# TheoCoombes/ClipCap

Measured on AMD Instinct MI355X. Metric: train samples/sec (512-d prefix, 40-tok caption), higher is better.
Workload: dtype bf16; 1 GPU; BASELINE configs[1]: TransformerMapper(8L,P=L=10,H=8)+frozen GPT-2-small; per_gpu_batch=256, global_batch=256, encoder_dim=512, train_language_model=False, parallelism=dp1

## Files before the change

### clipcap_amd/csrc/api.hip

```cpp
#include "../../include/clipcap_hip.h"
#include "gemm_api.h"
#include "kernels.h"
#include "shared.h"
#include "layout.h"
#include <vector>

using namespace CC_NS;

namespace {

#define CC_TIMED(site, st, expr)                 \
    do {                                         \
        cc_shared::ProfScope _ps(site, st);      \
        int _e = (expr);                         \
        if (_e != CC_OK) return _e;              \
    } while (0)

struct TileScope {
    int old;
    bool on;
    explicit TileScope(int mode) : old(cc_shared::g_gemm_tile_mode), on(mode != -2) { if (on) cc_shared::g_gemm_tile_mode = mode; }
    ~TileScope() { if (on) cc_shared::g_gemm_tile_mode = old; }
};
inline int env_tile(const char* name) {
// ... 70 lines not shown
        w.wg_scratch = cv.take<float>(WGRAD_SCRATCH_BYTES / sizeof(float));
        w.red = cv.take<float>(RED_SCRATCH_FLOATS);
        w.adelta = cv.take<float>((size_t)B * c->H * S);
        w.gimg = kX3 ? reinterpret_cast<uint16_t*>(cv.take<char>(x3_img(M, std::max<size_t>(3 * (size_t)D, c->Hm)))) : nullptr;
    } else {
        w.dx32 = nullptr; w.dx16 = w.dx16b = w.dh16 = w.dxn16 = w.datt16 = w.dqkv16 = w.dlin16 = nullptr; w.wg_scratch = nullptr; w.adelta = nullptr;
        w.red = nullptr;
        w.gimg = nullptr;
        for (int l = 0; l < c->N; l++) w.gdx[l] = w.gdxb[l] = w.gdh[l] = w.gdqkv[l] = nullptr;
        w.own_grads = false;
    }
    w.x3 = nullptr; w.x3_bytes = 0;
    if (kX3) {
        const size_t Hm = c->Hm, Mb = (size_t)B * c->W, PD = (size_t)c->P * D;
        size_t need = std::max(x3_img(Mb, c->E), x3_img(M, std::max(D, Hm)));
        if (save) {
            need = std::max(need, x3_img(M, 3 * D));
            need = std::max(need, std::max(x3_img(M, D) + x3_img(M, Hm), x3_img(M, 3 * D) + x3_img(M, D)));
            need = std::max(need, x3_img(Mb, PD) + x3_img(Mb, c->E));
        }
        w.x3_bytes = need;
        w.x3 = cv.take<char>(need);
    }
    w.bytes = cv.bytes();
}

struct MapperPass {
    hipStream_t st;
    MapperOff o;
    MapperWS w;
    Call cx;
    int D, PP, S, M, H, hd, Hm, PD;
    MapperPass(const cc_mapper_cfg* c, int B, int save, void* ws, void* stream)
        : st(S_(stream)), o(c), D(c->D), PP(c->W * c->P), S(PP + c->L), M(B * S), H(c->H), hd(c->D / c->H), Hm(c->Hm), PD(c->P * c->D) {
        mapper_carve(c, B, save, ws, w);
        cx = call_of(st, w);
    }
};

static bool x3_img_on() {
    static const bool on = []() { const char* e = cc_lab_env("CC_X3_IMG"); return !e || atoi(e) != 0; }();
    return on;
}
static bool lm_exp_form(const cc_gpt2_shape* s) {
    static const bool env = []() { const char* e = cc_lab_env("CC_LM_EXPFORM"); return !e || atoi(e) != 0; }();
    if (CC_OP == 0) return env;
    if (CC_OP == 2) return env && x3_img_on() && s->mode == 1;
    return false;
}
static Act lm_logits(const cc_gpt2_cfg* c, const cc_gpt2_shape* s, act_t* logits16) { return Act(logits16, (kX3 && lm_exp_form(s)) ? c->Vp : 0); }

struct Gpt2WS {
    float* x[MAX_LAYERS + 1];
    float* x1[MAX_LAYERS];
    act_t *qkv[MAX_LAYERS], *u[MAX_LAYERS];
    Act xn1[MAX_LAYERS], xn2[MAX_LAYERS], att[MAX_LAYERS], hact[MAX_LAYERS];
    float *lse[MAX_LAYERS], *mean1[MAX_LAYERS], *rstd1[MAX_LAYERS], *mean2[MAX_LAYERS], *rstd2[MAX_LAYERS];
    act_t* hf16;
    float *meanf, *rstdf;
    int *target, *row_map;
    int* keep;
    act_t* logits16;
    float *pmax, *psum, *tgt_logit, *lse_row, *row_loss;
    float *cref, *lmfac;
    act_t* hfs16;
    float* dx32;
    Act dx16, dx16b, du16, dqkv16;
    act_t *dhf16, *dxn16, *datt16;
    float* wg_scratch;
    float* red;
    void* scat;
    float* adelta;
    char* x3;
    size_t x3_bytes;
    size_t bytes;
};

void gpt2_carve(const cc_gpt2_cfg* c, const cc_gpt2_shape* s, int cap, void* ws, Gpt2WS& w) {
    Carver cv(ws);
    const int B = s->B, T = s->T, hd = c->D / c->H;
    const size_t M = (size_t)B * T, D = c->D, Mc = (size_t)B * cap;
    const bool keep = s->mode >= 1, full = s->mode >= 2;
    const auto take_img = [&](size_t n) { return cv.take<act_t>(n * ((kX3 && !full) ? 3 : 2) / 2); };
    const bool img = kX3 && !full && x3_img_on();
    const bool bimg = img && keep && s->p_resid == 0.f && s->p_attn == 0.f && s->p_embd == 0.f;
    const int xw = img ? (int)D : 0, attw = (img && attn_fwd_can_image(T, hd)) ? (int)D : 0, hw = img ? 4 * (int)D : 0;
    const int dxw = bimg ? (int)D : 0, dqw = (bimg && attn_bwd_can_image(T, hd)) ? 3 * (int)D : 0;
    const int nx = keep ? c->NL + 1 : 2;
    float* xb[MAX_LAYERS + 1];
    for (int i = 0; i < nx; i++) xb[i] = cv.take<float>(M * D);
    for (int l = 0; l <= c->NL; l++) w.x[l] = keep ? xb[l] : xb[l & 1];
    for (int l = 0; l < c->NL; l++) {
        const bool k0 = keep || l == 0, f0 = full || l == 0;
        w.x1[l] = k0 ? cv.take<float>(M * D) : w.x1[0];
        w.qkv[l] = k0 ? cv.take<act_t>(M * 3 * D) : w.qkv[0];
        w.u[l] = k0 ? cv.take<act_t>(M * 4 * D) : w.u[0];
        w.lse[l] = k0 ? cv.take<float>((size_t)B * c->H * T) : w.lse[0];
        w.mean1[l] = k0 ? cv.take<float>(M) : w.mean1[0];
        w.rstd1[l] = k0 ? cv.take<float>(M) : w.rstd1[0];
        w.mean2[l] = k0 ? cv.take<float>(M) : w.mean2[0];
        w.rstd2[l] = k0 ? cv.take<float>(M) : w.rstd2[0];
        w.xn1[l] = f0 ? Act(take_img(M * D), xw) : w.xn1[0];
        w.xn2[l] = f0 ? Act(take_img(M * D), xw) : w.xn2[0];
        w.att[l] = k0 ? Act(take_img(M * D), attw) : w.att[0];
        w.hact[l] = f0 ? Act(take_img(M * 4 * D), hw) : w.hact[0];
    }
    const size_t Mh = std::max(M, Mc);
    w.hf16 = cv.take<act_t>(Mh * D);
    w.meanf = cv.take<float>(Mh);
    w.rstdf = cv.take<float>(Mh);
    w.target = cv.take<int>(Mh);
    w.row_map = cv.take<int>(Mh);
    w.keep = nullptr;
    if (keep) {
        const int npart = c->Vp / 64;
        w.logits16 = take_img(Mc * c->Vp);
        w.pmax = cv.take<float>(Mc * npart);
        w.psum = cv.take<float>(Mc * npart);
        w.tgt_logit = cv.take<float>(Mc);
        w.lse_row = cv.take<float>(Mc);
        w.row_loss = cv.take<float>(Mc);
        w.cref = cv.take<float>(Mc);
        w.lmfac = cv.take<float>(2 * Mc);
        w.hfs16 = full ? cv.take<act_t>(Mc * D) : nullptr;
        w.dx32 = cv.take<float>(M * D);
        w.dx16 = Act(take_img(M * D), dxw);
        w.dx16b = full ? Act(cv.take<act_t>(M * D)) : w.dx16;
        w.dhf16 = cv.take<act_t>(Mc * D);
        w.du16 = Act(take_img(M * 4 * D), hw);
        w.dxn16 = cv.take<act_t>(M * D);
        w.datt16 = cv.take<act_t>(M * D);
        w.dqkv16 = Act(take_img(M * 3 * D), dqw);
        w.wg_scratch = full ? cv.take<float>(WGRAD_SCRATCH_BYTES / sizeof(float)) : nullptr;
        w.red = full ? cv.take<float>(RED_SCRATCH_FLOATS) : nullptr;
        w.scat = full ? cv.take<char>(scatter_ws_bytes((int)Mc, (int)D)) : nullptr;
        w.adelta = cv.take<float>((size_t)B * c->H * T);
    } else {
        w.wg_scratch = nullptr; w.adelta = nullptr; w.red = nullptr; w.scat = nullptr;
        w.logits16 = nullptr; w.pmax = w.psum = w.tgt_logit = w.lse_row = w.row_loss = nullptr;
        w.cref = w.lmfac = nullptr; w.hfs16 = nullptr;
        w.dx32 = nullptr; w.dx16 = w.dx16b = w.du16 = w.dqkv16 = Act(); w.dhf16 = w.dxn16 = w.datt16 = nullptr;
        if (Mc > 0) {
            const int npart = c->Vp / 64;
            w.pmax = cv.take<float>(Mc * npart);
            w.psum = cv.take<float>(Mc * npart);
            w.tgt_logit = cv.take<float>(Mc);
            w.lse_row = cv.take<float>(Mc);
            w.keep = cv.take<int>(Mc);
        }
    }
    w.x3 = nullptr; w.x3_bytes = 0;
    if (kX3) {
        size_t need = x3_img(Mh, 4 * D);
        if (keep) need = std::max(need, x3_img(Mc, c->Vp));
        if (full) need = std::max(need, std::max(x3_img(M, D) + x3_img(M, 4 * D), x3_img(Mc, c->Vp) + x3_img(Mc, D)));
        w.x3_bytes = need;
        w.x3 = cv.take<char>(need);
    }
    w.bytes = cv.bytes();
}

struct Gpt2Pass {
    hipStream_t st;
    Gpt2Off o;
    Gpt2WS w;
    Call cx;
    int D, M, H, hd;
    Gpt2Pass(const cc_gpt2_cfg* c, const cc_gpt2_shape* s, int cap, void* ws, void* stream)
        : st(S_(stream)), o(c), D(c->D), M(s->B * s->T), H(c->H), hd(c->D / c->H) {
        gpt2_carve(c, s, cap, ws, w);
        cx = call_of(st, w);
    }
};

}

extern "C" {

int CC_API(cc_mapper_bwd_range)(const cc_mapper_cfg* c, int32_t B, const float* w32, const uint16_t* w16, void* ws, const float* dout, float* g32,
                        int32_t l_hi, int32_t l_lo, void* stream);
int CC_API(cc_gpt2_bwd_range)(const cc_gpt2_cfg* c, const cc_gpt2_shape* s, const float* w32, const uint16_t* w16, void* ws, const int64_t* tokens,
                      float* dprefix, float* g32, int32_t l_hi, int32_t l_lo, void* stream);

int64_t CC_API(cc_mapper_param_count)(const cc_mapper_cfg* cfg) {
    if (!mapper_cfg_ok(cfg)) return CC_ERR_SHAPE;
    return MapperOff(cfg).total;
}

int CC_API(cc_mapper_param_offsets)(const cc_mapper_cfg* cfg, int64_t* offs) {
    if (!mapper_cfg_ok(cfg) || !offs) return CC_ERR_SHAPE;
    const MapperOff o(cfg);
    *offs++ = o.lin_w; *offs++ = o.lin_b; *offs++ = o.prefix; *offs++ = o.pos;
    for (int l = 0; l < cfg->N; l++) offs = put_layer(offs, o.layer(l));
    return CC_OK;
}

int64_t CC_API(cc_mapper_ws_bytes)(const cc_mapper_cfg* cfg, int32_t B, int32_t save) {
    if (!mapper_cfg_ok(cfg) || B <= 0) return CC_ERR_SHAPE;
    MapperWS w;
    mapper_carve(cfg, B, save, nullptr, w);
    return (int64_t)w.bytes;
}

#if CC_OP == 2
static int mapper_sync_x3(const cc_mapper_cfg* c, const float* w32, uint16_t* w16, hipStream_t st) {
    const MapperOff o(c);
    const int D = c->D, Hm = c->Hm;
    X3SplitBatch sb;
    sb.add(w32 + o.lin_w, W16(w16, o.lin_w), c->P * D, c->E, 0, 1);
    for (int l = 0; l < c->N; l++) {
        const auto y = o.layer(l);
        const int64_t off[4] = {y.wq, y.wp, y.w1, y.w2};
        const int R[4] = {3 * D, D, Hm, D}, C[4] = {D, D, D, Hm};
        for (int i = 0; i < 4; i++) {
            if (sb.n + 2 > 32) { CC_TRY(x3_split_multi(sb, st)); sb.n = 0; }
            sb.add(w32 + off[i], W16(w16, off[i]), R[i], C[i], 0, 1);
            sb.add(w32 + off[i], W16(w16, o.total + off[i]), R[i], C[i], 1, 1);
        }
    }
    return x3_split_multi(sb, st);
}
#endif

static int mapper_transposes(const cc_mapper_cfg* c, uint16_t* w16, hipStream_t st) {
    if (kX3) return CC_ERR_ARG;
    const MapperOff o(c);
    op16_t* t = w16 + o.total;
    const int D = c->D, Hm = c->Hm;
    TransposeBatch tb;
    for (int l = 0; l < c->N; l++) {
        const auto y = o.layer(l);
        tb.add(w16 + y.wq, t + y.wq, 3 * D, D);
        tb.add(w16 + y.wp, t + y.wp, D, D);
        tb.add(w16 + y.w1, t + y.w1, Hm, D);
        tb.add(w16 + y.w2, t + y.w2, D, Hm);
        if (tb.n == 32) { CC_TRY(transpose_bf16_multi(tb, st)); tb.n = 0; }
    }
    CC_TRY(transpose_bf16_multi(tb, st));
    return CC_OK;
}

int CC_API(cc_mapper_sync_weights)(const cc_mapper_cfg* c, const float* w32, uint16_t* w16, void* stream) {
    if (!mapper_cfg_ok(c) || !w32 || !w16) return CC_ERR_ARG;
    hipStream_t st = S_(stream);
#if CC_OP == 2
    return mapper_sync_x3(c, w32, w16, st);
#else
    CC_TRY(f32_to_bf16(w32, w16, (size_t)MapperOff(c).total, st));
    return mapper_transposes(c, w16, st);
#endif
}

int CC_API(cc_mapper_transpose_weights)(const cc_mapper_cfg* c, uint16_t* w16, void* stream) {
    if (!mapper_cfg_ok(c) || !w16) return CC_ERR_ARG;
    return mapper_transposes(c, w16, S_(stream));
}

int CC_API(cc_mapper_fwd)(const cc_mapper_cfg* c, int32_t B, const float* w32, const uint16_t* w16, const float* emb, void* ws, float* out,
                  int32_t save, void* stream) {
    if (!mapper_cfg_ok(c) || B <= 0 || !w32 || !w16 || !emb || !ws || !out) return CC_ERR_ARG;
    MapperPass ps(c, B, save, ws, stream);
    auto& [st, o, w, cx, D, PP, S, M, H, hd, Hm, PD] = ps;
    CC_TRY(f32_to_act(emb, w.emb16, (size_t)B * c->W * c->E, st));
    if (c->W == 1) {
        CC_TRY(gemm_f32out(0, 0, w.emb16, c->E, W16(w16, o.lin_w), c->E, B, PD, c->E, w.x[0], S * D, w32 + o.lin_b, 0, 1.0f, 1, cx));
    } else {
        CC_TRY(gemm_f32out(0, 0, w.emb16, c->E, W16(w16, o.lin_w), c->E, B * c->W, PD, c->E, w.lin_tmp, PD, w32 + o.lin_b, 0, 1.0f, 1, cx));
        CC_TRY(copy_rows(w.lin_tmp, (size_t)PP * D, w.x[0], (size_t)S * D, PP * D, B, st));
        if (o.pos >= 0) CC_TRY(add_rows(w.x[0], (size_t)S * D, w32 + o.pos, PP * D, B, st));
    }
    CC_TRY(broadcast_rows(w.x[0] + (size_t)PP * D, (size_t)S * D, w32 + o.prefix, c->L * D, B, st));
    for (int l = 0; l < c->N; l++) {
        const auto y = o.layer(l);
        CC_TRY(ln_fwd(w.x[l], D, nullptr, w32 + y.n1w, w32 + y.n1b, w.xn1[l], nullptr, w.mean1[l], w.rstd1[l], M, D, st));
        CC_TIMED(CC_SITE_MAPPER_QKV_FWD, st, gemm_bf16out(0, 0, w.xn1[l], D, W16(w16, y.wq), D, M, 3 * D, D, w.qkv[l], 3 * D, nullptr, 0, nullptr, cx));
        CC_TRY(attn_fwd(w.qkv[l], B, S, H, hd, false, w.att[l], w.lse[l], st));
        CC_TRY(gemm_resid(0, 0, w.att[l], D, W16(w16, y.wp), D, M, D, D, w.x1[l], w.x[l], D, w32 + y.bp, cx));
        CC_TRY(ln_fwd(w.x1[l], D, nullptr, w32 + y.n2w, w32 + y.n2b, w.xn2[l], nullptr, w.mean2[l], w.rstd2[l], M, D, st));
        CC_TIMED(CC_SITE_MAPPER_FC1_FWD, st, gemm_bf16out(0, 0, w.xn2[l], D, W16(w16, y.w1), D, M, Hm, D, w.h[l], Hm, w32 + y.b1, 1, nullptr, cx));
        CC_TRY(gemm_resid(0, 0, w.h[l], Hm, W16(w16, y.w2), Hm, M, D, Hm, w.x[l + 1], w.x1[l], D, w32 + y.b2, cx));
    }
    CC_TRY(copy_rows(w.x[c->N] + (size_t)PP * D, (size_t)S * D, out, (size_t)c->L * D, c->L * D, B, st));
    return CC_OK;
}

int CC_API(cc_mapper_attention_probs)(const cc_mapper_cfg* c, int32_t B, void* ws, int32_t layer, float* out, void* stream) {
    if (!mapper_cfg_ok(c) || B <= 0 || !ws || !out || layer < 0 || layer >= c->N) return CC_ERR_ARG;
    MapperPass ps(c, B, 1, ws, stream);
    return attn_probs(ps.w.qkv[layer], B, ps.S, ps.H, ps.hd, out, ps.st);
}

int CC_API(cc_mapper_bwd)(const cc_mapper_cfg* c, int32_t B, const float* w32, const uint16_t* w16, void* ws, const float* dout, float* g32,
                  void* stream) {
    if (!mapper_cfg_ok(c)) return CC_ERR_ARG;
    return CC_API(cc_mapper_bwd_range)(c, B, w32, w16, ws, dout, g32, c->N, 0, stream);
}

int CC_API(cc_mapper_bwd_range)(const cc_mapper_cfg* c, int32_t B, const float* w32, const uint16_t* w16, void* ws, const float* dout, float* g32,
                        int32_t l_hi, int32_t l_lo, void* stream) {
    if (!mapper_cfg_ok(c) || B <= 0 || !w32 || !w16 || !ws || !dout || !g32 || l_lo < 0 || l_hi > c->N || l_lo > l_hi) return CC_ERR_ARG;
    MapperPass ps(c, B, 1, ws, stream);
    auto& [st, o, w, cx, D, PP, S, M, H, hd, Hm, PD] = ps;
    const uint16_t* w16t = W16(w16, o.total);
    if (l_hi == c->N) {
        if (hipMemsetAsync(w.dx32, 0, (size_t)M * D * sizeof(float), st) != hipSuccess) return CC_ERR_LAUNCH;
        CC_TRY(copy_rows(dout, (size_t)c->L * D, w.dx32 + (size_t)PP * D, (size_t)S * D, c->L * D, B, st));
        if (c->N > 0) CC_TRY(f32_to_act(w.dx32, w.gdx[c->N - 1], (size_t)M * D, st));
    }
    WgradBatch wb;
    wb.defer = true;
    constexpr bool kDeferAll = !kX3;
    static const bool defer_all_on = []() { const char* e = cc_lab_env("CC_MAPPER_WGRAD_DEFER"); return !e || atoi(e) != 0; }();
    static const int defer_rows = []() { const char* e = cc_lab_env("CC_MAPPER_DEFER_ROWS"); return e ? std::min(atoi(e), kDeferRows) : kDeferRows; }();
    const bool defer_all = kDeferAll && defer_all_on && w.own_grads && 4 * (l_hi - l_lo) <= 32 && M <= defer_rows;
    if (defer_all) { wb.direct = true; wb.cap = 4 * (l_hi - l_lo); }
    ColsumBatch cs;
#if CC_OP == 2
    static const bool share = []() { const char* e = cc_lab_env("CC_X3_SHARE"); return !e || atoi(e) != 0; }();
    int g2rc = CC_OK;
    auto G2 = [&](const act_t* t, int width) -> ActIn {
        if (!share) return t;
        auto& [st, o, w, cx, D, PP, S, M, H, hd, Hm, PD] = ps;
        g2rc = x3_split_rows(t, (size_t)width, w.gimg, M, width, 0, st);
        return ActIn(reinterpret_cast<const act_t*>(w.gimg), width);
    };
#else
    auto G2 = [&](const act_t* t, int) -> ActIn { return t; };
    const int g2rc = CC_OK;
#endif
    for (int l = l_hi - 1; l >= l_lo; l--) {
        const auto y = o.layer(l);
        act_t* dx16 = w.gdx[l];
        act_t* dx16b = w.gdxb[l];
        act_t* dh16 = w.gdh[l];
        act_t* dqkv16 = w.gdqkv[l];
        act_t* dx16_below = l > 0 ? w.gdx[l - 1] : w.datt16;
        const ActIn gx = G2(dx16, D);
        CC_TRY(g2rc);
        CC_TIMED(CC_SITE_MAPPER_WGRAD_FC2, st, gemm_wgrad(gx, D, w.h[l], Hm, D, Hm, M, g32 + y.w2, Hm, w.wg_scratch, cx, &wb));
        if (l == c->N - 1) CC_TRY(colsum_bf16(dx16, D, M, D, g32 + y.b2, cx));
        CC_TRY(gemm_dact(0, 0, gx, D, W16(w16t, y.w2), D, M, Hm, D, dh16, Hm, w.h[l], 1, cx));
        const ActIn gh = G2(dh16, Hm);
        CC_TRY(g2rc);
        CC_TRY(gemm_wgrad(gh, Hm, w.xn2[l], D, Hm, D, M, g32 + y.w1, D, w.wg_scratch, cx, &wb));
        if (defer_all) cs.add(dh16, g32 + y.b1);
        else CC_TRY(colsum_bf16(dh16, Hm, M, Hm, g32 + y.b1, cx));
        CC_TRY(gemm_bf16out(0, 0, gh, Hm, W16(w16t, y.w1), Hm, M, D, Hm, w.dxn16, D, nullptr, 0, nullptr, cx));
        CC_TRY(ln_bwd(w.dxn16, w.x1[l], D, nullptr, w.mean2[l], w.rstd2[l], w32 + y.n2w, w.dx32, w.dx32, dx16b, g32 + y.n2w,
                      g32 + y.n2b, M, D, cx, g32 + y.bp));
        const ActIn gb = G2(dx16b, D);
        CC_TRY(g2rc);
        CC_TRY(gemm_wgrad(gb, D, w.att[l], D, D, D, M, g32 + y.wp, D, w.wg_scratch, cx, &wb));
        CC_TRY(gemm_bf16out(0, 0, gb, D, W16(w16t, y.wp), D, M, D, D, w.datt16, D, nullptr, 0, nullptr, cx));
        CC_TRY(attn_bwd(w.qkv[l], w.datt16, w.att[l], w.lse[l], w.adelta, B, S, H, hd, false, dqkv16, st));
        const ActIn gq = G2(dqkv16, 3 * D);
        CC_TRY(g2rc);
        CC_TRY(gemm_wgrad(gq, 3 * D, w.xn1[l], D, 3 * D, D, M, g32 + y.wq, D, w.wg_scratch, cx, &wb));
        CC_TRY(gemm_bf16out(0, 0, gq, 3 * D, W16(w16t, y.wq), 3 * D, M, D, 3 * D, w.dxn16, D, nullptr, 0, nullptr, cx));
        if (!defer_all) CC_TRY(wgrad_flush(wb, st));
        CC_TRY(ln_bwd(w.dxn16, w.x[l], D, nullptr, w.mean1[l], w.rstd1[l], w32 + y.n1w, w.dx32, w.dx32, dx16_below, g32 + y.n1w,
                      g32 + y.n1b, M, D, cx, l > 0 ? g32 + o.layer(l - 1).b2 : nullptr));
    }
    CC_TRY(wgrad_flush(wb, st));
    CC_TRY(colsum_bf16_multi(cs, Hm, M, Hm, cx));
    if (l_lo > 0) return CC_OK;
    CC_TRY(batch_sum(w.dx32 + (size_t)PP * D, (size_t)S * D, g32 + o.prefix, c->L * D, B, cx));
    if (o.pos >= 0) CC_TRY(batch_sum(w.dx32, (size_t)S * D, g32 + o.pos, PP * D, B, cx));
    CC_TRY(slice_f32_to_bf16(w.dx32, (size_t)S * D, w.dlin16, (size_t)PP * D, PP * D, B, st));
    CC_TRY(gemm_wgrad(w.dlin16, PD, w.emb16, c->E, PD, c->E, B * c->W, g32 + o.lin_w, c->E, w.wg_scratch, cx));
    CC_TRY(colsum_bf16(w.dlin16, PD, B * c->W, PD, g32 + o.lin_b, cx));
    return CC_OK;
}

namespace {
static bool gelu_grad_fwd() {
    static const bool on = []() { const char* e = cc_lab_env("CC_GELU_GRAD_FWD"); return !e || atoi(e) != 0; }();
    return on;
}
static bool shape_ok(const cc_gpt2_cfg* c, const cc_gpt2_shape* s) {
    return s && s->B > 0 && s->T > 0 && s->L >= 0 && s->L <= s->T && s->cap >= s->T - s->L && s->mode >= 0 && s->mode <= 2 && s->T <= c->NPOS &&
           s->p_embd >= 0.f && s->p_embd < 1.f && s->p_attn >= 0.f && s->p_attn < 1.f && s->p_resid >= 0.f && s->p_resid < 1.f;
}
}

int64_t CC_API(cc_gpt2_param_count)(const cc_gpt2_cfg* cfg) {
    if (!gpt2_cfg_ok(cfg)) return CC_ERR_SHAPE;
    return Gpt2Off(cfg).total;
}

int CC_API(cc_gpt2_param_offsets)(const cc_gpt2_cfg* cfg, int64_t* offs) {
    if (!gpt2_cfg_ok(cfg) || !offs) return CC_ERR_SHAPE;
    const Gpt2Off o(cfg);
    *offs++ = o.wte; *offs++ = o.wpe;
    for (int l = 0; l < cfg->NL; l++) offs = put_layer(offs, o.layer(l));
    *offs++ = o.lnf_w; *offs++ = o.lnf_b;
    return CC_OK;
}

int64_t CC_API(cc_gpt2_ws_bytes)(const cc_gpt2_cfg* cfg, const cc_gpt2_shape* s) {
    if (!gpt2_cfg_ok(cfg) || !shape_ok(cfg, s)) return CC_ERR_SHAPE;
    Gpt2WS w;
    gpt2_carve(cfg, s, s->T - s->L, nullptr, w);
    return (int64_t)w.bytes;
}

#if CC_OP == 2
static int gpt2_sync_x3(const cc_gpt2_cfg* c, const float* w32, uint16_t* w16, hipStream_t st) {
    const Gpt2Off o(c);
    const int D = c->D;
    X3SplitBatch sb;
    sb.add(w32 + o.wte, W16(w16, o.wte), c->Vp, D, 0, 1);
    sb.add(w32 + o.wte, W16(w16, o.total + o.wte), c->Vp, D, 1, 1);
    CC_TRY(x3_split_multi(sb, st));
    sb.n = 0;
    for (int l = 0; l < c->NL; l++) {
        const auto y = o.layer(l);
        const int64_t off[4] = {y.aw, y.pw, y.fw, y.p2w};
        const int R[4] = {D, D, D, 4 * D}, C[4] = {3 * D, D, 4 * D, D};
        for (int i = 0; i < 4; i++) {
            if (sb.n + 2 > 32) { CC_TRY(x3_split_multi(sb, st)); sb.n = 0; }
            sb.add(w32 + off[i], W16(w16, off[i]), R[i], C[i], 0, 1);
            sb.add(w32 + off[i], W16(w16, o.total + off[i]), R[i], C[i], 1, 1);
        }
    }
    return x3_split_multi(sb, st);
}
#endif

static int gpt2_transposes(const cc_gpt2_cfg* c, uint16_t* w16, hipStream_t st) {
    if (kX3) return CC_ERR_ARG;
    const Gpt2Off o(c);
    op16_t* t = w16 + o.total;
    const int D = c->D;
    CC_TRY(transpose_bf16(w16 + o.wte, t + o.wte, c->Vp, D, st));
    TransposeBatch tb;
    for (int l = 0; l < c->NL; l++) {
        const auto y = o.layer(l);
        tb.add(w16 + y.aw, t + y.aw, D, 3 * D);
        tb.add(w16 + y.pw, t + y.pw, D, D);
        tb.add(w16 + y.fw, t + y.fw, D, 4 * D);
        tb.add(w16 + y.p2w, t + y.p2w, 4 * D, D);
        if (tb.n == 32) { CC_TRY(transpose_bf16_multi(tb, st)); tb.n = 0; }
    }
    CC_TRY(transpose_bf16_multi(tb, st));
    return CC_OK;
}

int CC_API(cc_gpt2_sync_weights)(const cc_gpt2_cfg* c, const float* w32, uint16_t* w16, void* stream) {
    if (!gpt2_cfg_ok(c) || !w32 || !w16) return CC_ERR_ARG;
    hipStream_t st = S_(stream);
#if CC_OP == 2
    return gpt2_sync_x3(c, w32, w16, st);
#else
    CC_TRY(f32_to_bf16(w32, w16, (size_t)Gpt2Off(c).total, st));
    return gpt2_transposes(c, w16, st);
#endif
}

int CC_API(cc_gpt2_transpose_weights)(const cc_gpt2_cfg* c, uint16_t* w16, void* stream) {
    if (!gpt2_cfg_ok(c) || !w16) return CC_ERR_ARG;
    return gpt2_transposes(c, w16, S_(stream));
}

int CC_API(cc_dropout_mask)(uint64_t seed, int32_t site, int32_t layer, float p, int64_t n, uint8_t* out, void* stream) {
    if (!out || n < 0 || site < 0 || site > 3 || layer < 0 || layer > 255 || p < 0.f || p >= 1.f) return CC_ERR_ARG;
    return dropout_mask_u8(out, (size_t)n, make_drop(p, seed, (unsigned)site, (unsigned)layer), S_(stream));
}

int CC_API(cc_gpt2_embed)(const cc_gpt2_cfg* c, const cc_gpt2_shape* s, const float* w32, const float* prefix, const int64_t* tokens, void* ws,
                  void* stream) {
    if (!gpt2_cfg_ok(c) || !shape_ok(c, s) || !w32 || !ws || (s->L > 0 && !prefix) || (s->T > s->L && !tokens)) return CC_ERR_ARG;
    Gpt2Pass ps(c, s, s->T - s->L, ws, stream);
    auto& [st, o, w, cx, D, M, H, hd] = ps;
    CC_TRY(embed_concat(prefix, reinterpret_cast<const long long*>(tokens), s->cap, w32 + o.wte, w32 + o.wpe, w.x[0], s->B, s->L, s->T, D, 0, st));
    return dropout_f32(w.x[0], (size_t)s->B * s->T * D, make_drop(s->p_embd, s->drop_seed, DROP_EMBD, 0), st);
}

int CC_API(cc_gpt2_embed_from)(const cc_gpt2_cfg* c, const cc_gpt2_shape* s, const float* w32, const float* inputs_embeds, void* ws,
                       void* stream) {
    if (!gpt2_cfg_ok(c) || !shape_ok(c, s) || !w32 || !ws || !inputs_embeds) return CC_ERR_ARG;
    Gpt2Pass ps(c, s, s->T - s->L, ws, stream);
    return embed_concat(inputs_embeds, nullptr, 0, w32 + ps.o.wte, w32 + ps.o.wpe, ps.w.x[0], s->B, s->T, s->T, ps.D, 0, ps.st);
}

int CC_API(cc_gpt2_fwd)(const cc_gpt2_cfg* c, const cc_gpt2_shape* s, const float* w32, const uint16_t* w16, void* ws, void* stream) {
    if (!gpt2_cfg_ok(c) || !shape_ok(c, s) || !w32 || !w16 || !ws) return CC_ERR_ARG;
    Gpt2Pass ps(c, s, s->T - s->L, ws, stream);
    auto& [st, o, w, cx, D, M, H, hd] = ps;
    const uint16_t* w16t = W16(w16, o.total);
    for (int l = 0; l < c->NL; l++) {
        const auto y = o.layer(l);
        CC_TRY(ln_fwd(w.x[l], D, nullptr, w32 + y.l1w, w32 + y.l1b, w.xn1[l], nullptr, w.mean1[l], w.rstd1[l], M, D, st));
        CC_TRY(gemm_bf16out(0, 0, w.xn1[l], D, W16(w16t, y.aw), D, M, 3 * D, D, w.qkv[l], 3 * D, w32 + y.ab, 0, nullptr, cx));
        CC_TRY(attn_fwd(w.qkv[l], s->B, s->T, H, hd, true, w.att[l], w.lse[l], st, make_drop(s->p_attn, s->drop_seed, DROP_ATTN, l)));
        {
            static const int tile_proj = env_tile("CC_TILE_PROJ");
            TileScope ts(tile_proj);
            CC_TRY(gemm_resid(0, 0, w.att[l], D, W16(w16t, y.pw), D, M, D, D, w.x1[l], w.x[l], D, w32 + y.pb, cx,
                              make_drop(s->p_resid, s->drop_seed, DROP_RESID_ATTN, l)));
        }
        CC_TRY(ln_fwd(w.x1[l], D, nullptr, w32 + y.l2w, w32 + y.l2b, w.xn2[l], nullptr, w.mean2[l], w.rstd2[l], M, D, st));
        {
            static const int tile_fc = env_tile("CC_TILE_FC");
            TileScope ts(tile_fc);
            CC_TIMED(CC_SITE_GPT2_FC_FWD, st, gemm_bf16out(0, 0, w.xn2[l], D, W16(w16t, y.fw), D, M, 4 * D, D, w.hact[l], 4 * D, w32 + y.fb, (s->mode >= 1 && gelu_grad_fwd()) ? 3 : 2,
                                                            s->mode >= 1 ? w.u[l] : nullptr, cx));
        }
        {
            static const int tile_proj2 = env_tile("CC_TILE_PROJ2");
            TileScope ts(tile_proj2);
            CC_TIMED(CC_SITE_GPT2_PROJ2_FWD, st, gemm_resid(0, 0, w.hact[l], 4 * D, W16(w16t, y.p2w), 4 * D, M, D, 4 * D, w.x[l + 1], w.x1[l], D, w32 + y.p2b, cx,
                                                           make_drop(s->p_resid, s->drop_seed, DROP_RESID_MLP, l)));
        }
    }
    return CC_OK;
}

int CC_API(cc_gpt2_logits)(const cc_gpt2_cfg* c, const cc_gpt2_shape* s, const float* w32, const uint16_t* w16, void* ws, float* logits,
                   int64_t ldl, void* stream) {
    if (!gpt2_cfg_ok(c) || !shape_ok(c, s) || !w32 || !w16 || !ws || !logits) return CC_ERR_ARG;
    const int Ns = std::min(c->Vp, rup(c->V, 8));
    if (ldl < Ns || (ldl & 3) || ldl > 0x7fffffff) return CC_ERR_SHAPE;
    Gpt2Pass ps(c, s, s->T - s->L, ws, stream);
    auto& [st, o, w, cx, D, M, H, hd] = ps;
    CC_TRY(ln_fwd(w.x[c->NL], D, nullptr, w32 + o.lnf_w, w32 + o.lnf_b, w.hf16, nullptr, w.meanf, w.rstdf, M, D, st));
    return gemm_f32out(0, 0, w.hf16, D, W16(w16, o.wte), D, M, Ns, D, logits, (int)ldl, nullptr, 0, 1.0f, 1, cx);
}

int CC_API(cc_lmhead_ce_fwd)(const cc_gpt2_cfg* c, const cc_gpt2_shape* s, const float* w32, const uint16_t* w16, void* ws, const int64_t* tokens,
                     float* stats, void* stream) {
    if (!gpt2_cfg_ok(c) || !shape_ok(c, s) || s->mode < 1 || s->L < 1 || !w32 || !w16 || !ws || !tokens || !stats) return CC_ERR_ARG;
    const int cap = s->T - s->L;
    if (cap != s->cap) return CC_ERR_SHAPE;
    Gpt2Pass ps(c, s, cap, ws, stream);
    auto& [st, o, w, cx, D, M, H, hd] = ps;
    const int Mc = s->B * cap, npart = c->Vp / 64;
    if (hipMemsetAsync(stats, 0, 2 * sizeof(float), st) != hipSuccess) return CC_ERR_LAUNCH;
    CC_TRY(ce_targets(reinterpret_cast<const long long*>(tokens), w.target, w.row_map, s->B, cap, s->L, s->T, st));
    CC_TRY(ln_fwd(w.x[c->NL], D, w.row_map, w32 + o.lnf_w, w32 + o.lnf_b, w.hf16, nullptr, w.meanf, w.rstdf, Mc, D, st));
    const bool ef = lm_exp_form(s);
    const op16_t* wte_rows = kX3 ? reinterpret_cast<const op16_t*>(w32 + o.wte) : W16(w16, o.wte);
    if (ef) CC_TRY(lm_tgt_ref(w.hf16, wte_rows, D, w.target, w.cref, Mc, st));
    CC_TIMED(CC_SITE_LMHEAD_FWD, st, gemm_lmhead(w.hf16, D, W16(w16, o.wte), D, Mc, c->Vp, c->V, D, lm_logits(c, s, w.logits16), c->Vp, w.pmax, w.psum, npart, w.target, w.tgt_logit, cx,
                                                 ef ? w.cref : nullptr));
    CC_TRY(ce_rows(w.pmax, w.psum, npart, w.target, ef ? w.cref : w.tgt_logit, w.lse_row, w.row_loss, stats, Mc, st));
    return CC_OK;
}

int CC_API(cc_lmhead_score)(const cc_gpt2_cfg* c, const cc_gpt2_shape* s, const float* w32, const uint16_t* w16, void* ws, const int64_t* tokens,
                    int32_t ignore_zero, float* token_logprob, float* sample_stats, void* stream) {
    if (!gpt2_cfg_ok(c) || !shape_ok(c, s) || s->mode != 0 || s->L < 1 || !w32 || !w16 || !ws || !tokens || !token_logprob || !sample_stats)
        return CC_ERR_ARG;
    const int cap = s->T - s->L;
    if (cap < 1 || cap != s->cap) return CC_ERR_SHAPE;
    Gpt2Pass ps(c, s, cap, ws, stream);
    auto& [st, o, w, cx, D, M, H, hd] = ps;
    const int Mc = s->B * cap, npart = c->Vp / 64;
    CC_TRY(ce_targets(reinterpret_cast<const long long*>(tokens), w.target, w.row_map, s->B, cap, s->L, s->T, st));
    CC_TRY(score_keep(reinterpret_cast<const long long*>(tokens), w.keep, Mc, ignore_zero, st));
    CC_TRY(ln_fwd(w.x[c->NL], D, w.row_map, w32 + o.lnf_w, w32 + o.lnf_b, w.hf16, nullptr, w.meanf, w.rstdf, Mc, D, st));
    CC_TIMED(CC_SITE_LMHEAD_FWD, st, gemm_lmhead_score(w.hf16, D, W16(w16, o.wte), D, Mc, c->Vp, c->V, D, w.pmax, w.psum, npart, w.target, w.tgt_logit, cx));
    return score_rows(w.pmax, w.psum, npart, w.keep, w.tgt_logit, w.lse_row, token_logprob, sample_stats, s->B, cap, st);
}

int CC_API(cc_lmhead_ce_bwd)(const cc_gpt2_cfg* c, const cc_gpt2_shape* s, const float* w32, const uint16_t* w16, void* ws, const float* denom,
                     const float* loss_scale, float* g32, void* stream) {
    if (!gpt2_cfg_ok(c) || !shape_ok(c, s) || s->mode < 1 || !w32 || !w16 || !ws || !denom || (s->mode == 2 && !g32)) return CC_ERR_ARG;
    const int cap = s->T - s->L;
    Gpt2Pass ps(c, s, cap, ws, stream);
    auto& [st, o, w, cx, D, M, H, hd] = ps;
    const int Mc = s->B * cap;
    const bool full = s->mode == 2;
    const bool ef = lm_exp_form(s);
    const LmFix fix{w.lmfac, w.target, kX3 ? reinterpret_cast<const op16_t*>(w32 + o.wte) : W16(w16, o.wte)};
    if (ef) CC_TRY(lm_rowfac(w.cref, w.lse_row, w.target, denom, loss_scale, w.lmfac, Mc, st));
    const Act lg = lm_logits(c, s, w.logits16);
    ActIn dlog = lg;
    op16_t* dimg = (kX3 && !ef && !full && x3_img_on()) ? x3_scratch_block(cx, x3_img(Mc, c->Vp)) : nullptr;
    if (dimg) dlog = ActIn(reinterpret_cast<const act_t*>(dimg), c->Vp);
    if (!ef) CC_TRY(ce_dlogits(w.logits16, c->Vp, c->V, w.target, w.lse_row, denom, loss_scale, Mc, st, dimg));
    const auto lm_dgrad = [&]() {
        auto& [st, o, w, cx, D, M, H, hd] = ps;
        const int rc = gemm_nt_deepk(dlog, c->Vp, W16(w16, o.total + o.wte), c->Vp, Mc, D, c->Vp, w.dhf16, D, reinterpret_cast<float*>(w.du16.p),
                                     (size_t)M * 4 * D * sizeof(act_t), cx, ef ? &fix : nullptr);
        if (rc != CC_ERR_SHAPE) return rc;
        const int rc2 = gemm_bf16out(0, 0, dlog, c->Vp, W16(w16, o.total + o.wte), c->Vp, Mc, D, c->Vp, w.dhf16, D, nullptr, 0, nullptr, cx);
        return (rc2 != CC_OK || !ef) ? rc2 : lm_dgrad_fix(w.dhf16, w.lmfac, w.target, fix.wte, D, Mc, st);
    };
    CC_TIMED(CC_SITE_LMHEAD_DGRAD, st, lm_dgrad());
    if (full) {
        if (ef) {
            CC_TRY(lm_scale_rows(w.hf16, w.lmfac, w.hfs16, D, Mc, st));
            CC_TRY(gemm_wgrad(lg, c->Vp, w.hfs16, D, c->Vp, D, Mc, g32 + o.wte, D, w.wg_scratch, cx));
            ScatterSrc oh;
            oh.ids32 = w.target; oh.act = w.hf16; oh.fac = w.lmfac;
            CC_TRY(scatter_rows(oh, Mc, D, c->Vp, g32 + o.wte, w.scat, st));
        } else {
            CC_TRY(gemm_wgrad(lg, c->Vp, w.hf16, D, c->Vp, D, Mc, g32 + o.wte, D, w.wg_scratch, cx));
        }
    }
    if (hipMemsetAsync(w.dx32, 0, (size_t)M * D * sizeof(float), st) != hipSuccess) return CC_ERR_LAUNCH;
    const size_t dx16_bytes = (size_t)M * D * (w.dx16.img ? 3 * sizeof(op16_t) : sizeof(act_t));
    if (hipMemsetAsync(w.dx16.p, 0, dx16_bytes, st) != hipSuccess) return CC_ERR_LAUNCH;
    CC_TRY(ln_bwd(w.dhf16, w.x[c->NL], D, w.row_map, w.meanf, w.rstdf, w32 + o.lnf_w, nullptr, w.dx32, w.dx16, full ? g32 + o.lnf_w : nullptr,
                  full ? g32 + o.lnf_b : nullptr, Mc, D, cx));
    return CC_OK;
}

int CC_API(cc_lmhead_put_x)(const cc_gpt2_cfg* c, const cc_gpt2_shape* s, void* ws, const float* x, void* stream) {
    if (!gpt2_cfg_ok(c) || !shape_ok(c, s) || !ws || !x) return CC_ERR_ARG;
    Gpt2Pass ps(c, s, s->T - s->L, ws, stream);
    const size_t bytes = (size_t)s->B * s->T * c->D * sizeof(float);
    return hipMemcpyAsync(ps.w.x[c->NL], x, bytes, hipMemcpyDeviceToDevice, ps.st) == hipSuccess ? CC_OK : CC_ERR_LAUNCH;
}

int CC_API(cc_lmhead_get)(const cc_gpt2_cfg* c, const cc_gpt2_shape* s, void* ws, int32_t field, void* dst, int64_t dst_bytes, void* stream) {
    if (!gpt2_cfg_ok(c) || !shape_ok(c, s) || !ws || !dst || field < CC_LM_LSE || field > CC_LM_DX32) return CC_ERR_ARG;
    if (s->T - s->L < 1) return CC_ERR_SHAPE;
    Gpt2Pass ps(c, s, s->T - s->L, ws, stream);
    const Gpt2WS& w = ps.w;
    const size_t Mc = (size_t)s->B * (s->T - s->L), M = (size_t)s->B * s->T, D = c->D;
    const void* src = nullptr;
    size_t bytes = 0;
    switch (field) {
        case CC_LM_LSE: src = w.lse_row; bytes = Mc * sizeof(float); break;
        case CC_LM_TGT: src = (s->mode >= 1 && lm_exp_form(s)) ? w.cref : w.tgt_logit; bytes = Mc * sizeof(float); break;
        case CC_LM_ROW_LOSS: src = w.row_loss; bytes = Mc * sizeof(float); break;
        case CC_LM_HF: src = w.hf16; bytes = Mc * D * sizeof(act_t); break;
        case CC_LM_DHF: src = w.dhf16; bytes = Mc * D * sizeof(act_t); break;
        default: src = w.dx32; bytes = M * D * sizeof(float); break;
    }
    if (!src) return CC_ERR_STATE;
    if (dst_bytes < 0 || (size_t)dst_bytes != bytes) return CC_ERR_SHAPE;
    return hipMemcpyAsync(dst, src, bytes, hipMemcpyDeviceToDevice, ps.st) == hipSuccess ? CC_OK : CC_ERR_LAUNCH;
}

int CC_API(cc_gpt2_logits_bwd)(const cc_gpt2_cfg* c, const cc_gpt2_shape* s, const float* w32, const uint16_t* w16, void* ws, const float* dlogits,
                       int64_t ldl, float* dx0, float* g32, void* stream) {
    if (!gpt2_cfg_ok(c) || !shape_ok(c, s) || s->mode < 1 || s->L != 0 || !w32 || !w16 || !ws || !dlogits || ldl < c->V || (s->mode == 2 && !g32))
        return CC_ERR_ARG;
    Gpt2Pass ps(c, s, s->T, ws, stream);
    auto& [st, o, w, cx, D, M, H, hd] = ps;
    const bool full = s->mode == 2;
    CC_TRY(f32_to_op16_pad(dlogits, ldl, c->V, w.logits16, c->Vp, M, st));
    CC_TRY(gemm_bf16out(0, 0, w.logits16, c->Vp, W16(w16, o.total + o.wte), c->Vp, M, D, c->Vp, w.dhf16, D, nullptr, 0, nullptr, cx));
    if (full) CC_TRY(gemm_wgrad(w.logits16, c->Vp, w.hf16, D, c->Vp, D, M, g32 + o.wte, D, w.wg_scratch, cx));
    if (hipMemsetAsync(w.dx32, 0, (size_t)M * D * sizeof(float), st) != hipSuccess) return CC_ERR_LAUNCH;
    CC_TRY(ln_bwd(w.dhf16, w.x[c->NL], D, nullptr, w.meanf, w.rstdf, w32 + o.lnf_w, nullptr, w.dx32, w.dx16, full ? g32 + o.lnf_w : nullptr,
                  full ? g32 + o.lnf_b : nullptr, M, D, cx));
    CC_TRY(CC_API(cc_gpt2_bwd_range)(c, s, w32, w16, ws, nullptr, nullptr, g32, c->NL, 0, stream));
    if (dx0 && hipMemcpyAsync(dx0, w.dx32, (size_t)M * D * sizeof(float), hipMemcpyDeviceToDevice, st) != hipSuccess) return CC_ERR_LAUNCH;
    return CC_OK;
}

int CC_API(cc_gpt2_bwd)(const cc_gpt2_cfg* c, const cc_gpt2_shape* s, const float* w32, const uint16_t* w16, void* ws, const int64_t* tokens,
                float* dprefix, float* g32, void* stream) {
    if (!gpt2_cfg_ok(c)) return CC_ERR_ARG;
    return CC_API(cc_gpt2_bwd_range)(c, s, w32, w16, ws, tokens, dprefix, g32, c->NL, 0, stream);
}

int CC_API(cc_gpt2_bwd_range)(const cc_gpt2_cfg* c, const cc_gpt2_shape* s, const float* w32, const uint16_t* w16, void* ws, const int64_t* tokens,
                      float* dprefix, float* g32, int32_t l_hi, int32_t l_lo, void* stream) {
    if (!gpt2_cfg_ok(c) || !shape_ok(c, s) || s->mode < 1 || !w32 || !w16 || !ws || (s->L > 0 && !dprefix) || (s->mode == 2 && !g32) ||
        l_lo < 0 || l_hi > c->NL || l_lo > l_hi)
        return CC_ERR_ARG;
    Gpt2Pass ps(c, s, s->T - s->L, ws, stream);
    auto& [st, o, w, cx, D, M, H, hd] = ps;
    const int D3 = 3 * D, D4 = 4 * D;
    const bool full = s->mode == 2;
    WgradBatch wb;
    wb.defer = full;
    WgradBatch* wbp = full ? &wb : nullptr;
    if (full && (w.dx16.img || w.dx16b.img || w.du16.img || w.dqkv16.img)) return CC_ERR_STATE;
    for (int l = l_hi - 1; l >= l_lo; l--) {
        const auto y = o.layer(l);
        const bool top = l == c->NL - 1;
        if (top) CC_TRY(dropout_bf16(w.dx16.p, (size_t)M * D, make_drop(s->p_resid, s->drop_seed, DROP_RESID_MLP, l), st));
        if (full) {
            CC_TRY(gemm_wgrad(w.hact[l], D4, w.dx16.p, D, D4, D, M, g32 + y.p2w, D, w.wg_scratch, cx, wbp));
            if (top) CC_TRY(colsum_bf16(w.dx16.p, D, M, D, g32 + y.p2b, cx));
        }
        {
            static const int tile_dact = env_tile("CC_TILE_DACT");
            TileScope ts(tile_dact);
            CC_TRY(gemm_dact(0, 0, w.dx16, D, W16(w16, y.p2w), D, M, D4, D, w.du16, D4, w.u[l], gelu_grad_fwd() ? 3 : 2, cx));
        }
        if (full) {
            CC_TRY(gemm_wgrad(w.xn2[l], D, w.du16.p, D4, D, D4, M, g32 + y.fw, D4, w.wg_scratch, cx, wbp));
            CC_TRY(colsum_bf16(w.du16.p, D4, M, D4, g32 + y.fb, cx));
        }
        CC_TIMED(CC_SITE_GPT2_FC_DGRAD, st, gemm_bf16out(0, 0, w.du16, D4, W16(w16, y.fw), D4, M, D, D4, w.dxn16, D, nullptr, 0, nullptr, cx));
        CC_TRY(ln_bwd(w.dxn16, w.x1[l], D, nullptr, w.mean2[l], w.rstd2[l], w32 + y.l2w, w.dx32, w.dx32, w.dx16b, full ? g32 + y.l2w : nullptr,
                      full ? g32 + y.l2b : nullptr, M, D, cx, full ? g32 + y.pb : nullptr,
                      make_drop(s->p_resid, s->drop_seed, DROP_RESID_ATTN, l)));
        if (full) CC_TRY(gemm_wgrad(w.att[l], D, w.dx16b.p, D, D, D, M, g32 + y.pw, D, w.wg_scratch, cx, wbp));
        CC_TRY(gemm_bf16out(0, 0, w.dx16b, D, W16(w16, y.pw), D, M, D, D, w.datt16, D, nullptr, 0, nullptr, cx));
        CC_TRY(attn_bwd(w.qkv[l], w.datt16, w.att[l].p, w.lse[l], w.adelta, s->B, s->T, H, hd, true, w.dqkv16, st,
                        make_drop(s->p_attn, s->drop_seed, DROP_ATTN, l)));
        if (full) {
            CC_TRY(gemm_wgrad(w.xn1[l], D, w.dqkv16.p, D3, D, D3, M, g32 + y.aw, D3, w.wg_scratch, cx, wbp));
            CC_TRY(colsum_bf16(w.dqkv16.p, D3, M, D3, g32 + y.ab, cx));
        }
        CC_TRY(gemm_bf16out(0, 0, w.dqkv16, D3, W16(w16, y.aw), D3, M, D, D3, w.dxn16, D, nullptr, 0, nullptr, cx));
        if (full) CC_TRY(wgrad_flush(wb, st));
        CC_TRY(ln_bwd(w.dxn16, w.x[l], D, nullptr, w.mean1[l], w.rstd1[l], w32 + y.l1w, w.dx32, w.dx32, w.dx16, full ? g32 + y.l1w : nullptr,
                      full ? g32 + y.l1b : nullptr, M, D, cx, (full && l > 0) ? g32 + o.layer(l - 1).p2b : nullptr,
                      l > 0 ? make_drop(s->p_resid, s->drop_seed, DROP_RESID_MLP, l - 1) : Drop()));
    }
    if (l_lo > 0) return CC_OK;
    CC_TRY(dropout_f32(w.dx32, (size_t)M * D, make_drop(s->p_embd, s->drop_seed, DROP_EMBD, 0), st));
    if (s->L > 0) CC_TRY(copy_rows(w.dx32, (size_t)s->T * D, dprefix, (size_t)s->L * D, s->L * D, s->B, st));
    if (full) {
        if (tokens) {
            ScatterSrc e;
            e.ids64 = reinterpret_cast<const long long*>(tokens);
            e.ids_ld = s->cap;
            e.f32 = w.dx32 + (size_t)s->L * D; e.rpb = s->T - s->L; e.bstride = (size_t)s->T * D;
            CC_TRY(scatter_rows(e, s->B * (s->T - s->L), D, c->Vp, g32 + o.wte, w.scat, st));
        }
        CC_TRY(batch_sum(w.dx32, (size_t)s->T * D, g32 + o.wpe, s->T * D, s->B, cx));
    }
    return CC_OK;
}

int CC_API(cc_adamw_step)(float* p32, const float* g32, float* m, float* v, int64_t n, float lr, float beta1, float beta2, float eps,
                  float weight_decay, int32_t step, float grad_scale, const float* loss_scale, const float* found_inf, void* stream) {
    if (!p32 || !g32 || !m || !v || n < 0 || step < 0 || (step == 0 && !loss_scale)) return CC_ERR_ARG;
    return adamw(p32, g32, m, v, (size_t)n, lr, beta1, beta2, eps, weight_decay, step, grad_scale, loss_scale, found_inf, S_(stream));
}

int CC_API(cc_adamw_step_cast)(float* p32, const float* g32, float* m, float* v, int64_t n, float lr, float beta1, float beta2, float eps,
                       float weight_decay, int32_t step, float grad_scale, const float* loss_scale, const float* found_inf, uint16_t* w16, void* stream) {
    if (!p32 || !g32 || !m || !v || !w16 || n < 0 || step < 0 || (step == 0 && !loss_scale)) return CC_ERR_ARG;
    if (kX3) return CC_ERR_ARG;
    return adamw(p32, g32, m, v, (size_t)n, lr, beta1, beta2, eps, weight_decay, step, grad_scale, loss_scale, found_inf, S_(stream), w16);
}

int CC_API(cc_adamw_step_clip)(float* p32, const float* g32, float* m, float* v, int64_t n, float lr, float beta1, float beta2, float eps,
                       float weight_decay, int32_t step, float grad_scale, const float* loss_scale, const float* found_inf, const float* clip,
                       uint16_t* w16, void* stream) {
    if (!p32 || !g32 || !m || !v || n < 0 || step < 0 || (step == 0 && !loss_scale)) return CC_ERR_ARG;
    if (w16 && kX3) return CC_ERR_ARG;
    return adamw(p32, g32, m, v, (size_t)n, lr, beta1, beta2, eps, weight_decay, step, grad_scale, loss_scale, found_inf, S_(stream), w16, clip);
}

int64_t CC_API(cc_grad_norm_scratch_floats)(void) { return (int64_t)GRAD_NORM_BLOCKS; }

int CC_API(cc_cast_op16)(const float* src, uint16_t* dst, int64_t n, void* stream) {
    if (!src || !dst || n < 0 || kX3) return CC_ERR_ARG;
    return f32_to_bf16(src, dst, (size_t)n, S_(stream));
}

int CC_API(cc_gemm_op16_f32)(int32_t al, int32_t bl, const uint16_t* A, int32_t lda, const uint16_t* B, int32_t ldb, int32_t M, int32_t N, int32_t K,
                     float* C, int32_t ldc, const float* bias, int32_t ksplit, void* stream) {
    if (!A || !B || !C || kX3) return CC_ERR_ARG;
    Call cx{S_(stream)};
    return gemm_f32out(al, bl, reinterpret_cast<const act_t*>(A), lda, B, ldb, M, N, K, C, ldc, ksplit > 1 ? nullptr : bias, ksplit > 1 ? 2 : 0, 1.0f, ksplit, cx);
}

int64_t CC_API(cc_wgrad_scratch_bytes)(void) { return (int64_t)WGRAD_SCRATCH_BYTES; }

int CC_API(cc_gemm_wgrad)(const uint16_t* X, int32_t ldx, const uint16_t* Y, int32_t ldy, int32_t Mw, int32_t Nw, int32_t K, float* dW, int32_t ldw,
                  float* scratch, void* stream) {
    if (!X || !Y || !dW || kX3) return CC_ERR_ARG;
    Call cx{S_(stream)};
    return gemm_wgrad(reinterpret_cast<const act_t*>(X), ldx, reinterpret_cast<const act_t*>(Y), ldy, Mw, Nw, K, dW, ldw, scratch, cx);
}

int CC_API(cc_layernorm_fwd)(const float* x, const float* gamma, const float* beta, uint16_t* y, float* mean, float* rstd, int32_t rows, int32_t D,
                     void* stream) {
    if (!x || !gamma || !beta || !y) return CC_ERR_ARG;
    return ln_fwd(x, D, nullptr, gamma, beta, reinterpret_cast<act_t*>(y), nullptr, mean, rstd, rows, D, S_(stream));
}

int64_t CC_API(cc_red_scratch_floats)(void) { return (int64_t)RED_SCRATCH_FLOATS; }

int CC_API(cc_layernorm_bwd)(const uint16_t* dy, const float* x, int32_t ldx, const int32_t* row_map, const float* mean, const float* rstd,
                     const float* gamma, const float* dres, float* dx32, uint16_t* dx16, float* dgamma, float* dbeta, float* dcol, int32_t rows,
                     int32_t D, float* red_ws, void* stream) {
    if (!dy || !x || !mean || !rstd || !gamma || !dx32 || !dgamma != !dbeta || kX3) return CC_ERR_ARG;
    Call cx{S_(stream), red_ws};
    return ln_bwd(reinterpret_cast<const act_t*>(dy), x, ldx, row_map, mean, rstd, gamma, dres, dx32, reinterpret_cast<act_t*>(dx16), dgamma,
                  dbeta, rows, D, cx, dcol);
}

int CC_API(cc_colsum_bf16)(const uint16_t* X, int32_t ld, int32_t M, int32_t N, float* out, float* red_ws, void* stream) {
    if (!X || !out || kX3) return CC_ERR_ARG;
    Call cx{S_(stream), red_ws};
    return colsum_bf16(reinterpret_cast<const act_t*>(X), ld, M, N, out, cx);
}

int CC_API(cc_colsum_multi)(const uint16_t* const* X_host, float* const* out_host, int32_t n, int32_t ld, int32_t M, int32_t N, float* red_ws,
                    void* stream) {
    if (!X_host || !out_host || n < 0 || n > 32 || kX3) return CC_ERR_ARG;
    ColsumBatch b;
    for (int i = 0; i < n; i++) {
        if (!X_host[i] || !out_host[i]) return CC_ERR_ARG;
        b.add(reinterpret_cast<const act_t*>(X_host[i]), out_host[i]);
    }
    Call cx{S_(stream), red_ws};
    return colsum_bf16_multi(b, ld, M, N, cx);
}

int CC_API(cc_batch_sum)(const float* src, int64_t src_stride, float* dst, int32_t len, int32_t B, float* red_ws, void* stream) {
    if (!src || !dst || len < 0 || src_stride < len) return CC_ERR_ARG;
    Call cx{S_(stream), red_ws};
    return batch_sum(src, (size_t)src_stride, dst, len, B, cx);
}

int CC_API(cc_attention_fwd)(const uint16_t* qkv, int32_t B, int32_t S, int32_t H, int32_t hd, int32_t causal, uint16_t* out, float* lse, void* stream) {
    if (!qkv || !out) return CC_ERR_ARG;
    return attn_fwd(reinterpret_cast<const act_t*>(qkv), B, S, H, hd, causal != 0, reinterpret_cast<act_t*>(out), lse, S_(stream));
}

int CC_API(cc_attention_bwd)(const uint16_t* qkv, const uint16_t* dout, const uint16_t* o, const float* lse, float* delta_ws, int32_t B, int32_t S,
                     int32_t H, int32_t hd, int32_t causal, uint16_t* dqkv, void* stream) {
    if (!qkv || !dout || !lse || !dqkv) return CC_ERR_ARG;
    return attn_bwd(reinterpret_cast<const act_t*>(qkv), reinterpret_cast<const act_t*>(dout), reinterpret_cast<const act_t*>(o), lse, delta_ws, B, S, H, hd,
                    causal != 0, reinterpret_cast<act_t*>(dqkv), S_(stream));
}

int CC_API(cc_attention_fwd_x)(const uint16_t* qkv, int32_t B, int32_t S, int32_t H, int32_t hd, int32_t causal, uint16_t* out, int32_t out_img, float* lse,
                       float p, uint64_t seed, int32_t layer, void* stream) {
    if (!qkv || !out || !(p >= 0.f && p < 1.f) || layer < 0 || layer > 255 || out_img < 0 || (!kX3 && out_img)) return CC_ERR_ARG;
    return attn_fwd(reinterpret_cast<const act_t*>(qkv), B, S, H, hd, causal != 0, Act(reinterpret_cast<act_t*>(out), out_img), lse, S_(stream),
                    make_drop(p, seed, DROP_ATTN, (unsigned)layer));
}

int CC_API(cc_attention_bwd_x)(const uint16_t* qkv, const uint16_t* dout, const uint16_t* o, const float* lse, float* delta_ws, int32_t B, int32_t S,
                       int32_t H, int32_t hd, int32_t causal, uint16_t* dqkv, int32_t dqkv_img, float p, uint64_t seed, int32_t layer, void* stream) {
    if (!qkv || !dout || !lse || !dqkv || !(p >= 0.f && p < 1.f) || layer < 0 || layer > 255 || dqkv_img < 0 || (!kX3 && dqkv_img)) return CC_ERR_ARG;
    return attn_bwd(reinterpret_cast<const act_t*>(qkv), reinterpret_cast<const act_t*>(dout), reinterpret_cast<const act_t*>(o), lse, delta_ws, B, S, H, hd,
                    causal != 0, Act(reinterpret_cast<act_t*>(dqkv), dqkv_img), S_(stream), make_drop(p, seed, DROP_ATTN, (unsigned)layer));
}

namespace {
inline bool al16(const void* p) { return ((uintptr_t)p & 15) == 0; }
inline bool hook_operands_ok(int al, int bl, const void* A, int a_img, int lda, const void* B, int ldb, int M, int N, int K) {
    if (!A || !B || !al16(A) || !al16(B) || M <= 0 || N <= 0 || K <= 0 || a_img < 0) return false;
    if (!kX3 && a_img) return false;
    return lda >= (a_img ? 0 : (al ? M : K)) && ldb >= (bl ? N : K);
}
inline void hook_scratch(Call& cx, void* x3, int64_t x3_bytes) {
    if (kX3 && x3 && x3_bytes > 0 && al16(x3)) { cx.x3 = static_cast<char*>(x3); cx.x3_bytes = (size_t)x3_bytes; }
}
inline bool hook_c_img_ok(int c_img, int N) { return c_img == 0 || (kX3 && c_img == N); }
}

int64_t CC_API(cc_x3_image_bytes)(int64_t rows, int64_t depth) {
    if (rows < 0 || depth < 0) return CC_ERR_ARG;
    return (int64_t)x3_img((size_t)rows, (size_t)depth);
}

int CC_API(cc_x3_split_rows)(const float* src, int64_t ld, int32_t rows, int32_t width, int32_t form, uint16_t* dst, void* stream) {
#if CC_OP == 2
    if (!src || !dst || rows < 0 || width < 0 || ld < width || (form != 0 && form != 1)) return CC_ERR_ARG;
    return x3_split_rows(src, (size_t)ld, dst, rows, width, form, S_(stream));
#else
    (void)src; (void)ld; (void)rows; (void)width; (void)form; (void)dst; (void)stream;
    return CC_ERR_ARG;
#endif
}

int CC_API(cc_gemm_act)(int32_t al, int32_t bl, const void* A, int32_t a_img, int32_t lda, const uint16_t* B, int32_t ldb, int32_t M, int32_t N, int32_t K,
                void* C, int32_t c_img, int32_t ldc, const float* bias, int32_t act, void* pre, void* x3, int64_t x3_bytes, void* stream) {
    if (!hook_operands_ok(al, bl, A, a_img, lda, B, ldb, M, N, K) || !C || !al16(C) || !al16(pre) || !al16(bias) || ldc < N || act < 0 || act > 3 ||
        !hook_c_img_ok(c_img, N))
        return CC_ERR_ARG;
    Call cx{S_(stream)};
    hook_scratch(cx, x3, x3_bytes);
    return gemm_bf16out(al, bl, ActIn(static_cast<const act_t*>(A), a_img), lda, B, ldb, M, N, K, Act(static_cast<act_t*>(C), c_img), ldc, bias, act,
                        static_cast<act_t*>(pre), cx);
}

int CC_API(cc_gemm_resid)(int32_t al, int32_t bl, const void* A, int32_t a_img, int32_t lda, const uint16_t* B, int32_t ldb, int32_t M, int32_t N, int32_t K,
                  float* out, const float* res, int32_t ld, const float* bias, float p, uint64_t seed, int32_t site, int32_t layer, void* x3,
                  int64_t x3_bytes, void* stream) {
    if (!hook_operands_ok(al, bl, A, a_img, lda, B, ldb, M, N, K) || !out || !res || !al16(out) || !al16(res) || !al16(bias) || ld < N || site < 0 ||
        site > 3 || layer < 0 || layer > 255 || p < 0.f || p >= 1.f)
        return CC_ERR_ARG;
    Call cx{S_(stream)};
    hook_scratch(cx, x3, x3_bytes);
    return gemm_resid(al, bl, ActIn(static_cast<const act_t*>(A), a_img), lda, B, ldb, M, N, K, out, res, ld, bias, cx,
                      make_drop(p, seed, (unsigned)site, (unsigned)layer));
}

int CC_API(cc_gemm_dact)(int32_t al, int32_t bl, const void* A, int32_t a_img, int32_t lda, const uint16_t* B, int32_t ldb, int32_t M, int32_t N, int32_t K,
                 void* C, int32_t c_img, int32_t ldc, const void* aux, int32_t act, void* x3, int64_t x3_bytes, void* stream) {
    if (!hook_operands_ok(al, bl, A, a_img, lda, B, ldb, M, N, K) || !C || !aux || !al16(C) || !al16(aux) || ldc < N || act < 1 || act > 3 ||
        !hook_c_img_ok(c_img, N))
        return CC_ERR_ARG;
    Call cx{S_(stream)};
    hook_scratch(cx, x3, x3_bytes);
    return gemm_dact(al, bl, ActIn(static_cast<const act_t*>(A), a_img), lda, B, ldb, M, N, K, Act(static_cast<act_t*>(C), c_img), ldc,
                     static_cast<const act_t*>(aux), act, cx);
}

int CC_API(cc_gemm_f32)(int32_t al, int32_t bl, const void* A, int32_t a_img, int32_t lda, const uint16_t* B, int32_t ldb, int32_t M, int32_t N, int32_t K,
                float* C, int32_t ldc, const float* bias, int32_t mode, float alpha, int32_t ksplit, void* x3, int64_t x3_bytes, void* stream) {
    if (!hook_operands_ok(al, bl, A, a_img, lda, B, ldb, M, N, K) || !C || !al16(C) || !al16(bias) || ldc < N || mode < 0 || mode > 2 || ksplit < 1 ||
        (bias && mode != 0))
        return CC_ERR_ARG;
    Call cx{S_(stream)};
    hook_scratch(cx, x3, x3_bytes);
    return gemm_f32out(al, bl, ActIn(static_cast<const act_t*>(A), a_img), lda, B, ldb, M, N, K, C, ldc, bias, mode, alpha, ksplit, cx);
}

int CC_API(cc_gemm_wgrad_split)(const void* X, int32_t x_img, int32_t ldx, const float* Y, int32_t ldy, int32_t Mw, int32_t Nw, int32_t K, float* dW,
                     int32_t ldw, float* scratch, void* x3, int64_t x3_bytes, void* stream) {
#if CC_OP == 2
    if (!X || !Y || !dW || !al16(X) || !al16(Y) || !al16(dW) || Mw <= 0 || Nw <= 0 || K <= 0 || x_img < 0 || (!x_img && ldx < Mw) || ldy < Nw || ldw < Nw)
        return CC_ERR_ARG;
    Call cx{S_(stream)};
    hook_scratch(cx, x3, x3_bytes);
    return gemm_wgrad(ActIn(static_cast<const act_t*>(X), x_img), ldx, Y, ldy, Mw, Nw, K, dW, ldw, scratch, cx);
#else
    (void)X; (void)x_img; (void)ldx; (void)Y; (void)ldy; (void)Mw; (void)Nw; (void)K; (void)dW; (void)ldw; (void)scratch; (void)x3; (void)x3_bytes; (void)stream;
    return CC_ERR_ARG;
#endif
}

}
```

### clipcap_amd/csrc/attention.hip

```cpp
#include "kernels.h"

namespace CC_NS {

__device__ __forceinline__ void load_head_rows(float* dst, int hdp, const act_t* src, size_t ld, int S, int hd) {
    const int c8n = hd >> 3;
    for (int idx = threadIdx.x; idx < S * c8n; idx += blockDim.x) {
        const int r = idx / c8n, c = idx % c8n;
        float f[8];
        act_ld8(src + (size_t)r * ld + c * 8, f);
        float* d = dst + r * hdp + c * 8;
        *reinterpret_cast<float4*>(d) = make_float4(f[0], f[1], f[2], f[3]);
        *reinterpret_cast<float4*>(d + 4) = make_float4(f[4], f[5], f[6], f[7]);
    }
}

template <auto Kernel, class... Args>
static void attn_launch(dim3 grid, dim3 block, size_t sh, hipStream_t st, const Args&... args) {
    if (sh > 64 * 1024) (void)hipFuncSetAttribute((const void*)Kernel, hipFuncAttributeMaxDynamicSharedMemorySize, (int)sh);
    hipLaunchKernelGGL(Kernel, grid, block, sh, st, args...);
}
#define ATTN_LADDER(LAUNCH) { if (drop.thresh) { LAUNCH(true, true); } else if (causal) { LAUNCH(true, false); } else { LAUNCH(false, false); } }

__device__ __forceinline__ unsigned attn_drop_idx(int b, int H, int h, int S, int q, int k) { return ((unsigned)(b * H + h) * S + q) * S + k; }
template <bool CAUSAL>
// ... 223 lines not shown
            ps += p[r];
        }
        ps += __shfl_xor(ps, 32, 64);
        l = l * alpha + ps;
        m = m_new;
#pragma unroll
        for (int nb = 0; nb < NB; nb++)
#pragma unroll
            for (int r = 0; r < 16; r++) o[nb][r] *= alpha;
        if (DROP) {
            const unsigned rowbase = attn_drop_idx(b, H, h, S, min(q, S - 1), 0);
#pragma unroll
            for (int r = 0; r < 16; r++) p[r] *= drop_mul(drop, rowbase + min(kb * 32 + c_row(r, half), S - 1));
        }
        op16x8 ph[2], pl[2];
#pragma unroll
        for (int t = 0; t < 2; t++) {
            const float f[8] = {p[t * 8 + 0], p[t * 8 + 1], p[t * 8 + 2], p[t * 8 + 3], p[t * 8 + 4], p[t * 8 + 5], p[t * 8 + 6], p[t * 8 + 7]};
            x3_split8(f, ph[t], pl[t]);
        }
#pragma unroll
        for (int t = 0; t < 2; t++)
#pragma unroll
            for (int nb = 0; nb < NB; nb++) {
                const op16x8 fh = frag_tr<HD>(vh, nb, t, lane), fl = frag_tr<HD>(vl, nb, t, lane);
                o[nb] = CC_MFMA_32x32x16(fl, ph[t], o[nb]);
                o[nb] = CC_MFMA_32x32x16(fh, pl[t], o[nb]);
                o[nb] = CC_MFMA_32x32x16(fh, ph[t], o[nb]);
            }
    }
    if (q < S) {
        const float inv = l > 0.f ? 1.f / l : 0.f;
#pragma unroll
        for (int nb = 0; nb < NB; nb++)
#pragma unroll
            for (int g = 0; g < 4; g++) {
                const int d0 = nb * 32 + 8 * g + 4 * half;
                const float o0 = o[nb][g * 4 + 0] * inv, o1 = o[nb][g * 4 + 1] * inv, o2 = o[nb][g * 4 + 2] * inv, o3 = o[nb][g * 4 + 3] * inv;
                if (img) {
                    const unsigned h01 = pack2op(o0, o1), h23 = pack2op(o2, o3);
                    float a0, a1, a2, a3;
                    unpack2(h01, a0, a1);
                    unpack2(h23, a2, a3);
                    const uint2 hi = make_uint2(h01, h23), lo = make_uint2(pack2op(o0 - a0, o1 - a1), pack2op(o2 - a2, o3 - a3));
                    op16_t* r3 = reinterpret_cast<op16_t*>(out) + ((size_t)b * S + q) * 3 * D + h * HD + d0;
                    *reinterpret_cast<uint2*>(r3) = hi;
                    *reinterpret_cast<uint2*>(r3 + D) = hi;
                    *reinterpret_cast<uint2*>(r3 + 2 * D) = lo;
                } else {
                    *reinterpret_cast<float4*>(out + ((size_t)b * S + q) * D + h * HD + d0) = make_float4(o0, o1, o2, o3);
                }
            }
        if (half == 0 && lse_out) lse_out[((size_t)b * H + h) * S + q] = m + __logf(l);
    }
}
template <int HD>
static int attn_fwd_mfma3_launch(const float* qkv, int B, int S, int H, bool causal, float* out, float* lse, hipStream_t st, Drop drop, int img) {
    const int items = B * H * ((S + 31) / 32);
    const float scale = 1.0f / sqrtf((float)HD);
    if (drop.thresh && !causal) return CC_ERR_SHAPE;
#define CC_L(C, DR) attn_launch<k_attn_fwd_mfma3<HD, C, DR>>(dim3((items + 3) / 4), dim3(256), 0, st, qkv, B, S, H, scale, out, lse, drop, img)
    ATTN_LADDER(CC_L)
#undef CC_L
    return hipGetLastError() == hipSuccess ? CC_OK : CC_ERR_LAUNCH;
}
template <int LD>
__device__ __forceinline__ op16x8 frag_tr_p(const op16_t* blk, int nb, int t, int lane) {
    typedef __attribute__((ext_vector_type(4))) short s16x4_t;
    typedef __attribute__((address_space(3))) s16x4_t* lp_t;
    const int half = lane >> 5, j = lane & 15, dsub = (lane >> 4) & 1;
    const op16_t* p = blk + (16 * t + 4 * half + (j >> 2)) * LD + nb * 32 + 16 * dsub + 4 * (j & 3);
    const s16x4_t lo = __builtin_amdgcn_ds_read_tr16_b64_v4i16((lp_t)p);
    const s16x4_t hi = __builtin_amdgcn_ds_read_tr16_b64_v4i16((lp_t)(p + 8 * LD));
    typedef __attribute__((ext_vector_type(8))) short s16x8_t;
    const s16x8_t v = {lo[0], lo[1], lo[2], lo[3], hi[0], hi[1], hi[2], hi[3]};
    return __builtin_bit_cast(op16x8, v);
}
__device__ __forceinline__ op16x8 frag_row_p(const op16_t* row, int t, int half) {
    const uint2 a = *reinterpret_cast<const uint2*>(row + 16 * t + 4 * half), c = *reinterpret_cast<const uint2*>(row + 16 * t + 8 + 4 * half);
    return __builtin_bit_cast(op16x8, make_uint4(a.x, a.y, c.x, c.y));
}
#define CC_MFMA3(AH, AL, BH, BL, ACC) { ACC = CC_MFMA_32x32x16(AL, BH, ACC); ACC = CC_MFMA_32x32x16(AH, BL, ACC); ACC = CC_MFMA_32x32x16(AH, BH, ACC); }
template <int HD, int NBLK> struct AttM3 {
    static constexpr int R = 32 * NBLK, LD = AttLd<HD>::v, LDP = NBLK == 2 ? 96 : 32, SP = NBLK == 2 ? 68 : 32, NW = NBLK == 2 ? 8 : 4;
    static constexpr int PLANE = R * LD, PPLANE = R * LDP;
    static constexpr size_t lds = (size_t)8 * PLANE * 2 + (size_t)4 * PPLANE * 2 + R * 4;
};
template <int HD, int NBLK, bool CAUSAL, bool DROP>
__global__ __launch_bounds__(NBLK == 2 ? 512 : 256, 1) void k_attn_bwd_m3(const float* __restrict__ qkv, const float* __restrict__ dout,
                                                                              const float* __restrict__ lse, int B, int S, int H, float scale,
                                                                              float* __restrict__ dqkv, Drop drop, int img) {
    typedef AttM3<HD, NBLK> G;
    constexpr int R = G::R, LD = G::LD, LDP = G::LDP, SP = G::SP, NW = G::NW, NB = HD / 32, KK = HD / 16, C8 = HD / 8, NT = 64 * NW;
    static_assert((size_t)2 * R * SP * 4 <= (size_t)4 * G::PPLANE * 2, "the fp32 scratch lives in the P / dS plane area");
    extern __shared__ __attribute__((aligned(16))) unsigned char m3raw[];
    op16_t* pl = reinterpret_cast<op16_t*>(m3raw);
    op16_t* Qh = pl, *Ql = pl + G::PLANE, *Kh = pl + 2 * G::PLANE, *Kl = pl + 3 * G::PLANE, *Vh = pl + 4 * G::PLANE, *Vl = pl + 5 * G::PLANE;
    op16_t* Oh = pl + 6 * G::PLANE, *Ol = pl + 7 * G::PLANE;
    op16_t* pp = pl + 8 * G::PLANE;
    op16_t* Ph = pp, *Pl = pp + G::PPLANE, *Dh = pp + 2 * G::PPLANE, *Dl = pp + 3 * G::PPLANE;
    float* scrS = reinterpret_cast<float*>(pp);
    float* scrD = scrS + R * SP;
    float* lse_s = reinterpret_cast<float*>(pp + 4 * G::PPLANE);
    const int tid = threadIdx.x, lane = tid & 63, wave = tid >> 6, half = lane >> 5, l31 = lane & 31;
    const int D = H * HD, nitems = B * H;
    const size_t rs = (size_t)3 * D;
    constexpr int PER = 4 * R * C8 / NT;
    static_assert(PER * NT == 4 * R * C8, "staging items tile the threads");
    float4 x[PER], y[PER];
    float lse_r = 0.f;
    auto request = [&](int item) {
        const int b_ = item / H, h_ = item - b_ * H;
        const float* base = qkv + (size_t)b_ * S * rs + h_ * HD;
        const float* dbase = dout + (size_t)b_ * S * D + h_ * HD;
#pragma unroll
        for (int it = 0; it < PER; it++) {
            const int idx = tid + it * NT;
            const int which = idx / (R * C8), rem = idx - which * (R * C8), row = rem / C8, c = rem - row * C8;
            const float* src = which == 3 ? dbase + (size_t)min(row, S - 1) * D + c * 8 : base + which * D + (size_t)min(row, S - 1) * rs + c * 8;
            x[it] = *reinterpret_cast<const float4*>(src);
            y[it] = *reinterpret_cast<const float4*>(src + 4);
        }
        if (tid < R) lse_r = lse[((size_t)b_ * H + h_) * S + min(tid, S - 1)];
    };
    if ((int)blockIdx.x < nitems) request(blockIdx.x);
    for (int item = blockIdx.x; item < nitems; item += gridDim.x) {
    const int b = item / H, h = item - b * H;
    {
#pragma unroll
        for (int it = 0; it < PER; it++) {
            const int idx = tid + it * NT;
            const int which = idx / (R * C8), rem = idx - which * (R * C8), row = rem / C8, c = rem - row * C8;
            const bool ok = row < S;
            const float f[8] = {ok ? x[it].x : 0.f, ok ? x[it].y : 0.f, ok ? x[it].z : 0.f, ok ? x[it].w : 0.f,
                                ok ? y[it].x : 0.f, ok ? y[it].y : 0.f, ok ? y[it].z : 0.f, ok ? y[it].w : 0.f};
            op16x8 hi, lo;
            x3_split8(f, hi, lo);
            *reinterpret_cast<op16x8*>(pl + (2 * which) * G::PLANE + row * LD + c * 8) = hi;
            *reinterpret_cast<op16x8*>(pl + (2 * which + 1) * G::PLANE + row * LD + c * 8) = lo;
        }
        if (tid < R) lse_s[tid] = tid < S ? lse_r : 0.f;
    }
    if (item + (int)gridDim.x < nitems) request(item + gridDim.x);
    __syncthreads();
    {
        constexpr int NTILE = CAUSAL ? NBLK * (NBLK + 1) / 2 : NBLK * NBLK;
        for (int job = wave; job < 2 * NTILE; job += NW) {
            const int prod = job & 1, tl = job >> 1;
            int i, j;
            if (CAUSAL) { i = tl == 0 ? 0 : 1; j = tl == 2 ? 1 : 0; if (NBLK == 1) { i = 0; j = 0; } }
            else { i = tl / NBLK; j = tl % NBLK; }
            const op16_t* ah = (prod ? Oh : Qh) + (i * 32 + l31) * LD + 8 * half;
            const op16_t* al = (prod ? Ol : Ql) + (i * 32 + l31) * LD + 8 * half;
            const op16_t* bh = (prod ? Vh : Kh) + (j * 32 + l31) * LD + 8 * half;
            const op16_t* bl = (prod ? Vl : Kl) + (j * 32 + l31) * LD + 8 * half;
            f32x16 acc;
#pragma unroll
            for (int r = 0; r < 16; r++) acc[r] = 0.f;
#pragma unroll
            for (int kk = 0; kk < KK; kk++) {
                const op16x8 a_h = *reinterpret_cast<const op16x8*>(ah + kk * 16), a_l = *reinterpret_cast<const op16x8*>(al + kk * 16);
                const op16x8 b_h = *reinterpret_cast<const op16x8*>(bh + kk * 16), b_l = *reinterpret_cast<const op16x8*>(bl + kk * 16);
                CC_MFMA3(a_h, a_l, b_h, b_l, acc)
            }
            float* dst = (prod ? scrD : scrS) + j * 32 + l31;
#pragma unroll
            for (int r = 0; r < 16; r++) dst[(i * 32 + (r & 3) + 8 * (r >> 2) + 4 * half) * SP] = acc[r];
        }
    }
    __syncthreads();
    {
        constexpr int CPR = R / 8;
        const int q = tid / CPR, c = tid - q * CPR;
        const bool act = q < R;
        float pm[8], ds[8];
        {
            float sv[8], dv[8];
            const float* ps = scrS + (act ? q : 0) * SP + c * 8;
            const float* pd = scrD + (act ? q : 0) * SP + c * 8;
            const float4 s0 = *reinterpret_cast<const float4*>(ps), s1 = *reinterpret_cast<const float4*>(ps + 4);
            const float4 d0 = *reinterpret_cast<const float4*>(pd), d1 = *reinterpret_cast<const float4*>(pd + 4);
            sv[0] = s0.x; sv[1] = s0.y; sv[2] = s0.z; sv[3] = s0.w; sv[4] = s1.x; sv[5] = s1.y; sv[6] = s1.z; sv[7] = s1.w;
            dv[0] = d0.x; dv[1] = d0.y; dv[2] = d0.z; dv[3] = d0.w; dv[4] = d1.x; dv[5] = d1.y; dv[6] = d1.z; dv[7] = d1.w;
            const float lq = lse_s[act ? q : 0];
            float dpm[8], dl = 0.f;
#pragma unroll
            for (int e = 0; e < 8; e++) {
                const int key = c * 8 + e;
                const bool ok = act && attn_live<CAUSAL>(q, key, S);
                const float pe = ok ? __expf(sv[e] * scale - lq) : 0.f;
                const float mk = DROP ? drop_mul(drop, attn_drop_idx(b, H, h, S, min(q, S - 1), min(key, S - 1))) : 1.f;
                dpm[e] = ok ? dv[e] * mk : 0.f;
                dl += pe * dpm[e];
                pm[e] = pe;
                ds[e] = mk;
            }
#pragma unroll
            for (int o = CPR / 2; o > 0; o >>= 1) dl += __shfl_xor(dl, o, 64);
#pragma unroll
            for (int e = 0; e < 8; e++) {
                const float mk = ds[e];
                ds[e] = pm[e] * (dpm[e] - dl) * scale;
                pm[e] *= mk;
            }
        }
        __syncthreads();
        if (act) {
            op16x8 ph, plo, dh, dlo;
            x3_split8(pm, ph, plo);
            x3_split8(ds, dh, dlo);
            *reinterpret_cast<op16x8*>(Ph + q * LDP + c * 8) = ph;
            *reinterpret_cast<op16x8*>(Pl + q * LDP + c * 8) = plo;
            *reinterpret_cast<op16x8*>(Dh + q * LDP + c * 8) = dh;
            *reinterpret_cast<op16x8*>(Dl + q * LDP + c * 8) = dlo;
        }
    }
    __syncthreads();
    for (int job = wave; job < 3 * NBLK * NB; job += NW) {
        const int kind = job / (NBLK * NB), rem = job - kind * (NBLK * NB), blk = rem / NB, nb = rem - blk * NB;
        f32x16 acc;
#pragma unroll
        for (int r = 0; r < 16; r++) acc[r] = 0.f;
        if (kind == 0) {
            const int jn = CAUSAL ? blk + 1 : NBLK;
            for (int j = 0; j < jn; j++)
#pragma unroll
                for (int t = 0; t < 2; t++) {
                    const op16x8 a_h = frag_row_p(Dh + (blk * 32 + l31) * LDP + j * 32, t, half), a_l = frag_row_p(Dl + (blk * 32 + l31) * LDP + j * 32, t, half);
                    const op16x8 b_h = frag_tr_p<LD>(Kh + j * 32 * LD, nb, t, lane), b_l = frag_tr_p<LD>(Kl + j * 32 * LD, nb, t, lane);
                    CC_MFMA3(a_h, a_l, b_h, b_l, acc)
                }
        } else {
            const op16_t* Ah = kind == 1 ? Dh : Ph, *Al = kind == 1 ? Dl : Pl, *Bh = kind == 1 ? Qh : Oh, *Bl = kind == 1 ? Ql : Ol;
            for (int i = CAUSAL ? blk : 0; i < NBLK; i++)
#pragma unroll
                for (int t = 0; t < 2; t++) {
                    const op16x8 a_h = frag_tr_p<LDP>(Ah + i * 32 * LDP, blk, t, lane), a_l = frag_tr_p<LDP>(Al + i * 32 * LDP, blk, t, lane);
                    const op16x8 b_h = frag_tr_p<LD>(Bh + i * 32 * LD, nb, t, lane), b_l = frag_tr_p<LD>(Bl + i * 32 * LD, nb, t, lane);
                    CC_MFMA3(a_h, a_l, b_h, b_l, acc)
                }
        }
        const int d = nb * 32 + l31;
        if (img) {
            const int odd = lane & 1;
            op16_t* r3 = reinterpret_cast<op16_t*>(dqkv) + (size_t)b * S * 9 * D + kind * D + h * HD + (d & ~1);
#pragma unroll
            for (int rp = 0; rp < 8; rp++) {
                const float v0 = acc[2 * rp], v1 = acc[2 * rp + 1];
                const float got = __shfl_xor(odd ? v0 : v1, 1, 64);
                const float a0 = odd ? got : v0, a1 = odd ? v1 : got;
                const int row = blk * 32 + ((2 * rp) & 3) + 8 * ((2 * rp) >> 2) + 4 * half + odd;
                const unsigned hi = pack2op(a0, a1);
                float h0, h1;
                unpack2(hi, h0, h1);
                const unsigned lo = pack2op(a0 - h0, a1 - h1);
                if (row < S) {
                    op16_t* o3 = r3 + (size_t)row * 9 * D;
                    *reinterpret_cast<unsigned*>(o3) = hi;
                    *reinterpret_cast<unsigned*>(o3 + 3 * D) = hi;
                    *reinterpret_cast<unsigned*>(o3 + 6 * D) = lo;
                }
            }
        } else {
            float* o1 = dqkv + (size_t)b * S * rs + kind * D + h * HD + d;
#pragma unroll
            for (int r = 0; r < 16; r++) {
                const int row = blk * 32 + (r & 3) + 8 * (r >> 2) + 4 * half;
                if (row < S) o1[(size_t)row * rs] = acc[r];
            }
        }
    }
    __syncthreads();
    }
}
template <int HD, int NBLK>
static int attn_bwd_m3_launch(const float* qkv, const float* dout, const float* lse, int B, int S, int H, bool causal, float* dqkv, hipStream_t st,
                              Drop drop, int img) {
    typedef AttM3<HD, NBLK> G;
    const float scale = 1.0f / sqrtf((float)HD);
    static int ncu = 0;
    if (!ncu) {
        int dev = 0;
        hipDeviceProp_t pr;
        if (hipGetDevice(&dev) != hipSuccess || hipGetDeviceProperties(&pr, dev) != hipSuccess) return CC_ERR_STATE;
        ncu = pr.multiProcessorCount;
    }
    const int per_cu = (int)((size_t)160 * 1024 / G::lds);
    const dim3 grid(min(B * H, ncu * max(1, per_cu))), blk(64 * G::NW);
    if (drop.thresh && !causal) return CC_ERR_SHAPE;
#define CC_L(C, DR) attn_launch<k_attn_bwd_m3<HD, NBLK, C, DR>>(grid, blk, G::lds, st, qkv, dout, lse, B, S, H, scale, dqkv, drop, img)
    ATTN_LADDER(CC_L)
#undef CC_L
    return hipGetLastError() == hipSuccess ? CC_OK : CC_ERR_LAUNCH;
}
static bool attn_x3mfma_on();
static bool attn_bwd_m3_ok(int S, int hd) { return attn_x3mfma_on() && (hd == 64 || hd == 96) && S > 0 && S <= 64; }
static bool attn_x3mfma_on() {
    static const bool on = !(cc_lab_env("CC_ATTN_X3MFMA") && atoi(cc_lab_env("CC_ATTN_X3MFMA")) == 0) && !cc_lab_env("CC_ATTN_F32MFMA");
    return on;
}
#endif

#if CC_OP != 2
template <int HD, bool CAUSAL, bool DROP = false>
__global__ __launch_bounds__(256, HD == 64 ? 3 : 2) void k_attn_fwd_mfma(const op16_t* __restrict__ qkv, int B, int S, int H, float scale,
                                                       op16_t* __restrict__ out, float* __restrict__ lse_out, Drop drop = Drop()) {
    constexpr int KK = HD / 16, NB = HD / 32, C8 = HD / 8;
    __shared__ __attribute__((aligned(16))) op16_t vsm[4][32 * AttLd<HD>::v];
    const int lane = threadIdx.x & 63, wave = threadIdx.x >> 6;
    const int nqb = (S + 31) >> 5;
    const int item = blockIdx.x * 4 + wave;
    if (item >= B * H * nqb) return;
    const int qb = item % nqb, h = (item / nqb) % H, b = item / (nqb * H);
    const int D = H * HD;
    const size_t rs = (size_t)3 * D;
    const op16_t* base = qkv + (size_t)b * S * rs + h * HD;
    const int half = lane >> 5, q = qb * 32 + (lane & 31);
    op16_t* vs = vsm[wave];

    op16x8 qf[KK];
#pragma unroll
    for (int kk = 0; kk < KK; kk++) {
        qf[kk] = load_frag(base + (size_t)min(q, S - 1) * rs + kk * 16 + half * 8, q < S);
    }
    f32x16 o[NB];
    acc_zero(o);
    float m = -INFINITY, l = 0.f;
    const int nkb = CAUSAL ? qb + 1 : nqb;
    uint4 kq[KK], vq[HD / 16];
    auto fetch = [&](int kb, uint4 (&kd)[KK], uint4 (&vd)[HD / 16]) {
        const int key = kb * 32 + (lane & 31);
#pragma unroll
        for (int kk = 0; kk < KK; kk++) {
            kd[kk] = *reinterpret_cast<const uint4*>(base + D + (size_t)min(key, S - 1) * rs + kk * 16 + half * 8);
            if (key >= S) kd[kk] = make_uint4(0, 0, 0, 0);
        }
#pragma unroll
        for (int c = 0; c < HD / 16; c++) {
            const int idx = lane + 64 * c;
            const int vk = idx / C8, vc = idx % C8;
            vd[c] = *reinterpret_cast<const uint4*>(base + 2 * D + (size_t)min(kb * 32 + vk, S - 1) * rs + vc * 8);
            if (kb * 32 + vk >= S) vd[c] = make_uint4(0, 0, 0, 0);
        }
    };
    fetch(0, kq, vq);
    for (int kb = 0; kb < nkb; kb++) {
        uint4 kn[KK], vn[HD / 16];
        fetch(kb + 1, kn, vn);
        f32x16 s;
        acc_zero(s);
#pragma unroll
        for (int kk = 0; kk < KK; kk++) s = CC_MFMA_32x32x16(__builtin_bit_cast(op16x8, kq[kk]), qf[kk], s);
#pragma unroll
        for (int c = 0; c < HD / 16; c++) {
            const int idx = lane + 64 * c;
            *reinterpret_cast<uint4*>(vs + (idx / C8) * AttLd<HD>::v + (idx % C8) * 8) = vq[c];
        }
        float mx = -INFINITY;
#pragma unroll
        for (int r = 0; r < 16; r++) {
            const int kr = kb * 32 + c_row(r, half);
            const bool ok = kr < S && (!CAUSAL || kr <= q);
            s[r] = ok ? s[r] * scale : -INFINITY;
            mx = fmaxf(mx, s[r]);
        }
        mx = fmaxf(mx, __shfl_xor(mx, 32, 64));
        const float m_new = fmaxf(m, mx);
        const float alpha = (m == -INFINITY) ? 0.f : __expf(m - m_new);
        float p[16], ps = 0.f;
#pragma unroll
        for (int r = 0; r < 16; r++) {
            p[r] = (m_new == -INFINITY) ? 0.f : __expf(s[r] - m_new);
            ps += p[r];
        }
        ps += __shfl_xor(ps, 32, 64);
        l = l * alpha + ps;
        m = m_new;
#pragma unroll
        for (int nb = 0; nb < NB; nb++)
#pragma unroll
            for (int r = 0; r < 16; r++) o[nb][r] *= alpha;
        if (DROP) {
            const unsigned rowbase = attn_drop_idx(b, H, h, S, min(q, S - 1), 0);
#pragma unroll
            for (int r = 0; r < 16; r++) p[r] *= drop_mul(drop, rowbase + min(kb * 32 + c_row(r, half), S - 1));
        }
        op16x8 pf[2];
#pragma unroll
        for (int t = 0; t < 2; t++) pf[t] = pack_frag(p + t * 8);
#pragma unroll
        for (int t = 0; t < 2; t++)
#pragma unroll
            for (int nb = 0; nb < NB; nb++) o[nb] = CC_MFMA_32x32x16(frag_tr<HD>(vs, nb, t, lane), pf[t], o[nb]);
#pragma unroll
        for (int kk = 0; kk < KK; kk++) kq[kk] = kn[kk];
#pragma unroll
        for (int c = 0; c < HD / 16; c++) vq[c] = vn[c];
    }
    if (q < S) {
        const float inv = l > 0.f ? 1.f / l : 0.f;
        op16_t* orow = out + ((size_t)b * S + q) * D + h * HD;
        store_acc_row<NB, true>(orow, o, half, inv);
        if (half == 0 && lse_out) lse_out[((size_t)b * H + h) * S + q] = m + __logf(l);
    }
}

template <int HD>
static int attn_fwd_mfma_launch(const op16_t* qkv, int B, int S, int H, bool causal, op16_t* out, float* lse, hipStream_t st, Drop drop) {
    const int items = B * H * ((S + 31) / 32);
    const float scale = 1.0f / sqrtf((float)HD);
    if (drop.thresh && !causal) return CC_ERR_SHAPE;
#define CC_L(C, DR) attn_launch<k_attn_fwd_mfma<HD, C, DR>>(dim3((items + 3) / 4), dim3(256), 0, st, qkv, B, S, H, scale, out, lse, drop)
    ATTN_LADDER(CC_L)
#undef CC_L
    return hipGetLastError() == hipSuccess ? CC_OK : CC_ERR_LAUNCH;
}


template <int HD, bool CAUSAL, bool DROP = false>
__global__ __launch_bounds__(256, HD == 64 ? 2 : 1) void k_attn_bwd_dkv(const op16_t* __restrict__ qkv, const op16_t* __restrict__ dout,
                                                      const float* __restrict__ lse, const float* __restrict__ delta, int B, int S, int H,
                                                      float scale, op16_t* __restrict__ dqkv, Drop drop = Drop()) {
    constexpr int KK = HD / 16, NB = HD / 32;
    __shared__ __attribute__((aligned(16))) op16_t qsm[4][32 * AttLd<HD>::v];
    __shared__ __attribute__((aligned(16))) op16_t dsm[4][32 * AttLd<HD>::v];
    __shared__ __attribute__((aligned(16))) float ldsm[4][64];
    const int lane = threadIdx.x & 63, wave = threadIdx.x >> 6;
    const int nblk = (S + 31) >> 5;
    const int item = blockIdx.x * 4 + wave;
    if (item >= B * H * nblk) return;
    const int j = item % nblk, h = (item / nblk) % H, b = item / (nblk * H);
    const int D = H * HD;
    const size_t rs = (size_t)3 * D;
    const op16_t* base = qkv + (size_t)b * S * rs + h * HD;
    const op16_t* dbase = dout + (size_t)b * S * D + h * HD;
    const float* lrow = lse + ((size_t)b * H + h) * S;
    const float* drow = delta + ((size_t)b * H + h) * S;
    const int half = lane >> 5, key = j * 32 + (lane & 31);
    op16x8 kf[KK], vf[KK];
#pragma unroll
    for (int kk = 0; kk < KK; kk++) {
        kf[kk] = load_frag(base + D + (size_t)min(key, S - 1) * rs + kk * 16 + half * 8, key < S);
        vf[kk] = load_frag(base + 2 * D + (size_t)min(key, S - 1) * rs + kk * 16 + half * 8, key < S);
    }
    f32x16 dk[NB], dv[NB];
#pragma unroll
    for (int nb = 0; nb < NB; nb++)
#pragma unroll
        for (int r = 0; r < 16; r++) { dk[nb][r] = 0.f; dv[nb][r] = 0.f; }
    const int i0 = CAUSAL ? j : 0;
    op16x8 qf[KK], df[KK];
    {
        const int qa = i0 * 32 + (lane & 31);
#pragma unroll
        for (int kk = 0; kk < KK; kk++) {
            qf[kk] = load_frag(base + (size_t)min(qa, S - 1) * rs + kk * 16 + half * 8, qa < S);
            df[kk] = load_frag(dbase + (size_t)min(qa, S - 1) * D + kk * 16 + half * 8, qa < S);
        }
    }
    for (int i = i0; i < nblk; i++) {
        op16x8 qn[KK], dn[KK];
        {
            const int qa = (i + 1) * 32 + (lane & 31);
#pragma unroll
            for (int kk = 0; kk < KK; kk++) {
                qn[kk] = load_frag(base + (size_t)min(qa, S - 1) * rs + kk * 16 + half * 8, qa < S);
                dn[kk] = load_frag(dbase + (size_t)min(qa, S - 1) * D + kk * 16 + half * 8, qa < S);
            }
        }
        f32x16 s, dp;
#pragma unroll
        for (int r = 0; r < 16; r++) { s[r] = 0.f; dp[r] = 0.f; }
#pragma unroll
        for (int kk = 0; kk < KK; kk++) {
            s = CC_MFMA_32x32x16(qf[kk], kf[kk], s);
            dp = CC_MFMA_32x32x16(df[kk], vf[kk], dp);
            *reinterpret_cast<op16x8*>(qsm[wave] + (lane & 31) * AttLd<HD>::v + kk * 16 + half * 8) = qf[kk];
            *reinterpret_cast<op16x8*>(dsm[wave] + (lane & 31) * AttLd<HD>::v + kk * 16 + half * 8) = df[kk];
        }
        {
            const int qq = min(i * 32 + (lane & 31), S - 1);
            ldsm[wave][lane] = half ? drow[qq] : lrow[qq];
        }
        float lq[16], dq_[16];
#pragma unroll
        for (int g4 = 0; g4 < 4; g4++) {
            const float4 a = *reinterpret_cast<const float4*>(&ldsm[wave][4 * half + 8 * g4]);
            const float4 b = *reinterpret_cast<const float4*>(&ldsm[wave][32 + 4 * half + 8 * g4]);
            lq[g4 * 4 + 0] = a.x; lq[g4 * 4 + 1] = a.y; lq[g4 * 4 + 2] = a.z; lq[g4 * 4 + 3] = a.w;
            dq_[g4 * 4 + 0] = b.x; dq_[g4 * 4 + 1] = b.y; dq_[g4 * 4 + 2] = b.z; dq_[g4 * 4 + 3] = b.w;
        }
        float p[16], ds[16];
#pragma unroll
        for (int r = 0; r < 16; r++) {
            const int qr = i * 32 + c_row(r, half);
            const bool ok = attn_live<CAUSAL>(qr, key, S);
            p[r] = ok ? __expf(s[r] * scale - lq[r]) : 0.f;
            if (DROP) {
                const float mk = drop_mul(drop, attn_drop_idx(b, H, h, S, min(qr, S - 1), min(key, S - 1)));
                ds[r] = p[r] * (mk * dp[r] - dq_[r]) * scale;
                p[r] *= mk;
            } else {
                ds[r] = p[r] * (dp[r] - dq_[r]) * scale;
            }
        }
        const op16x8 pf[2] = {pack_frag(p), pack_frag(p + 8)};
        const op16x8 dsf[2] = {pack_frag(ds), pack_frag(ds + 8)};
#pragma unroll
        for (int t = 0; t < 2; t++)
#pragma unroll
            for (int nb = 0; nb < NB; nb++) {
                dv[nb] = CC_MFMA_32x32x16(frag_tr<HD>(dsm[wave], nb, t, lane), pf[t], dv[nb]);
                dk[nb] = CC_MFMA_32x32x16(frag_tr<HD>(qsm[wave], nb, t, lane), dsf[t], dk[nb]);
            }
#pragma unroll
        for (int kk = 0; kk < KK; kk++) { qf[kk] = qn[kk]; df[kk] = dn[kk]; }
    }
    if (key < S) {
        op16_t* orow = dqkv + ((size_t)b * S + key) * rs + h * HD;
#pragma unroll
        for (int nb = 0; nb < NB; nb++)
#pragma unroll
            for (int g = 0; g < 4; g++) {
                const int d0 = nb * 32 + 8 * g + 4 * half;
                *reinterpret_cast<uint2*>(orow + D + d0) =
                    make_uint2(pack2op(dk[nb][g * 4 + 0], dk[nb][g * 4 + 1]), pack2op(dk[nb][g * 4 + 2], dk[nb][g * 4 + 3]));
                *reinterpret_cast<uint2*>(orow + 2 * D + d0) =
                    make_uint2(pack2op(dv[nb][g * 4 + 0], dv[nb][g * 4 + 1]), pack2op(dv[nb][g * 4 + 2], dv[nb][g * 4 + 3]));
            }
    }
}

template <int HD, bool CAUSAL, bool DROP = false>
__global__ __launch_bounds__(256, HD == 64 ? 3 : (HD == 96 ? 2 : 1)) void k_attn_bwd_dq(const op16_t* __restrict__ qkv, const op16_t* __restrict__ dout, const op16_t* __restrict__ o,
                                                     const float* __restrict__ lse, float* __restrict__ delta, int B, int S, int H,
                                                     float scale, op16_t* __restrict__ dqkv, Drop drop = Drop()) {
    constexpr int KK = HD / 16, NB = HD / 32;
    __shared__ __attribute__((aligned(16))) op16_t ksm[4][32 * AttLd<HD>::v];
    const int lane = threadIdx.x & 63, wave = threadIdx.x >> 6;
    const int nblk = (S + 31) >> 5;
    const int item = blockIdx.x * 4 + wave;
    if (item >= B * H * nblk) return;
    const int i = item % nblk, h = (item / nblk) % H, b = item / (nblk * H);
    const int D = H * HD;
    const size_t rs = (size_t)3 * D;
    const op16_t* base = qkv + (size_t)b * S * rs + h * HD;
    const op16_t* dbase = dout + (size_t)b * S * D + h * HD;
    const int half = lane >> 5, q = i * 32 + (lane & 31);
    const float my_lse = q < S ? lse[((size_t)b * H + h) * S + q] : 0.f;
    op16x8 qf[KK], dof[KK];
    float my_delta = 0.f;
#pragma unroll
    for (int kk = 0; kk < KK; kk++) {
        qf[kk] = load_frag(base + (size_t)min(q, S - 1) * rs + kk * 16 + half * 8, q < S);
        dof[kk] = load_frag(dbase + (size_t)min(q, S - 1) * D + kk * 16 + half * 8, q < S);
        const op16x8 of = load_frag(o + ((size_t)b * S + min(q, S - 1)) * D + h * HD + kk * 16 + half * 8, q < S);
        float x[8], y[8];
        unpack8(__builtin_bit_cast(uint4, dof[kk]), x);
        unpack8(__builtin_bit_cast(uint4, of), y);
#pragma unroll
        for (int e = 0; e < 8; e++) my_delta += x[e] * y[e];
    }
    my_delta += __shfl_xor(my_delta, 32, 64);
    if (half == 0 && q < S) delta[((size_t)b * H + h) * S + q] = my_delta;
    f32x16 dq[NB];
#pragma unroll
    for (int nb = 0; nb < NB; nb++)
#pragma unroll
        for (int r = 0; r < 16; r++) dq[nb][r] = 0.f;
    const int jend = CAUSAL ? i + 1 : nblk;
    op16x8 kf[KK], vf[KK];
    {
        const int key = lane & 31;
#pragma unroll
        for (int kk = 0; kk < KK; kk++) {
            kf[kk] = load_frag(base + D + (size_t)min(key, S - 1) * rs + kk * 16 + half * 8, key < S);
            vf[kk] = load_frag(base + 2 * D + (size_t)min(key, S - 1) * rs + kk * 16 + half * 8, key < S);
        }
    }
    for (int j = 0; j < jend; j++) {
        op16x8 kn[KK], vn[KK];
        {
            const int key = (j + 1) * 32 + (lane & 31);
#pragma unroll
            for (int kk = 0; kk < KK; kk++) {
                kn[kk] = load_frag(base + D + (size_t)min(key, S - 1) * rs + kk * 16 + half * 8, key < S);
                vn[kk] = load_frag(base + 2 * D + (size_t)min(key, S - 1) * rs + kk * 16 + half * 8, key < S);
            }
        }
        f32x16 st, dpt;
#pragma unroll
        for (int r = 0; r < 16; r++) { st[r] = 0.f; dpt[r] = 0.f; }
#pragma unroll
        for (int kk = 0; kk < KK; kk++) {
            st = CC_MFMA_32x32x16(kf[kk], qf[kk], st);
            dpt = CC_MFMA_32x32x16(vf[kk], dof[kk], dpt);
            *reinterpret_cast<op16x8*>(ksm[wave] + (lane & 31) * AttLd<HD>::v + kk * 16 + half * 8) = kf[kk];
        }
        float ds[16];
#pragma unroll
        for (int r = 0; r < 16; r++) {
            const int kr = j * 32 + c_row(r, half);
            const bool ok = kr < S && q < S && (!CAUSAL || kr <= q);
            const float p = ok ? __expf(st[r] * scale - my_lse) : 0.f;
            const float mk = DROP ? drop_mul(drop, attn_drop_idx(b, H, h, S, min(q, S - 1), min(kr, S - 1))) : 1.0f;
            ds[r] = p * (mk * dpt[r] - my_delta) * scale;
        }
        const op16x8 dsf[2] = {pack_frag(ds), pack_frag(ds + 8)};
#pragma unroll
        for (int t = 0; t < 2; t++)
#pragma unroll
            for (int nb = 0; nb < NB; nb++)
                dq[nb] = CC_MFMA_32x32x16(frag_tr<HD>(ksm[wave], nb, t, lane), dsf[t], dq[nb]);
#pragma unroll
        for (int kk = 0; kk < KK; kk++) { kf[kk] = kn[kk]; vf[kk] = vn[kk]; }
    }
    if (q < S) {
        op16_t* orow = dqkv + ((size_t)b * S + q) * rs + h * HD;
        store_acc_row<NB>(orow, dq, half);
    }
}

#ifndef CC_ATTN_FUSED_OCC
#define CC_ATTN_FUSED_OCC 2
#endif
template <int LD, int ROWS = 32>
__device__ __forceinline__ op16x8 frag_tr_ld(const op16_t* blk, int nb, int t, int lane) {
    typedef __attribute__((ext_vector_type(4))) short s16x4_t;
    typedef __attribute__((address_space(3))) s16x4_t* lp_t;
    const int half = lane >> 5, j = lane & 15, dsub = (lane >> 4) & 1;
    const int r0 = 16 * t + 4 * half + (j >> 2);
    const op16_t* col = blk + nb * 32 + 16 * dsub + 4 * (j & 3);
    const op16_t* p = col + (ROWS < 32 ? min(r0, ROWS - 1) : r0) * LD;
    const op16_t* ph = col + (ROWS < 32 ? min(r0 + 8, ROWS - 1) : r0 + 8) * LD;
    const s16x4_t lo = __builtin_amdgcn_ds_read_tr16_b64_v4i16((lp_t)p);
    const s16x4_t hi = __builtin_amdgcn_ds_read_tr16_b64_v4i16((lp_t)ph);
    typedef __attribute__((ext_vector_type(8))) short s16x8_t;
    const s16x8_t v = {lo[0], lo[1], lo[2], lo[3], hi[0], hi[1], hi[2], hi[3]};
    return __builtin_bit_cast(op16x8, v);
}

template <int HD>
__device__ __forceinline__ void attn_store_tile(op16_t* T, const f32x16 (&acc)[HD / 32], op16_t* gblock, size_t gstride, int rows_left, int lane) {
    constexpr int LD = AttLd<HD>::v, C8 = HD / 8;
    const int half = lane >> 5, l31 = lane & 31;
#pragma unroll
    for (int nb = 0; nb < HD / 32; nb++)
#pragma unroll
        for (int g = 0; g < 4; g++)
            *reinterpret_cast<uint2*>(T + l31 * LD + nb * 32 + 8 * g + 4 * half) =
                make_uint2(pack2op(acc[nb][g * 4 + 0], acc[nb][g * 4 + 1]), pack2op(acc[nb][g * 4 + 2], acc[nb][g * 4 + 3]));
#pragma unroll
    for (int it = 0; it < C8 / 2; it++) {
        const int idx = lane + 64 * it, row = idx / C8, chunk = idx % C8;
        const uint4 v = *reinterpret_cast<const uint4*>(T + row * LD + chunk * 8);
        if (row < rows_left) *reinterpret_cast<uint4*>(gblock + (size_t)row * gstride + chunk * 8) = v;
    }
}

template <int HD, bool CAUSAL, bool DROP, int NBLK, int OCC, int DR = 32>
__global__ __launch_bounds__(256, OCC) void k_attn_bwd_fused(const op16_t* __restrict__ qkv, const op16_t* __restrict__ dout, const op16_t* __restrict__ o,
                                                             const float* __restrict__ lse, int B, int S, int H, float scale,
                                                             op16_t* __restrict__ dqkv, Drop drop = Drop()) {
    constexpr int KK = HD / 16, NB = HD / 32, LD = AttLd<HD>::v;
    constexpr bool SPARE = LD >= HD + 32;
    constexpr int LT = SPARE ? LD : 32;
    __shared__ __attribute__((aligned(16))) op16_t ksm[4][32 * LD];
    __shared__ __attribute__((aligned(16))) op16_t qsm[4][32 * LD];
    __shared__ __attribute__((aligned(16))) op16_t dsm[4][32 * LD];
    static_assert(DR == 32 || (!SPARE && NBLK == 1), "the short dS^T tile is for the single-block form with its own tile");
    __shared__ __attribute__((aligned(16))) op16_t dtx[SPARE ? 1 : 4][SPARE ? 8 : DR * 32];
    __shared__ __attribute__((aligned(16))) float ldsm[4][NBLK][64];
    const int lane = threadIdx.x & 63, wave = threadIdx.x >> 6;
    const int item = blockIdx.x * 4 + wave;
    if (item >= B * H) return;
    const int h = item % H, b = item / H;
    const int D = H * HD;
    const size_t rs = (size_t)3 * D;
    const op16_t* base = qkv + (size_t)b * S * rs + h * HD;
    const op16_t* dbase = dout + (size_t)b * S * D + h * HD;
    const op16_t* obase = o + (size_t)b * S * D + h * HD;
    const float* lrow = lse + ((size_t)b * H + h) * S;
    const int half = lane >> 5, l31 = lane & 31;
    const int coff = half * 8;
    op16_t* dtm = SPARE ? ksm[wave] + HD : dtx[SPARE ? 0 : wave];

    op16x8 qf[KK], dof[KK], kf[KK], vf[KK];
    auto load_q = [&](int i) {
        const int q = i * 32 + l31, qc = min(q, S - 1);
#pragma unroll
        for (int kk = 0; kk < KK; kk++) {
            qf[kk] = load_frag(base + (size_t)qc * rs + kk * 16 + coff, q < S);
            dof[kk] = load_frag(dbase + (size_t)qc * D + kk * 16 + coff, q < S);
        }
    };
    auto load_k = [&](int j) {
        const int key = j * 32 + l31, kc = min(key, S - 1);
#pragma unroll
        for (int kk = 0; kk < KK; kk++) {
            kf[kk] = load_frag(base + D + (size_t)kc * rs + kk * 16 + coff, key < S);
            vf[kk] = load_frag(base + 2 * D + (size_t)kc * rs + kk * 16 + coff, key < S);
        }
    };
    load_k(0);
    load_q(0);
#pragma unroll
    for (int i = 0; i < NBLK; i++) {
        const int q = i * 32 + l31, qc = min(q, S - 1);
        float acc = 0.f;
#pragma unroll
        for (int kk = 0; kk < KK; kk++) {
            const op16x8 df = load_frag(dbase + (size_t)qc * D + kk * 16 + coff, q < S);
            const op16x8 of = load_frag(obase + (size_t)qc * D + kk * 16 + coff, q < S);
            float x[8], y[8];
// ... 918 lines not shown
```

### clipcap_amd/csrc/gemm.hip.h

```cpp
#pragma once
#include <cstdlib>
#include <type_traits>
#include "common.hip.h"
#include "gemm_api.h"
#include "gemm_plan.h"

namespace CC_NS {

using cc_plan::G_BM; using cc_plan::G_BN; using cc_plan::G_BK; using cc_plan::G_THREADS; using cc_plan::G_TILE_BYTES;
using cc_plan::H_BM; using cc_plan::H_BN; using cc_plan::H_BK; using cc_plan::H_NS; using cc_plan::H_STAGE;
constexpr int G_EPI_LD = 68;

struct GemmShape {
    int M, N, K;
    int lda, ldb;
    int k_chunk;
    int group_m;
    int stagger;
    int flags = 0;
};

__device__ __forceinline__ int g_lds_off(int row, int chunk) {
    return row * 128 + (((chunk ^ (row >> 1) ^ ((row >> 4) & 3)) & 7) << 4);
}

struct StageRegs {
    uint4 v[4];
};

__device__ __forceinline__ void g_load_kc(StageRegs& s, const op16_t* __restrict__ base, int ld, int rows, int r0,
                                          int k0, int kend, int tid) {
    const int c = tid & 7, rr = tid >> 3;
    const int k = k0 + c * 8;
#pragma unroll
    for (int i = 0; i < 4; i++) {
        const int r = r0 + rr + 32 * i;
        if (r < rows && k < kend)
            s.v[i] = *reinterpret_cast<const uint4*>(base + (size_t)r * ld + k);
        else
            s.v[i] = make_uint4(0, 0, 0, 0);
    }
}
__device__ __forceinline__ void l_store_kc(const StageRegs& s, char* lds, int tid) {
    const int c = tid & 7, rr = tid >> 3;
#pragma unroll
    for (int i = 0; i < 4; i++) *reinterpret_cast<uint4*>(lds + g_lds_off(rr + 32 * i, c)) = s.v[i];
}

__device__ __forceinline__ void g_load_ks(StageRegs& s, const op16_t* __restrict__ base, int ld, int rows, int r0,
                                          int k0, int kend, int tid) {
    const int ng = (tid & 7) | (((tid >> 4) & 1) << 3);
    const int kg = ((tid >> 3) & 1) | ((tid >> 5) << 1);
    const int r = r0 + ng * 8;
#pragma unroll
    for (int j = 0; j < 4; j++) {
        const int k = k0 + kg * 4 + j;
        if (k < kend && r < rows)
            s.v[j] = *reinterpret_cast<const uint4*>(base + (size_t)k * ld + r);
        else
            s.v[j] = make_uint4(0, 0, 0, 0);
    }
}
__device__ __forceinline__ void l_store_ks(const StageRegs& s, char* lds, int tid) {
    const int ng = (tid & 7) | (((tid >> 4) & 1) << 3);
    const int kg = ((tid >> 3) & 1) | ((tid >> 5) << 1);
    const int kc = kg >> 1, half = (kg & 1) * 8;
    const unsigned in[4][4] = {{s.v[0].x, s.v[0].y, s.v[0].z, s.v[0].w},
                               {s.v[1].x, s.v[1].y, s.v[1].z, s.v[1].w},
                               {s.v[2].x, s.v[2].y, s.v[2].z, s.v[2].w},
                               {s.v[3].x, s.v[3].y, s.v[3].z, s.v[3].w}};
#pragma unroll
    for (int c = 0; c < 4; c++) {
        uint2 ev, od;
        ev.x = __builtin_amdgcn_perm(in[1][c], in[0][c], 0x05040100u);
        ev.y = __builtin_amdgcn_perm(in[3][c], in[2][c], 0x05040100u);
        od.x = __builtin_amdgcn_perm(in[1][c], in[0][c], 0x07060302u);
        od.y = __builtin_amdgcn_perm(in[3][c], in[2][c], 0x07060302u);
        const int n = ng * 8 + 2 * c;
        *reinterpret_cast<uint2*>(lds + g_lds_off(n, kc) + half) = ev;
        *reinterpret_cast<uint2*>(lds + g_lds_off(n + 1, kc) + half) = od;
    }
}

template <int L>
__device__ __forceinline__ void g_load(StageRegs& s, const op16_t* base, int ld, int rows, int r0, int k0, int kend,
                                       int tid) {
    if constexpr (L == 0)
        g_load_kc(s, base, ld, rows, r0, k0, kend, tid);
    else
        g_load_ks(s, base, ld, rows, r0, k0, kend, tid);
}
template <int L>
__device__ __forceinline__ void l_store(const StageRegs& s, char* lds, int tid) {
    if constexpr (L == 0)
        l_store_kc(s, lds, tid);
    else
        l_store_ks(s, lds, tid);
}


template <class E> struct epi_row_strip { static constexpr bool value = false; };
template <class E, class = void> struct epi_acc_init { static constexpr bool value = false; };
template <class E> struct epi_acc_init<E, decltype((void)&E::init4)> { static constexpr bool value = true; };
template <class E, class = void> struct epi_strip_aux { static constexpr bool value = false; typedef char type; };
template <class E> struct epi_strip_aux<E, decltype((void)sizeof(typename E::StripAux))> { static constexpr bool value = true; typedef typename E::StripAux type; };

template <class Epi, int I0 = 0, int I1 = 4>
__device__ __forceinline__ void gemm_epilogue(f32x4 (&acc)[4][4], char* smem, int wave, int lane, int row0, int col0, const Epi& epi) {
    float* strip = reinterpret_cast<float*>(smem) + wave * (16 * G_EPI_LD);
    const int er = (lane >> 4) * 4, ec = lane & 15;
    constexpr bool kAux = epi_strip_aux<Epi>::value;
    typename epi_strip_aux<Epi>::type aux[4][2];
    (void)aux;
    if constexpr (kAux) {
#pragma unroll
        for (int i = I0; i < I1; i++)
#pragma unroll
            for (int s = 0; s < 2; s++) {
                const int q = lane + 64 * s;
                aux[i][s] = epi.load_aux(row0 + i * 16 + (q >> 3), col0 + (q & 7) * 8);
            }
        __builtin_amdgcn_sched_barrier(0);
    }
#pragma unroll
    for (int i = I0; i < I1; i++) {
#pragma unroll
        for (int j = 0; j < 4; j++)
#pragma unroll
            for (int r = 0; r < 4; r++) strip[(er + r) * G_EPI_LD + j * 16 + ec] = acc[i][j][r];
#pragma unroll
        for (int s = 0; s < 2; s++) {
            const int q = lane + 64 * s;
            const int lr = q >> 3, c8 = q & 7;
            float v[8];
            const float4 a = *reinterpret_cast<const float4*>(strip + lr * G_EPI_LD + c8 * 8);
            const float4 b = *reinterpret_cast<const float4*>(strip + lr * G_EPI_LD + c8 * 8 + 4);
            v[0] = a.x; v[1] = a.y; v[2] = a.z; v[3] = a.w; v[4] = b.x; v[5] = b.y; v[6] = b.z; v[7] = b.w;
            if constexpr (kAux) epi(row0 + i * 16 + lr, col0 + c8 * 8, v, aux[i][s]);
            else epi(row0 + i * 16 + lr, col0 + c8 * 8, v);
        }
    }
}

template <class Epi, int NI, int NJ>
__device__ __forceinline__ void gemm_epilogue_regs(f32x4 (&acc)[NI][NJ], int lane, int row0, int col0, const Epi& epi) {
    static_assert(NI % 2 == 0 || NJ % 2 == 0, "leftover column tiles pair along i");
    const int q = lane >> 4, rl = lane & 15;
#define G_PAIR(X, Y, V)                                                                                                  \
    _Pragma("unroll") for (int r_ = 0; r_ < 4; r_++) {                                                                   \
        const auto s_ = __builtin_amdgcn_permlane16_swap(__float_as_uint((X)[r_]), __float_as_uint((Y)[r_]), false, false); \
        (V)[r_] = __uint_as_float(s_[0]);                                                                                \
        (V)[4 + r_] = __uint_as_float(s_[1]);                                                                            \
    }
    if constexpr (epi_row_strip<Epi>::value) {
        static_assert(!epi_row_strip<Epi>::value || NJ == 4, "row-strip epilogues need a 64-column wave strip");
        typename Epi::RowAux tg[NI];
#pragma unroll
        for (int i = 0; i < NI; i++) tg[i] = epi.load_row(row0 + i * 16 + rl);
#pragma unroll
        for (int i = 0; i < NI; i++) {
            float va[8], vb[8];
            G_PAIR(acc[i][0], acc[i][1], va);
            G_PAIR(acc[i][NJ - 2], acc[i][NJ - 1], vb);
            const int cb = col0 + (q & 1) * 16 + (q >> 1) * 8;
            epi.strip(row0 + i * 16 + rl, cb, cb + 32, va, vb, tg[i]);
        }
    } else {
        if constexpr (Epi::kPre) {
#pragma unroll
            for (int i = 0; i < NI; i++)
#pragma unroll
                for (int j = 0; j < NJ; j++) epi.pre4(row0 + i * 16 + rl, col0 + j * 16 + q * 4, acc[i][j]);
        }
        float bias[(NJ + 1) / 2][8];
#pragma unroll
        for (int jp = 0; jp < NJ / 2; jp++) epi.bias8(col0 + (2 * jp + (q & 1)) * 16 + (q >> 1) * 8, bias[jp]);
        if constexpr (NJ & 1) epi.bias8(col0 + (NJ - 1) * 16 + (q >> 1) * 8, bias[NJ / 2]);
        __builtin_amdgcn_sched_barrier(0);
#pragma unroll
        for (int i = 0; i < NI; i++) {
#pragma unroll
            for (int jp = 0; jp < NJ / 2; jp++) {
                float v[8];
                G_PAIR(acc[i][2 * jp], acc[i][2 * jp + 1], v);
                epi.fin(row0 + i * 16 + rl, col0 + (2 * jp + (q & 1)) * 16 + (q >> 1) * 8, v, bias[jp]);
            }
            if constexpr (NJ & 1) {
                if (i & 1) {
                    float v[8];
                    G_PAIR(acc[i - 1][NJ - 1], acc[i][NJ - 1], v);
                    epi.fin(row0 + (i - 1 + (q & 1)) * 16 + rl, col0 + (NJ - 1) * 16 + (q >> 1) * 8, v, bias[NJ / 2]);
                }
            }
        }
    }
#undef G_PAIR
}

__device__ __forceinline__ void tile_coords(int tile, int tiles_m, int tiles_n, int G, int& tm, int& tn) {
    const int band = tile / (G * tiles_n);
    const int first = band * G;
    const int gm = min(G, tiles_m - first);
    const int r = tile - band * G * tiles_n;
    tm = first + r % gm;
    tn = r / gm;
}

__device__ __forceinline__ void acc_zero(f32x4 (&acc)[4][4]) {
#pragma unroll
    for (int i = 0; i < 4; i++)
#pragma unroll
        for (int j = 0; j < 4; j++) acc[i][j] = f32x4{0.f, 0.f, 0.f, 0.f};
}

template <int AL, int BL, class Epi>
__global__ __launch_bounds__(G_THREADS, 2) void gemm_bf16_kernel(const op16_t* __restrict__ A,
                                                                  const op16_t* __restrict__ B, GemmShape g, Epi epi) {
    __shared__ __attribute__((aligned(16))) char smem[4 * G_TILE_BYTES];
    const int tid = threadIdx.x, lane = tid & 63, wave = tid >> 6;
    const int wm = wave >> 1, wn = wave & 1;
    const int tiles_n = (g.N + G_BN - 1) / G_BN, tiles_m = (g.M + G_BM - 1) / G_BM;
    int tm, tn;
    tile_coords(xcd_remap(blockIdx.x, gridDim.x), tiles_m, tiles_n, g.group_m, tm, tn);
    const int m0 = tm * G_BM, n0 = tn * G_BN;
    const int kbeg = blockIdx.z * g.k_chunk;
    const int kend = min(g.K, kbeg + g.k_chunk);
    const int nk = (kend - kbeg + G_BK - 1) / G_BK;

    f32x4 acc[4][4];
    acc_zero(acc);

    StageRegs ra, rb;
    if (nk > 0) {
        g_load<AL>(ra, A, g.lda, g.M, m0, kbeg, kend, tid);
        g_load<BL>(rb, B, g.ldb, g.N, n0, kbeg, kend, tid);
        l_store<AL>(ra, smem, tid);
        l_store<BL>(rb, smem + G_TILE_BYTES, tid);
    }
    __syncthreads();

    const int frow = lane & 15, fchunk = lane >> 4;
    for (int kt = 0; kt < nk; kt++) {
        char* cur = smem + (kt & 1) * 2 * G_TILE_BYTES;
        char* nxt = smem + ((kt + 1) & 1) * 2 * G_TILE_BYTES;
        const bool more = (kt + 1 < nk);
        if (more) {
            const int k0 = kbeg + (kt + 1) * G_BK;
            g_load<AL>(ra, A, g.lda, g.M, m0, k0, kend, tid);
            g_load<BL>(rb, B, g.ldb, g.N, n0, k0, kend, tid);
        }
#pragma unroll
        for (int ks = 0; ks < 2; ks++) {
            op16x8 af[4], bfr[4];
#pragma unroll
            for (int i = 0; i < 4; i++)
                af[i] = *reinterpret_cast<const op16x8*>(cur + g_lds_off(wm * 64 + i * 16 + frow, ks * 4 + fchunk));
#pragma unroll
            for (int j = 0; j < 4; j++)
                bfr[j] = *reinterpret_cast<const op16x8*>(cur + G_TILE_BYTES +
                                                          g_lds_off(wn * 64 + j * 16 + frow, ks * 4 + fchunk));
#pragma unroll
            for (int i = 0; i < 4; i++)
#pragma unroll
                for (int j = 0; j < 4; j++)
                    acc[i][j] = CC_MFMA_16x16x32(af[i], bfr[j], acc[i][j]);
        }
        if (more) {
            l_store<AL>(ra, nxt, tid);
            l_store<BL>(rb, nxt + G_TILE_BYTES, tid);
        }
        __syncthreads();
    }

    gemm_epilogue(acc, smem, wave, lane, m0 + wm * 64, n0 + wn * 64, epi);
}

typedef const __attribute__((address_space(1))) void* gptr_t;
typedef __attribute__((address_space(3))) void* lptr_t;

__device__ __forceinline__ void glds_tile(const op16_t* __restrict__ base, int ld, int rows, int r0, int k0, char* lds, int wave, int lane) {
#pragma unroll
    for (int i = 0; i < 4; i++) {
        const int seg = wave + 4 * i;
        const int row = seg * 8 + (lane >> 3);
        const int chunk = (lane & 7) ^ ((row >> 1) & 7) ^ ((row >> 4) & 3);
        const int gr = min(r0 + row, rows - 1);
        const op16_t* src = base + (size_t)gr * ld + k0 + chunk * 8;
        __builtin_amdgcn_global_load_lds((gptr_t)src, (lptr_t)(lds + seg * 1024), 16, 0, 0);
    }
}

template <class Epi, int ABL = 0>
__global__ __launch_bounds__(G_THREADS, 2) void gemm_nt_glds_kernel(const op16_t* __restrict__ A, const op16_t* __restrict__ B,
                                                                     GemmShape g, Epi epi) {
    __shared__ __attribute__((aligned(1024))) char smem[4 * G_TILE_BYTES];
    const int tid = threadIdx.x, lane = tid & 63;
    const int wave = __builtin_amdgcn_readfirstlane(tid >> 6);
    const int wm = wave >> 1, wn = wave & 1;
    const int tiles_n = (g.N + G_BN - 1) / G_BN, tiles_m = (g.M + G_BM - 1) / G_BM;
    int tm, tn;
    tile_coords(xcd_remap(blockIdx.x, gridDim.x), tiles_m, tiles_n, g.group_m, tm, tn);
    const int m0 = tm * G_BM, n0 = tn * G_BN;
    const int kbeg = blockIdx.z * g.k_chunk;
    const int nk = (min(g.K, kbeg + g.k_chunk) - kbeg) / G_BK;

    f32x4 acc[4][4];
    acc_zero(acc);

    if (g.stagger > 0 && ((blockIdx.x >> 8) & 1)) {
        for (int s_ = g.stagger; s_ > 0; s_ -= 64) __builtin_amdgcn_s_sleep(64);
    }
    glds_tile(A, g.lda, g.M, m0, kbeg, smem, wave, lane);
    glds_tile(B, g.ldb, g.N, n0, kbeg, smem + G_TILE_BYTES, wave, lane);
    const int frow = lane & 15, fchunk = lane >> 4;
    for (int kt = 0; kt < nk; kt++) {
        char* cur = smem + (kt & 1) * 2 * G_TILE_BYTES;
        char* nxt = smem + ((kt + 1) & 1) * 2 * G_TILE_BYTES;
        asm volatile("s_waitcnt vmcnt(0)" ::: "memory");
        __syncthreads();
        if (kt + 1 < nk && !(ABL & 1)) {
            glds_tile(A, g.lda, g.M, m0, kbeg + (kt + 1) * G_BK, nxt, wave, lane);
            glds_tile(B, g.ldb, g.N, n0, kbeg + (kt + 1) * G_BK, nxt + G_TILE_BYTES, wave, lane);
        }
#pragma unroll
        for (int ks = 0; ks < 2; ks++) {
            op16x8 af[4], bfr[4];
#pragma unroll
            for (int i = 0; i < 4; i++) {
                if (!(ABL & 4) || kt == 0) af[i] = *reinterpret_cast<const op16x8*>(cur + g_lds_off(wm * 64 + i * 16 + frow, ks * 4 + fchunk));
                else asm volatile("" : "=v"(af[i]));
            }
#pragma unroll
            for (int j = 0; j < 4; j++) {
                if (!(ABL & 4) || kt == 0) bfr[j] = *reinterpret_cast<const op16x8*>(cur + G_TILE_BYTES + g_lds_off(wn * 64 + j * 16 + frow, ks * 4 + fchunk));
                else asm volatile("" : "=v"(bfr[j]));
            }
            if (ABL & 2) {
#pragma unroll
                for (int i = 0; i < 4; i++) asm volatile("" ::"v"(af[i]), "v"(bfr[i]));
            } else {
#pragma unroll
                for (int i = 0; i < 4; i++)
#pragma unroll
                    for (int j = 0; j < 4; j++)
                        acc[i][j] = CC_MFMA_16x16x32(af[i], bfr[j], acc[i][j]);
            }
        }
    }
    __syncthreads();
    gemm_epilogue(acc, smem, wave, lane, m0 + wm * 64, n0 + wn * 64, epi);
}

template <class Epi>
__global__ __launch_bounds__(G_THREADS, 2) void gemm_nt_glds_x3f_kernel(const op16_t* __restrict__ A, const op16_t* __restrict__ B,
                                                                         GemmShape g, Epi epi) {
    __shared__ __attribute__((aligned(1024))) char smem[4 * G_TILE_BYTES];
    const int tid = threadIdx.x, lane = tid & 63;
    const int wave = __builtin_amdgcn_readfirstlane(tid >> 6);
    const int wm = wave >> 1, wn = wave & 1;
    const int tiles_n = (g.N + G_BN - 1) / G_BN, tiles_m = (g.M + G_BM - 1) / G_BM;
    int tm, tn;
    tile_coords(xcd_remap(blockIdx.x, gridDim.x), tiles_m, tiles_n, g.group_m, tm, tn);
    const int m0 = tm * G_BM, n0 = tn * G_BN;
    const int Kl = g.K / 3, nc = Kl / G_BK;
    f32x4 acc[4][4];
    acc_zero(acc);
    const int frow = lane & 15, fchunk = lane >> 4;
    op16x8 ah[2][4], bh[2][4];
#define X3F_ISSUE(C, LO, BUF)                                                                                            \
    {                                                                                                                    \
        glds_tile(A, g.lda, g.M, m0, (C)*G_BK + ((LO) ? 2 * Kl : 0), (BUF), wave, lane);                                 \
        glds_tile(B, g.ldb, g.N, n0, (C)*G_BK + ((LO) ? Kl : 0), (BUF) + G_TILE_BYTES, wave, lane);                      \
    }
    char* buf0 = smem;
    char* buf1 = smem + 2 * G_TILE_BYTES;
    X3F_ISSUE(0, 0, buf0)
    for (int c = 0; c < nc; c++) {
        asm volatile("s_waitcnt vmcnt(0)" ::: "memory");
        __syncthreads();
        X3F_ISSUE(c, 1, buf1)
#pragma unroll
        for (int ks = 0; ks < 2; ks++) {
#pragma unroll
            for (int i = 0; i < 4; i++) ah[ks][i] = *reinterpret_cast<const op16x8*>(buf0 + g_lds_off(wm * 64 + i * 16 + frow, ks * 4 + fchunk));
#pragma unroll
            for (int j = 0; j < 4; j++) bh[ks][j] = *reinterpret_cast<const op16x8*>(buf0 + G_TILE_BYTES + g_lds_off(wn * 64 + j * 16 + frow, ks * 4 + fchunk));
#pragma unroll
            for (int i = 0; i < 4; i++)
#pragma unroll
                for (int j = 0; j < 4; j++) acc[i][j] = CC_MFMA_16x16x32(ah[ks][i], bh[ks][j], acc[i][j]);
        }
        asm volatile("s_waitcnt vmcnt(0)" ::: "memory");
        __syncthreads();
        if (c + 1 < nc) X3F_ISSUE(c + 1, 0, buf0)
#pragma unroll
        for (int ks = 0; ks < 2; ks++) {
            op16x8 al[4], bl[4];
#pragma unroll
            for (int i = 0; i < 4; i++) al[i] = *reinterpret_cast<const op16x8*>(buf1 + g_lds_off(wm * 64 + i * 16 + frow, ks * 4 + fchunk));
#pragma unroll
            for (int j = 0; j < 4; j++) bl[j] = *reinterpret_cast<const op16x8*>(buf1 + G_TILE_BYTES + g_lds_off(wn * 64 + j * 16 + frow, ks * 4 + fchunk));
#pragma unroll
            for (int i = 0; i < 4; i++)
#pragma unroll
                for (int j = 0; j < 4; j++) acc[i][j] = CC_MFMA_16x16x32(ah[ks][i], bl[j], acc[i][j]);
#pragma unroll
            for (int i = 0; i < 4; i++)
#pragma unroll
                for (int j = 0; j < 4; j++) acc[i][j] = CC_MFMA_16x16x32(al[i], bh[ks][j], acc[i][j]);
        }
    }
#undef X3F_ISSUE
    __syncthreads();
    gemm_epilogue(acc, smem, wave, lane, m0 + wm * 64, n0 + wn * 64, epi);
}

template <class Epi>
__global__ __launch_bounds__(G_THREADS, 1) void gemm_nt_glds4_kernel(const op16_t* __restrict__ A, const op16_t* __restrict__ B,
                                                                      GemmShape g, Epi epi) {
    extern __shared__ __attribute__((aligned(1024))) char smem4[];
    const int tid = threadIdx.x, lane = tid & 63;
    const int wave = __builtin_amdgcn_readfirstlane(tid >> 6);
    const int wm = wave >> 1, wn = wave & 1;
    const int tiles_n = (g.N + G_BN - 1) / G_BN, tiles_m = (g.M + G_BM - 1) / G_BM;
    int tm, tn;
    tile_coords(xcd_remap(blockIdx.x, gridDim.x), tiles_m, tiles_n, g.group_m, tm, tn);
    const int m0 = tm * G_BM, n0 = tn * G_BN;
    const int kbeg = blockIdx.z * g.k_chunk;
    const int nk = (min(g.K, kbeg + g.k_chunk) - kbeg) / G_BK;
    f32x4 acc[4][4];
    acc_zero(acc);
#define G4_ISSUE(T)                                                                                                      \
    {                                                                                                                    \
        char* st_ = smem4 + ((T) & 3) * 2 * G_TILE_BYTES;                                                                \
        glds_tile(A, g.lda, g.M, m0, kbeg + (T)*G_BK, st_, wave, lane);                                                  \
        glds_tile(B, g.ldb, g.N, n0, kbeg + (T)*G_BK, st_ + G_TILE_BYTES, wave, lane);                                   \
    }
    G4_ISSUE(0);
    if (nk > 1) G4_ISSUE(1);
    if (nk > 2) G4_ISSUE(2);
    const int frow = lane & 15, fchunk = lane >> 4;
    for (int kt = 0; kt < nk; kt++) {
        const int rem = min(nk - 1, kt + 2) - kt;
        if (rem >= 2) asm volatile("s_waitcnt vmcnt(16)" ::: "memory");
        else if (rem == 1) asm volatile("s_waitcnt vmcnt(8)" ::: "memory");
        else asm volatile("s_waitcnt vmcnt(0)" ::: "memory");
        __builtin_amdgcn_s_barrier();
        if (kt + 3 < nk) G4_ISSUE(kt + 3);
        const char* cur = smem4 + (kt & 3) * 2 * G_TILE_BYTES;
#pragma unroll
        for (int ks = 0; ks < 2; ks++) {
            op16x8 af[4], bfr[4];
#pragma unroll
            for (int i = 0; i < 4; i++) af[i] = *reinterpret_cast<const op16x8*>(cur + g_lds_off(wm * 64 + i * 16 + frow, ks * 4 + fchunk));
#pragma unroll
            for (int j = 0; j < 4; j++) bfr[j] = *reinterpret_cast<const op16x8*>(cur + G_TILE_BYTES + g_lds_off(wn * 64 + j * 16 + frow, ks * 4 + fchunk));
#pragma unroll
            for (int i = 0; i < 4; i++)
#pragma unroll
                for (int j = 0; j < 4; j++) acc[i][j] = CC_MFMA_16x16x32(af[i], bfr[j], acc[i][j]);
        }
    }
#undef G4_ISSUE
    __syncthreads();
    gemm_epilogue(acc, smem4, wave, lane, m0 + wm * 64, n0 + wn * 64, epi);
}

template <class Epi>
__global__ __launch_bounds__(2 * G_THREADS, 1) void gemm_nt_glds4x2_kernel(const op16_t* __restrict__ A, const op16_t* __restrict__ B,
                                                                            GemmShape g, Epi epi) {
    extern __shared__ __attribute__((aligned(1024))) char smem4[];
    const int tid = threadIdx.x, lane = tid & 63;
    const int wave = __builtin_amdgcn_readfirstlane(tid >> 6);
    const int grp = wave >> 2, w4 = wave & 3;
    const int wm = w4 >> 1, wn = w4 & 1;
    const int tiles_n = (g.N + G_BN - 1) / G_BN, tiles_m = (g.M + G_BM - 1) / G_BM;
    int tm, tn;
    tile_coords(xcd_remap(blockIdx.x, gridDim.x), tiles_m, tiles_n, g.group_m, tm, tn);
    const int m0 = tm * G_BM, n0 = tn * G_BN;
    const int kbeg = blockIdx.z * g.k_chunk;
    const int nk = (min(g.K, kbeg + g.k_chunk) - kbeg) / G_BK;
    f32x4 acc[4][4];
#pragma unroll
    for (int i = 0; i < 4; i++)
#pragma unroll
        for (int j = 0; j < 4; j++) acc[i][j] = f32x4{0.f, 0.f, 0.f, 0.f};
#define G4_ISSUE(T)                                                                                                      \
    {                                                                                                                    \
        char* st_ = smem4 + ((T) & 3) * 2 * G_TILE_BYTES;                                                                \
        if (grp == 0) glds_tile(A, g.lda, g.M, m0, kbeg + (T)*G_BK, st_, w4, lane);                                      \
        else glds_tile(B, g.ldb, g.N, n0, kbeg + (T)*G_BK, st_ + G_TILE_BYTES, w4, lane);                                \
    }
    G4_ISSUE(0);
    if (nk > 1) G4_ISSUE(1);
    if (nk > 2) G4_ISSUE(2);
    const int frow = lane & 15, fchunk = lane >> 4;
    for (int kt = 0; kt < nk; kt++) {
        const int rem = min(nk - 1, kt + 2) - kt;
        if (rem >= 2) asm volatile("s_waitcnt vmcnt(8)" ::: "memory");
        else if (rem == 1) asm volatile("s_waitcnt vmcnt(4)" ::: "memory");
        else asm volatile("s_waitcnt vmcnt(0)" ::: "memory");
        __builtin_amdgcn_s_barrier();
        if (kt + 3 < nk) G4_ISSUE(kt + 3);
        const char* cur = smem4 + (kt & 3) * 2 * G_TILE_BYTES;
        op16x8 af[4], bfr[4];
#pragma unroll
        for (int i = 0; i < 4; i++) af[i] = *reinterpret_cast<const op16x8*>(cur + g_lds_off(wm * 64 + i * 16 + frow, grp * 4 + fchunk));
#pragma unroll
        for (int j = 0; j < 4; j++) bfr[j] = *reinterpret_cast<const op16x8*>(cur + G_TILE_BYTES + g_lds_off(wn * 64 + j * 16 + frow, grp * 4 + fchunk));
#pragma unroll
        for (int i = 0; i < 4; i++)
#pragma unroll
            for (int j = 0; j < 4; j++) acc[i][j] = CC_MFMA_16x16x32(af[i], bfr[j], acc[i][j]);
    }
#undef G4_ISSUE
    __syncthreads();
    f32x4* xch = reinterpret_cast<f32x4*>(smem4 + 4 * 2 * G_TILE_BYTES / 2) + grp * (8 * G_THREADS) + (tid & (G_THREADS - 1));
#pragma unroll
    for (int i = 0; i < 2; i++)
#pragma unroll
        for (int j = 0; j < 4; j++) xch[(i * 4 + j) * G_THREADS] = grp ? acc[i][j] : acc[2 + i][j];
    __syncthreads();
    const f32x4* xin = reinterpret_cast<const f32x4*>(smem4 + 4 * 2 * G_TILE_BYTES / 2) + (grp ^ 1) * (8 * G_THREADS) + (tid & (G_THREADS - 1));
    if (grp == 0) {
#pragma unroll
        for (int i = 0; i < 2; i++)
#pragma unroll
            for (int j = 0; j < 4; j++) acc[i][j] += xin[(i * 4 + j) * G_THREADS];
        gemm_epilogue<Epi, 0, 2>(acc, smem4, wave, lane, m0 + wm * 64, n0 + wn * 64, epi);
    } else {
#pragma unroll
        for (int i = 0; i < 2; i++)
#pragma unroll
            for (int j = 0; j < 4; j++) acc[2 + i][j] += xin[(i * 4 + j) * G_THREADS];
        gemm_epilogue<Epi, 2, 4>(acc, smem4, wave, lane, m0 + wm * 64, n0 + wn * 64, epi);
    }
}

template <class Epi>
__global__ __launch_bounds__(2 * G_THREADS, 1) void gemm_nt_glds4x2_x3f_kernel(const op16_t* __restrict__ A, const op16_t* __restrict__ B,
                                                                            GemmShape g, Epi epi) {
    extern __shared__ __attribute__((aligned(1024))) char smem4[];
    const int tid = threadIdx.x, lane = tid & 63;
    const int wave = __builtin_amdgcn_readfirstlane(tid >> 6);
    const int grp = wave >> 2, w4 = wave & 3;
    const int wm = w4 >> 1, wn = w4 & 1;
    const int tiles_n = (g.N + G_BN - 1) / G_BN, tiles_m = (g.M + G_BM - 1) / G_BM;
    int tm, tn;
    tile_coords(xcd_remap(blockIdx.x, gridDim.x), tiles_m, tiles_n, g.group_m, tm, tn);
    const int m0 = tm * G_BM, n0 = tn * G_BN;
    const int Kl = g.K / 3;
    const int nk = 2 * (Kl / G_BK);
    f32x4 acc[4][4];
    acc_zero(acc);
#define G4_ISSUE(T)                                                                                                      \
    {                                                                                                                    \
        char* st_ = smem4 + ((T) & 3) * 2 * G_TILE_BYTES;                                                                \
        if (grp == 0) glds_tile(A, g.lda, g.M, m0, ((T) >> 1) * G_BK + (((T) & 1) ? 2 * Kl : 0), st_, w4, lane);           \
        else glds_tile(B, g.ldb, g.N, n0, ((T) >> 1) * G_BK + (((T) & 1) ? Kl : 0), st_ + G_TILE_BYTES, w4, lane);       \
    }
    G4_ISSUE(0);
    if (nk > 1) G4_ISSUE(1);
    if (nk > 2) G4_ISSUE(2);
    const int frow = lane & 15, fchunk = lane >> 4;
#define G4_WAIT(KT)                                                                                                      \
    {                                                                                                                    \
        const int rem_ = min(nk - 1, (KT) + 2) - (KT);                                                                   \
        if (rem_ >= 2) asm volatile("s_waitcnt vmcnt(8)" ::: "memory");                                                  \
        else if (rem_ == 1) asm volatile("s_waitcnt vmcnt(4)" ::: "memory");                                             \
        else asm volatile("s_waitcnt vmcnt(0)" ::: "memory");                                                            \
        __builtin_amdgcn_s_barrier();                                                                                    \
        if ((KT) + 3 < nk) G4_ISSUE((KT) + 3);                                                                           \
    }
    op16x8 af[4], bfr[4];
    for (int kt = 0; kt < nk; kt += 2) {
        G4_WAIT(kt)
        const char* cur = smem4 + (kt & 3) * 2 * G_TILE_BYTES;
#pragma unroll
        for (int i = 0; i < 4; i++) af[i] = *reinterpret_cast<const op16x8*>(cur + g_lds_off(wm * 64 + i * 16 + frow, grp * 4 + fchunk));
#pragma unroll
        for (int j = 0; j < 4; j++) bfr[j] = *reinterpret_cast<const op16x8*>(cur + G_TILE_BYTES + g_lds_off(wn * 64 + j * 16 + frow, grp * 4 + fchunk));
#pragma unroll
        for (int i = 0; i < 4; i++)
#pragma unroll
            for (int j = 0; j < 4; j++) acc[i][j] = CC_MFMA_16x16x32(af[i], bfr[j], acc[i][j]);
        G4_WAIT(kt + 1)
        const char* cur2 = smem4 + ((kt + 1) & 3) * 2 * G_TILE_BYTES;
        op16x8 al[4], bl[4];
#pragma unroll
        for (int i = 0; i < 4; i++) al[i] = *reinterpret_cast<const op16x8*>(cur2 + g_lds_off(wm * 64 + i * 16 + frow, grp * 4 + fchunk));
#pragma unroll
        for (int j = 0; j < 4; j++) bl[j] = *reinterpret_cast<const op16x8*>(cur2 + G_TILE_BYTES + g_lds_off(wn * 64 + j * 16 + frow, grp * 4 + fchunk));
#pragma unroll
        for (int i = 0; i < 4; i++)
#pragma unroll
            for (int j = 0; j < 4; j++) acc[i][j] = CC_MFMA_16x16x32(af[i], bl[j], acc[i][j]);
#pragma unroll
        for (int i = 0; i < 4; i++)
#pragma unroll
            for (int j = 0; j < 4; j++) acc[i][j] = CC_MFMA_16x16x32(al[i], bfr[j], acc[i][j]);
    }
#undef G4_WAIT
#undef G4_ISSUE
    __syncthreads();
    f32x4* xch = reinterpret_cast<f32x4*>(smem4 + 4 * 2 * G_TILE_BYTES / 2) + grp * (8 * G_THREADS) + (tid & (G_THREADS - 1));
#pragma unroll
    for (int i = 0; i < 2; i++)
#pragma unroll
        for (int j = 0; j < 4; j++) xch[(i * 4 + j) * G_THREADS] = grp ? acc[i][j] : acc[2 + i][j];
    __syncthreads();
    const f32x4* xin = reinterpret_cast<const f32x4*>(smem4 + 4 * 2 * G_TILE_BYTES / 2) + (grp ^ 1) * (8 * G_THREADS) + (tid & (G_THREADS - 1));
    if (grp == 0) {
#pragma unroll
        for (int i = 0; i < 2; i++)
#pragma unroll
            for (int j = 0; j < 4; j++) acc[i][j] += xin[(i * 4 + j) * G_THREADS];
        gemm_epilogue<Epi, 0, 2>(acc, smem4, wave, lane, m0 + wm * 64, n0 + wn * 64, epi);
    } else {
#pragma unroll
        for (int i = 0; i < 2; i++)
#pragma unroll
            for (int j = 0; j < 4; j++) acc[2 + i][j] += xin[(i * 4 + j) * G_THREADS];
        gemm_epilogue<Epi, 2, 4>(acc, smem4, wave, lane, m0 + wm * 64, n0 + wn * 64, epi);
    }
}

typedef __attribute__((ext_vector_type(16))) float f32x16;
template <int ROWS>
__device__ __forceinline__ void glds_rows(const op16_t* __restrict__ base, int ld, int rows, int r0, int k0, char* lds, int wave, int lane) {
#pragma unroll
    for (int i = 0; i < ROWS / 32; i++) {
        const int seg = wave + 4 * i;
        const int row = seg * 8 + (lane >> 3);
        const int chunk = (lane & 7) ^ ((row >> 1) & 7) ^ ((row >> 4) & 3);
        const int gr = min(r0 + row, rows - 1);
        const op16_t* src = base + (size_t)gr * ld + k0 + chunk * 8;
        __builtin_amdgcn_global_load_lds((gptr_t)src, (lptr_t)(lds + seg * 1024), 16, 0, 0);
    }
}
template <int N> __device__ __forceinline__ void s_wait_vm() {
    __builtin_amdgcn_s_waitcnt((N & 15) | ((N >> 4) << 14) | (7 << 4) | (15 << 8));
    asm volatile("" ::: "memory");
}
template <int ROWS_A, int ROWS_B, int W>
__device__ __forceinline__ void glds_pair(const op16_t* __restrict__ A, int lda, int M, int m0, const op16_t* __restrict__ B, int ldb, int N, int n0,
                                          int k0, char* lds, int wave, int lane) {
#pragma unroll
    for (int i = 0; i < (ROWS_A + ROWS_B) / 8 / W; i++) {
        const bool is_a = W * i < ROWS_A / 8;
        const int seg = wave + W * i - (is_a ? 0 : ROWS_A / 8);
        const int row = seg * 8 + (lane >> 3);
        const int chunk = (lane & 7) ^ ((row >> 1) & 7) ^ ((row >> 4) & 3);
        const op16_t* src = is_a ? A + (size_t)min(m0 + row, M - 1) * lda + k0 + chunk * 8 : B + (size_t)min(n0 + row, N - 1) * ldb + k0 + chunk * 8;
// ... 1469 lines not shown
```

### clipcap_amd/csrc/kernels.h

```cpp
#pragma once
#include <algorithm>
#include <cmath>
#include <cstdlib>
#include "common.hip.h"

namespace CC_NS {

inline dim3 flat_grid(size_t total, int per_block, int cap) { return dim3((unsigned)std::min<size_t>((total + per_block - 1) / per_block, cap)); }

int f32_to_bf16(const float* src, op16_t* dst, size_t n, hipStream_t st);
int f32_to_act(const float* src, act_t* dst, size_t n, hipStream_t st);
int slice_f32_to_bf16(const float* src, size_t src_stride, act_t* dst, size_t dst_stride, int len, int B, hipStream_t st);
int broadcast_rows(float* dst, size_t dst_stride, const float* src, int len, int B, hipStream_t st);
int add_rows(float* dst, size_t dst_stride, const float* add, int len, int B, hipStream_t st);
constexpr size_t RED_SCRATCH_FLOATS = size_t(1) << 20;
int batch_sum(const float* src, size_t src_stride, float* dst, int len, int B, Call& cx);
struct FoldOut { float* p[32]; int m; int k; };
inline float* red_scratch(const Call& cx, size_t floats) { return floats <= RED_SCRATCH_FLOATS ? cx.red : nullptr; }
int fold_partials(const float* part, int S, int n, int groups, const FoldOut& o, hipStream_t st);
int copy_rows(const float* src, size_t src_stride, float* dst, size_t dst_stride, int len, int B, hipStream_t st);

int transpose_bf16(const op16_t* src, op16_t* dst, int R, int C, hipStream_t st);
struct TransposeBatch {
    struct Item { const op16_t* src; op16_t* dst; int R, C; };
    Item it[32];
    int n = 0;
    void add(const op16_t* s, op16_t* d, int R, int C) { it[n++] = Item{s, d, R, C}; }
};
int transpose_bf16_multi(const TransposeBatch& b, hipStream_t st);

int ln_fwd(const float* x, int ldx, const int* row_map, const float* gamma, const float* beta, Act y, float* y32, float* mean,
           float* rstd, int rows, int D, hipStream_t st);
int ln_bwd(const act_t* dy, const float* x, int ldx, const int* row_map, const float* mean, const float* rstd, const float* gamma,
           const float* dres, float* dx32, Act dx16, float* dgamma, float* dbeta, int rows, int D, Call& cx,
           float* dcol = nullptr, Drop dmask = Drop());
int colsum_bf16(const act_t* X, int ld, int M, int N, float* out, Call& cx);
struct ColsumBatch { const act_t* X[32]; float* out[32]; int n = 0; void add(const act_t* x, float* o) { X[n] = x; out[n] = o; n++; } };
int colsum_bf16_multi(const ColsumBatch& b, int ld, int M, int N, Call& cx);

int attn_probs(const act_t* qkv, int B, int S, int H, int hd, float* out, hipStream_t st);
int attn_fwd(const act_t* qkv, int B, int S, int H, int hd, bool causal, Act out, float* lse, hipStream_t st, Drop drop = Drop());
int attn_bwd(const act_t* qkv, const act_t* dout, const act_t* o, const float* lse, float* delta, int B, int S, int H, int hd, bool causal,
             Act dqkv, hipStream_t st, Drop drop = Drop());
bool attn_fwd_can_image(int S, int hd);
bool attn_bwd_can_image(int S, int hd);
int dropout_f32(float* x, size_t n, Drop drop, hipStream_t st);
int dropout_bf16(act_t* x, size_t n, Drop drop, hipStream_t st);
int dropout_mask_u8(unsigned char* out, size_t n, Drop drop, hipStream_t st);

int embed_concat(const float* prefix, const long long* tokens, int cap, const float* wte, const float* wpe, float* x0, int B, int L,
                 int T, int D, int pos0, hipStream_t st);
int f32_to_op16_pad(const float* src, long long lds, int V, act_t* dst, int ldd, int M, hipStream_t st);
constexpr int SCATTER_CHUNK = 512;
constexpr unsigned SC_SKIP = 0xffffffffu;
struct ScatterSrc {
    const int* ids32 = nullptr;
    const long long* ids64 = nullptr;
    const float* f32 = nullptr;
    size_t bstride = 0;
    int rpb = 1;
    size_t ids_ld = 1;
    const act_t* act = nullptr;
    const float* fac = nullptr;
};
size_t scatter_ws_bytes(int R, int D);
int scatter_rows(const ScatterSrc& s, int R, int D, int Vp, float* dst, void* ws, hipStream_t st);

int ce_rows(const float* pmax, const float* psum, int npart, const int* target, const float* tgt_logit, float* lse, float* row_loss,
            float* stats, int M, hipStream_t st);
int score_rows(const float* pmax, const float* psum, int npart, const int* keep, const float* tgt_logit, float* lse, float* token_logprob,
               float* sample_stats, int B, int cap, hipStream_t st);
int ce_dlogits(act_t* logits, int ld, int V, const int* target, const float* lse, const float* denom, const float* loss_scale, int M,
               hipStream_t st, op16_t* img = nullptr);
int ce_targets(const long long* tokens, int* target, int* row_map, int B, int cap, int L, int T, hipStream_t st);
int score_keep(const long long* tokens, int* keep, int n, int ignore_zero, hipStream_t st);
int lm_tgt_ref(const act_t* hf, const op16_t* wte, int D, const int* target, float* cref, int M, hipStream_t st);
int lm_rowfac(const float* cref, const float* lse, const int* target, const float* denom, const float* loss_scale, float* fac, int M, hipStream_t st);
int lm_dgrad_fix(act_t* dhf, const float* fac, const int* target, const op16_t* wte, int D, int M, hipStream_t st);
int lm_scale_rows(const act_t* hf, const float* fac, act_t* out, int D, int M, hipStream_t st);

int adamw(float* p, const float* g, float* m, float* v, size_t n, float lr, float b1, float b2, float eps, float wd, int step, float gscale,
          const float* loss_scale, const float* found_inf, hipStream_t st, op16_t* w16 = nullptr,
          const float* clip = nullptr);
constexpr int GRAD_NORM_BLOCKS = 1024;
constexpr int GRAD_NORM_THREADS = 256;
constexpr int GRAD_NORM_ACC = 4;

int x3_split_rows(const float* src, size_t lds, op16_t* dst, int M, int K, int form, hipStream_t st);
struct X3SplitBatch {
    struct Item { const float* src; op16_t* dst; int R, C, tr, form; };
    Item it[32];
    int n = 0;
    void add(const float* s, op16_t* d, int R, int C, int tr, int form) { it[n++] = Item{s, d, R, C, tr, form}; }
};
int x3_split_multi(const X3SplitBatch& b, hipStream_t st);

}
```

### clipcap_amd/csrc/kernels.hip

```cpp
#include "kernels.h"
#include "gemm_api.h"

namespace CC_NS {

__device__ __forceinline__ void ld8_f32(const float* p, float (&v)[8]) {
    const float4 a = *reinterpret_cast<const float4*>(p), b = *reinterpret_cast<const float4*>(p + 4);
    v[0] = a.x; v[1] = a.y; v[2] = a.z; v[3] = a.w; v[4] = b.x; v[5] = b.y; v[6] = b.z; v[7] = b.w;
}
__global__ void k_f32_to_bf16(const float* __restrict__ src, op16_t* __restrict__ dst, size_t n8) {
    for (size_t i = (size_t)blockIdx.x * blockDim.x + threadIdx.x; i < n8; i += (size_t)gridDim.x * blockDim.x) {
        float v[8];
        ld8_f32(src + 8 * i, v);
        reinterpret_cast<uint4*>(dst)[i] = pack8(v);
    }
}
int f32_to_bf16(const float* src, op16_t* dst, size_t n, hipStream_t st) {
    if (n & 7) return CC_ERR_SHAPE;
    const size_t n8 = n >> 3;
    if (!n8) return CC_OK;
    hipLaunchKernelGGL(k_f32_to_bf16, flat_grid(n8, 256, 2048), dim3(256), 0, st, src, dst, n8);
    return CC_OK;
}

int f32_to_act(const float* src, act_t* dst, size_t n, hipStream_t st) {
    if constexpr (kX3) {
        if (!n) return CC_OK;
        return hipMemcpyAsync(dst, src, n * sizeof(float), hipMemcpyDeviceToDevice, st) == hipSuccess ? CC_OK : CC_ERR_LAUNCH;
    } else {
        return f32_to_bf16(src, reinterpret_cast<op16_t*>(dst), n, st);
    }
}

__global__ void k_slice_f32_to_bf16(const float* __restrict__ src, size_t src_stride, act_t* __restrict__ dst,
                                    size_t dst_stride, int len8, int B) {
    const size_t total = (size_t)len8 * B;
    for (size_t i = (size_t)blockIdx.x * blockDim.x + threadIdx.x; i < total; i += (size_t)gridDim.x * blockDim.x) {
        const int b = (int)(i / len8), c = (int)(i % len8);
        const float* s = src + b * src_stride + (size_t)c * 8;
        float v[8];
        ld8_f32(s, v);
        act_st8(dst + b * dst_stride + (size_t)c * 8, v);
    }
}
int slice_f32_to_bf16(const float* src, size_t src_stride, act_t* dst, size_t dst_stride, int len, int B, hipStream_t st) {
    if (len & 7) return CC_ERR_SHAPE;
    const size_t total = (size_t)(len >> 3) * B;
    if (!total) return CC_OK;
    hipLaunchKernelGGL(k_slice_f32_to_bf16, flat_grid(total, 256, 2048), dim3(256), 0, st, src, src_stride, dst, dst_stride, len >> 3, B);
    return CC_OK;
}

__global__ void k_broadcast_rows(float* __restrict__ dst, size_t dst_stride, const float* __restrict__ src, int len4, int B) {
    const size_t total = (size_t)len4 * B;
    for (size_t i = (size_t)blockIdx.x * blockDim.x + threadIdx.x; i < total; i += (size_t)gridDim.x * blockDim.x) {
        const int b = (int)(i / len4), c = (int)(i % len4);
        reinterpret_cast<float4*>(dst + b * dst_stride)[c] = reinterpret_cast<const float4*>(src)[c];
    }
}
int broadcast_rows(float* dst, size_t dst_stride, const float* src, int len, int B, hipStream_t st) {
    if (len & 3) return CC_ERR_SHAPE;
    const size_t total = (size_t)(len >> 2) * B;
    if (!total) return CC_OK;
    hipLaunchKernelGGL(k_broadcast_rows, flat_grid(total, 256, 2048), dim3(256), 0, st, dst, dst_stride, src, len >> 2, B);
    return CC_OK;
}

__global__ void k_add_rows(float* __restrict__ dst, size_t dst_stride, const float* __restrict__ add, int len, int B) {
    const size_t total = (size_t)len * B;
    for (size_t i = (size_t)blockIdx.x * blockDim.x + threadIdx.x; i < total; i += (size_t)gridDim.x * blockDim.x) {
        const int b = (int)(i / len), c = (int)(i % len);
        dst[b * dst_stride + c] += add[c];
    }
}
int add_rows(float* dst, size_t dst_stride, const float* add, int len, int B, hipStream_t st) {
    const size_t total = (size_t)len * B;
    if (!total) return CC_OK;
    hipLaunchKernelGGL(k_add_rows, flat_grid(total, 256, 2048), dim3(256), 0, st, dst, dst_stride, add, len, B);
    return CC_OK;
}

__global__ void k_copy_rows(const float* __restrict__ src, size_t src_stride, float* __restrict__ dst, size_t dst_stride, int len4, int B) {
    const size_t total = (size_t)len4 * B;
    for (size_t i = (size_t)blockIdx.x * blockDim.x + threadIdx.x; i < total; i += (size_t)gridDim.x * blockDim.x) {
        const int b = (int)(i / len4), c = (int)(i % len4);
        reinterpret_cast<float4*>(dst + b * dst_stride)[c] = reinterpret_cast<const float4*>(src + b * src_stride)[c];
    }
}
int copy_rows(const float* src, size_t src_stride, float* dst, size_t dst_stride, int len, int B, hipStream_t st) {
    if (len & 3) return CC_ERR_SHAPE;
    const size_t total = (size_t)(len >> 2) * B;
    if (!total) return CC_OK;
    hipLaunchKernelGGL(k_copy_rows, flat_grid(total, 256, 2048), dim3(256), 0, st, src, src_stride, dst, dst_stride, len >> 2, B);
    return CC_OK;
}

__global__ __launch_bounds__(256) void k_transpose_bf16_multi(TransposeBatch b) {
    const TransposeBatch::Item& m = b.it[blockIdx.z];
    if ((int)blockIdx.x * 64 >= m.C || (int)blockIdx.y * 64 >= m.R) return;
    __shared__ op16_t tile[64][66];
    const int r0 = blockIdx.y * 64, c0 = blockIdx.x * 64, R = m.R, C = m.C;
    const int cg = threadIdx.x & 7, rl = threadIdx.x >> 3;
#pragma unroll
    for (int p = 0; p < 2; p++) {
        const int r = r0 + rl + 32 * p, c = c0 + cg * 8;
        uint4 v = make_uint4(0, 0, 0, 0);
        if (r < R && c < C) v = *reinterpret_cast<const uint4*>(m.src + (size_t)r * C + c);
        const op16_t* e = reinterpret_cast<const op16_t*>(&v);
#pragma unroll
        for (int k = 0; k < 8; k++) tile[rl + 32 * p][cg * 8 + k] = e[k];
    }
    __syncthreads();
#pragma unroll
    for (int p = 0; p < 2; p++) {
        const int c = c0 + rl + 32 * p, r = r0 + cg * 8;
        if (c < C && r < R) {
            op16_t e[8];
#pragma unroll
            for (int k = 0; k < 8; k++) e[k] = tile[cg * 8 + k][rl + 32 * p];
            *reinterpret_cast<uint4*>(m.dst + (size_t)c * R + r) = *reinterpret_cast<const uint4*>(e);
        }
    }
}
int transpose_bf16_multi(const TransposeBatch& b, hipStream_t st) {
    if (b.n <= 0) return CC_OK;
    int mr = 0, mc = 0;
    for (int i = 0; i < b.n; i++) {
        if ((b.it[i].R & 7) || (b.it[i].C & 7)) return CC_ERR_SHAPE;
        mr = std::max(mr, b.it[i].R);
        mc = std::max(mc, b.it[i].C);
    }
    hipLaunchKernelGGL(k_transpose_bf16_multi, dim3((mc + 63) / 64, (mr + 63) / 64, b.n), dim3(256), 0, st, b);
    return hipGetLastError() == hipSuccess ? CC_OK : CC_ERR_LAUNCH;
}
int transpose_bf16(const op16_t* src, op16_t* dst, int R, int C, hipStream_t st) {
    if ((R & 7) || (C & 7)) return CC_ERR_SHAPE;
    if (R <= 0 || C <= 0) return CC_OK;
    TransposeBatch b;
    b.add(src, dst, R, C);
    return transpose_bf16_multi(b, st);
}

__global__ void k_dropout_f32(float* __restrict__ x, size_t n4, Drop d) {
    for (size_t i = (size_t)blockIdx.x * blockDim.x + threadIdx.x; i < n4; i += (size_t)gridDim.x * blockDim.x) {
        float4 v = reinterpret_cast<float4*>(x)[i];
        const unsigned e = (unsigned)(i * 4);
        float m0, m1, m2, m3;
        drop_mul_pair(d, e, m0, m1);
        drop_mul_pair(d, e + 2, m2, m3);
        v.x *= m0; v.y *= m1; v.z *= m2; v.w *= m3;
        reinterpret_cast<float4*>(x)[i] = v;
    }
}
__global__ void k_dropout_bf16(act_t* __restrict__ x, size_t n8, Drop d) {
    for (size_t i = (size_t)blockIdx.x * blockDim.x + threadIdx.x; i < n8; i += (size_t)gridDim.x * blockDim.x) {
        float f[8];
        act_ld8(x + i * 8, f);
        const unsigned e = (unsigned)(i * 8);
#pragma unroll
        for (int k = 0; k < 8; k += 2) {
            float m0, m1;
            drop_mul_pair(d, e + k, m0, m1);
            f[k] *= m0; f[k + 1] *= m1;
        }
        act_st8(x + i * 8, f);
    }
}
__global__ void k_dropout_mask(unsigned char* __restrict__ out, size_t n, Drop d) {
    for (size_t i = (size_t)blockIdx.x * blockDim.x + threadIdx.x; i < n; i += (size_t)gridDim.x * blockDim.x)
        out[i] = (d.thresh == 0 || drop_keep(d, (unsigned)i)) ? 1 : 0;
}
int dropout_f32(float* x, size_t n, Drop d, hipStream_t st) {
    if (!d.thresh || !n) return CC_OK;
    if (n & 3) return CC_ERR_SHAPE;
    hipLaunchKernelGGL(k_dropout_f32, flat_grid(n / 4, 256, 4096), dim3(256), 0, st, x, n / 4, d);
    return CC_OK;
}
int dropout_bf16(act_t* x, size_t n, Drop d, hipStream_t st) {
    if (!d.thresh || !n) return CC_OK;
    if (n & 7) return CC_ERR_SHAPE;
    hipLaunchKernelGGL(k_dropout_bf16, flat_grid(n / 8, 256, 4096), dim3(256), 0, st, x, n / 8, d);
    return CC_OK;
}
int dropout_mask_u8(unsigned char* out, size_t n, Drop d, hipStream_t st) {
    if (!n) return CC_OK;
    hipLaunchKernelGGL(k_dropout_mask, flat_grid(n, 256, 4096), dim3(256), 0, st, out, n, d);
    return CC_OK;
}

__global__ void k_embed_concat(const float* __restrict__ prefix, const long long* __restrict__ tokens, int cap,
                               const float* __restrict__ wte, const float* __restrict__ wpe, float* __restrict__ x0,
                               int B, int L, int T, int D, int pos0) {
    const int d4n = D >> 2;
    const size_t total = (size_t)B * T * d4n;
    for (size_t i = (size_t)blockIdx.x * blockDim.x + threadIdx.x; i < total; i += (size_t)gridDim.x * blockDim.x) {
        const int c = (int)(i % d4n);
        const int t = (int)((i / d4n) % T), b = (int)(i / ((size_t)d4n * T));
        float4 v;
        if (t < L)
            v = reinterpret_cast<const float4*>(prefix + ((size_t)b * L + t) * D)[c];
        else {
            long long id = tokens[(size_t)b * cap + (t - L)];
            if (id < 0) id = 0;
            v = reinterpret_cast<const float4*>(wte + (size_t)id * D)[c];
        }
        const float4 p = reinterpret_cast<const float4*>(wpe + (size_t)(pos0 + t) * D)[c];
        reinterpret_cast<float4*>(x0)[i] = make_float4(v.x + p.x, v.y + p.y, v.z + p.z, v.w + p.w);
    }
}
int embed_concat(const float* prefix, const long long* tokens, int cap, const float* wte, const float* wpe, float* x0, int B, int L,
                 int T, int D, int pos0, hipStream_t st) {
    if (D & 3) return CC_ERR_SHAPE;
    const size_t total = (size_t)B * T * (D >> 2);
    if (!total) return CC_OK;
    hipLaunchKernelGGL(k_embed_concat, flat_grid(total, 256, 4096), dim3(256), 0, st, prefix, tokens, cap, wte, wpe, x0, B, L, T, D, pos0);
    return CC_OK;
}

__global__ __launch_bounds__(256) void k_f32_to_op16_pad(const float* __restrict__ src, long long lds, int V, act_t* __restrict__ dst, int ldd,
                                                         int M) {
    const size_t total = (size_t)M * ldd;
    for (size_t i = (size_t)blockIdx.x * blockDim.x + threadIdx.x; i < total; i += (size_t)gridDim.x * blockDim.x) {
        const int c = (int)(i % ldd);
        const size_t r = i / ldd;
        dst[i] = c < V ? f2act(src[r * lds + c]) : (act_t)0;
    }
}
int f32_to_op16_pad(const float* src, long long lds, int V, act_t* dst, int ldd, int M, hipStream_t st) {
    const size_t total = (size_t)M * ldd;
    if (!total) return CC_OK;
    hipLaunchKernelGGL(k_f32_to_op16_pad, flat_grid(total, 256, 8192), dim3(256), 0, st, src, lds, V, dst, ldd, M);
    return CC_OK;
}

template <bool DEVSTEP>
__global__ __launch_bounds__(256) void k_adamw(float* __restrict__ p, const float* __restrict__ g, float* __restrict__ m,
                                               float* __restrict__ v, size_t n4, float lr, float b1, float b2, float eps, float wd, float bc1,
                                               float bc2_sqrt, float gscale, const float* __restrict__ loss_scale,
                                               const float* __restrict__ found_inf, op16_t* __restrict__ w16,
                                               const float* __restrict__ clip) {
    if (found_inf && found_inf[0] != 0.f) return;
    if (loss_scale) gscale /= loss_scale[0];
    if (clip) gscale *= clip[0];
    if constexpr (DEVSTEP) {
        const float t = loss_scale[2] + 1.0f;
        bc1 = 1.0f - __builtin_amdgcn_exp2f(t * __log2f(b1));
        bc2_sqrt = sqrtf(1.0f - __builtin_amdgcn_exp2f(t * __log2f(b2)));
    }
    for (size_t i = (size_t)blockIdx.x * blockDim.x + threadIdx.x; i < n4; i += (size_t)gridDim.x * blockDim.x) {
        float4 P = reinterpret_cast<float4*>(p)[i], G = reinterpret_cast<const float4*>(g)[i];
        float4 M = reinterpret_cast<float4*>(m)[i], V = reinterpret_cast<float4*>(v)[i];
        float* pp = &P.x; float* gg = &G.x; float* mm = &M.x; float* vv = &V.x;
#pragma unroll
        for (int e = 0; e < 4; e++) {
            const float gr = gg[e] * gscale;
            pp[e] *= (1.0f - lr * wd);
            mm[e] = b1 * mm[e] + (1.0f - b1) * gr;
            vv[e] = b2 * vv[e] + (1.0f - b2) * gr * gr;
            const float denom = sqrtf(vv[e]) / bc2_sqrt + eps;
            pp[e] -= (lr / bc1) * (mm[e] / denom);
        }
        reinterpret_cast<float4*>(p)[i] = P;
        reinterpret_cast<float4*>(m)[i] = M;
        reinterpret_cast<float4*>(v)[i] = V;
        if (w16) reinterpret_cast<uint2*>(w16)[i] = make_uint2(pack2op(P.x, P.y), pack2op(P.z, P.w));
    }
}
int adamw(float* p, const float* g, float* m, float* v, size_t n, float lr, float b1, float b2, float eps, float wd, int step, float gscale,
          const float* loss_scale, const float* found_inf, hipStream_t st, op16_t* w16, const float* clip) {
    if (n & 3) return CC_ERR_SHAPE;
    if (!n) return CC_OK;
    if (step < 1 && !loss_scale) return CC_ERR_ARG;
    const float bc1 = 1.0f - powf(b1, (float)std::max(step, 1));
    const float bc2s = sqrtf(1.0f - powf(b2, (float)std::max(step, 1)));
    const size_t n4 = n >> 2;
    const dim3 gr = flat_grid(n4, 256, 4096);
    if (step < 1) hipLaunchKernelGGL(k_adamw<true>, gr, dim3(256), 0, st, p, g, m, v, n4, lr, b1, b2, eps, wd, bc1, bc2s, gscale, loss_scale, found_inf, w16, clip);
    else hipLaunchKernelGGL(k_adamw<false>, gr, dim3(256), 0, st, p, g, m, v, n4, lr, b1, b2, eps, wd, bc1, bc2s, gscale, loss_scale, found_inf, w16, clip);
    return CC_OK;
}

#if CC_OP == 2
__global__ __launch_bounds__(256) void k_x3_split_rows(const float* __restrict__ src, size_t lds, op16_t* __restrict__ dst, int M, int K, int form) {
    const int k8 = K >> 3;
    const size_t total = (size_t)M * k8;
    for (size_t i = (size_t)blockIdx.x * blockDim.x + threadIdx.x; i < total; i += (size_t)gridDim.x * blockDim.x) {
        const size_t r = i / k8;
        const int c = (int)(i - r * k8) * 8;
        float f[8];
        ld8_f32(src + r * lds + c, f);
        uint4 hi, lo;
        x3_pair8(f, hi, lo);
        x3_store(dst + r * 3 * (size_t)K, K, c, form, hi, lo);
    }
}
int x3_split_rows(const float* src, size_t lds, op16_t* dst, int M, int K, int form, hipStream_t st) {
    if ((K & 7) || (lds & 3) || ((uintptr_t)src & 15) || ((uintptr_t)dst & 15)) return CC_ERR_SHAPE;
    const size_t total = (size_t)M * (K >> 3);
    if (!total) return CC_OK;
    hipLaunchKernelGGL(k_x3_split_rows, flat_grid(total, 256, 8192), dim3(256), 0, st, src, lds, dst, M, K, form);
    return hipGetLastError() == hipSuccess ? CC_OK : CC_ERR_LAUNCH;
}
__global__ __launch_bounds__(256) void k_x3_split_multi(X3SplitBatch b) {
    const X3SplitBatch::Item& m = b.it[blockIdx.z];
    if ((int)blockIdx.x * 64 >= m.C || (int)blockIdx.y * 64 >= m.R) return;
    __shared__ float tile[64][65];
    const int r0 = blockIdx.y * 64, c0 = blockIdx.x * 64, R = m.R, C = m.C;
    const int cg = threadIdx.x & 7, rl = threadIdx.x >> 3;
    if (!m.tr) {
#pragma unroll
        for (int p = 0; p < 2; p++) {
            const int r = r0 + rl + 32 * p, c = c0 + cg * 8;
            if (r < R && c < C) {
                float f[8];
                ld8_f32(m.src + (size_t)r * C + c, f);
                uint4 hi, lo;
                x3_pair8(f, hi, lo);
                x3_store(m.dst + (size_t)r * 3 * C, C, c, m.form, hi, lo);
            }
        }
        return;
    }
#pragma unroll
    for (int p = 0; p < 2; p++) {
        const int r = r0 + rl + 32 * p, c = c0 + cg * 8;
        float f[8] = {0, 0, 0, 0, 0, 0, 0, 0};
        if (r < R && c < C) ld8_f32(m.src + (size_t)r * C + c, f);
#pragma unroll
        for (int k = 0; k < 8; k++) tile[rl + 32 * p][cg * 8 + k] = f[k];
    }
    __syncthreads();
#pragma unroll
    for (int p = 0; p < 2; p++) {
        const int c = c0 + rl + 32 * p, r = r0 + cg * 8;
        if (c < C && r < R) {
            float f[8];
#pragma unroll
            for (int k = 0; k < 8; k++) f[k] = tile[cg * 8 + k][rl + 32 * p];
            uint4 hi, lo;
            x3_pair8(f, hi, lo);
            x3_store(m.dst + (size_t)c * 3 * R, R, r, m.form, hi, lo);
        }
    }
}
int x3_split_multi(const X3SplitBatch& b, hipStream_t st) {
    if (b.n <= 0) return CC_OK;
    int mr = 0, mc = 0;
    for (int i = 0; i < b.n; i++) {
        if ((b.it[i].R & 7) || (b.it[i].C & 7)) return CC_ERR_SHAPE;
        mr = std::max(mr, b.it[i].R);
        mc = std::max(mc, b.it[i].C);
    }
    hipLaunchKernelGGL(k_x3_split_multi, dim3((mc + 63) / 64, (mr + 63) / 64, b.n), dim3(256), 0, st, b);
    return hipGetLastError() == hipSuccess ? CC_OK : CC_ERR_LAUNCH;
}

const op16_t* x3_operand(Call& cx, const float* src, size_t ld, int rows, int width, int form, bool first, int* rc) {
    if (first) cx.x3_used = 0;
    const size_t need = (((size_t)rows * 3 * width * sizeof(op16_t)) + 255) & ~size_t(255);
    if (!cx.x3 || cx.x3_used + need > cx.x3_bytes) { *rc = CC_ERR_STATE; return nullptr; }
    op16_t* dst = reinterpret_cast<op16_t*>(cx.x3 + cx.x3_used);
    cx.x3_used += need;
    *rc = x3_split_rows(src, ld, dst, rows, width, form, cx.st);
    return *rc == CC_OK ? dst : nullptr;
}
#endif

}
```

### clipcap_amd/csrc/layernorm.hip

```cpp
#include "kernels.h"

namespace CC_NS {

constexpr int LN_MAXV = 8;
#define LN_NV(D, LAUNCH, ...) { if ((D) <= 256) LAUNCH(1, ##__VA_ARGS__); else if ((D) <= 512) LAUNCH(2, ##__VA_ARGS__); else if ((D) <= 768) LAUNCH(3, ##__VA_ARGS__); else if ((D) <= 1024) LAUNCH(4, ##__VA_ARGS__); else LAUNCH(LN_MAXV, ##__VA_ARGS__); }
__device__ __forceinline__ int ln_col(int lane, int it) { return lane * 4 + it * 256; }

template <int NV>
__global__ __launch_bounds__(256) void k_ln_fwd(const float* __restrict__ x, int ldx, const int* __restrict__ row_map,
                                                const float* __restrict__ gamma, const float* __restrict__ beta,
                                                act_t* __restrict__ y, float* __restrict__ y32, float* __restrict__ mean,
                                                float* __restrict__ rstd, int rows, int D, float eps, int img) {
    constexpr int R = NV <= 4 ? 2 : 1;
    const int lane = threadIdx.x & 63;
    const int row0 = (blockIdx.x * 4 + (threadIdx.x >> 6)) * R;
    if (row0 >= rows) return;
    float4 v[R][NV], g[NV], bt[NV];
#pragma unroll
    for (int r = 0; r < R; r++) {
        const int row = min(row0 + r, rows - 1);
        const float* xr = x + (size_t)(row_map ? row_map[row] : row) * ldx;
#pragma unroll
        for (int it = 0; it < NV; it++) {
            const int c = ln_col(lane, it);
            v[r][it] = c < D ? *reinterpret_cast<const float4*>(xr + c) : make_float4(0, 0, 0, 0);
        }
    }
#pragma unroll
    for (int it = 0; it < NV; it++) {
        const int c = ln_col(lane, it);
        g[it] = c < D ? *reinterpret_cast<const float4*>(gamma + c) : make_float4(0, 0, 0, 0);
        bt[it] = c < D ? *reinterpret_cast<const float4*>(beta + c) : make_float4(0, 0, 0, 0);
    }
    float mu[R], rs[R];
#pragma unroll
    for (int r = 0; r < R; r++) {
        float s = 0.f;
#pragma unroll
        for (int it = 0; it < NV; it++) s += v[r][it].x + v[r][it].y + v[r][it].z + v[r][it].w;
        mu[r] = wave_sum(s) / D;
        float q = 0.f;
#pragma unroll
        for (int it = 0; it < NV; it++) {
            const int c = ln_col(lane, it);
            if (c < D) {
                const float a = v[r][it].x - mu[r], b = v[r][it].y - mu[r], cc_ = v[r][it].z - mu[r], d = v[r][it].w - mu[r];
                q += a * a + b * b + cc_ * cc_ + d * d;
            }
        }
        rs[r] = rsqrtf(wave_sum(q) / D + eps);
    }
#pragma unroll
    for (int r = 0; r < R; r++) {
        const int row = row0 + r;
        if (row >= rows) break;
        if (lane == 0) {
            if (mean) mean[row] = mu[r];
            if (rstd) rstd[row] = rs[r];
        }
#pragma unroll
        for (int it = 0; it < NV; it++) {
            const int c = lane * 4 + it * 256;
            if (c < D) {
                const float o0 = (v[r][it].x - mu[r]) * rs[r] * g[it].x + bt[it].x, o1 = (v[r][it].y - mu[r]) * rs[r] * g[it].y + bt[it].y;
                const float o2 = (v[r][it].z - mu[r]) * rs[r] * g[it].z + bt[it].z, o3 = (v[r][it].w - mu[r]) * rs[r] * g[it].w + bt[it].w;
#if CC_OP == 2
                if (y && img) {
                    uint2 hi, lo;
                    x3_pair4(o0, o1, o2, o3, hi, lo);
                    op16_t* r3 = reinterpret_cast<op16_t*>(y) + (size_t)row * 3 * D + c;
                    *reinterpret_cast<uint2*>(r3) = hi;
                    *reinterpret_cast<uint2*>(r3 + D) = hi;
                    *reinterpret_cast<uint2*>(r3 + 2 * D) = lo;
                } else
#endif
                if (y) act_st4(y + (size_t)row * D + c, o0, o1, o2, o3);
                if (y32) *reinterpret_cast<float4*>(y32 + (size_t)row * D + c) = make_float4(o0, o1, o2, o3);
            }
        }
    }
}
int ln_fwd(const float* x, int ldx, const int* row_map, const float* gamma, const float* beta, Act yo, float* y32,
           float* mean, float* rstd, int rows, int D, hipStream_t st) {
    if (D > LN_MAXV * 256 || (D & 3) || (ldx & 3)) return CC_ERR_SHAPE;
    if (rows <= 0) return CC_OK;
    const int rpb = D <= 1024 ? 8 : 4;
    const dim3 gr((rows + rpb - 1) / rpb);
    act_t* const y = yo.p;
    const int img = yo.img ? 1 : 0;
    if (img && (!kX3 || yo.img != D)) return CC_ERR_STATE;
#define LN_FWD(NV) hipLaunchKernelGGL(k_ln_fwd<NV>, gr, dim3(256), 0, st, x, ldx, row_map, gamma, beta, y, y32, mean, rstd, rows, D, 1e-5f, img)
    LN_NV(D, LN_FWD)
#undef LN_FWD
    return CC_OK;
}

template <int NV, bool DG, int NW>
__global__ __launch_bounds__(NW * 64) void k_ln_bwd(const act_t* __restrict__ dy, const float* __restrict__ x, int ldx,
                                                const int* __restrict__ row_map, const float* __restrict__ mean,
                                                const float* __restrict__ rstd, const float* __restrict__ gamma,
                                                const float* __restrict__ dres, float* __restrict__ dx32,
                                                act_t* __restrict__ dx16, float* __restrict__ dgamma, float* __restrict__ dbeta,
                                                float* __restrict__ dcol, int rows, int D, Drop dmask, int img, float* __restrict__ part) {
    extern __shared__ __attribute__((aligned(16))) float ln_red[];
    const int lane = threadIdx.x & 63, wave = threadIdx.x >> 6;
    float4 pg[DG ? NV : 1], pb[DG ? NV : 1], pc[DG ? NV : 1];
#pragma unroll
    for (int it = 0; it < (DG ? NV : 1); it++) pg[it] = pb[it] = pc[it] = make_float4(0, 0, 0, 0);
    float4 gmv[NV];
#pragma unroll
    for (int it = 0; it < NV; it++) {
        const int c = ln_col(lane, it);
        gmv[it] = c < D ? *reinterpret_cast<const float4*>(gamma + c) : make_float4(0, 0, 0, 0);
    }
    struct RowIn { act_raw4 d[NV]; float4 xv[NV], rr[NV]; float mu, rs; size_t xr; };
    auto fetch = [&](int row, RowIn& r) {
        r.xr = (size_t)(row_map ? row_map[row] : row) * ldx;
        r.mu = mean[row]; r.rs = rstd[row];
#pragma unroll
        for (int it = 0; it < NV; it++) {
            const int c = ln_col(lane, it);
            if (c < D) {
                r.d[it] = act_ldraw4(dy + (size_t)row * D + c);
                r.xv[it] = *reinterpret_cast<const float4*>(x + r.xr + c);
                r.rr[it] = dres ? *reinterpret_cast<const float4*>(dres + r.xr + c) : make_float4(0, 0, 0, 0);
            }
        }
    };
    const int rstep = gridDim.x * NW;
    int row = blockIdx.x * NW + wave;
    RowIn cur;
    if (row < rows) fetch(row, cur);
    for (; row < rows; row += rstep) {
        RowIn nxt;
        const bool more = DG && row + rstep < rows;
        if constexpr (DG) { if (more) fetch(row + rstep, nxt); }
        const size_t xr = cur.xr;
        const float mu = cur.mu, rs = cur.rs;
        float4 g[NV], xh[NV], rr[NV];
        float s1 = 0.f, s2 = 0.f;
#pragma unroll
        for (int it = 0; it < NV; it++) {
            const int c = ln_col(lane, it);
            if (c < D) {
                float d0, d1, d2, d3;
                act_unpack4(cur.d[it], d0, d1, d2, d3);
                const float4 xv = cur.xv[it];
                const float4 gm = gmv[it];
                rr[it] = cur.rr[it];
                xh[it] = make_float4((xv.x - mu) * rs, (xv.y - mu) * rs, (xv.z - mu) * rs, (xv.w - mu) * rs);
                g[it] = make_float4(d0 * gm.x, d1 * gm.y, d2 * gm.z, d3 * gm.w);
                s1 += g[it].x + g[it].y + g[it].z + g[it].w;
                s2 += g[it].x * xh[it].x + g[it].y * xh[it].y + g[it].z * xh[it].z + g[it].w * xh[it].w;
                if constexpr (DG) {
                    pg[it].x += d0 * xh[it].x; pg[it].y += d1 * xh[it].y; pg[it].z += d2 * xh[it].z; pg[it].w += d3 * xh[it].w;
                    pb[it].x += d0; pb[it].y += d1; pb[it].z += d2; pb[it].w += d3;
                }
            }
        }
        const float m1 = wave_sum(s1) / D, m2 = wave_sum(s2) / D;
#pragma unroll
        for (int it = 0; it < NV; it++) {
            const int c = ln_col(lane, it);
            if (c < D) {
                float4 o = make_float4(rs * (g[it].x - m1 - xh[it].x * m2), rs * (g[it].y - m1 - xh[it].y * m2),
                                       rs * (g[it].z - m1 - xh[it].z * m2), rs * (g[it].w - m1 - xh[it].w * m2));
                o.x += rr[it].x; o.y += rr[it].y; o.z += rr[it].z; o.w += rr[it].w;
                *reinterpret_cast<float4*>(dx32 + xr + c) = o;
                if (dx16) {
                    if (dmask.thresh) {
                        const unsigned e = (unsigned)(xr + c);
                        float m0, m1, m2, m3;
                        drop_mul_pair(dmask, e, m0, m1);
                        drop_mul_pair(dmask, e + 2, m2, m3);
                        o.x *= m0; o.y *= m1; o.z *= m2; o.w *= m3;
                    }
                    const act_raw4 pk = act_pack4(o.x, o.y, o.z, o.w);
#if CC_OP == 2
                    if (img) {
                        uint2 hi, lo;
                        x3_pair4(o.x, o.y, o.z, o.w, hi, lo);
                        x3_store4(reinterpret_cast<op16_t*>(dx16) + 3 * (size_t)xr + c, D, hi, lo);
                    } else
#endif
                    act_straw4(dx16 + xr + c, pk);
                    if constexpr (DG) {
                        if (dcol) {
                            float r0, r1, r2, r3;
                            act_unpack4(pk, r0, r1, r2, r3);
                            pc[it].x += r0; pc[it].y += r1; pc[it].z += r2; pc[it].w += r3;
                        }
                    }
                }
            }
        }
        if constexpr (DG) { if (more) cur = nxt; } else { if (row + rstep < rows) fetch(row + rstep, cur); }
    }
    if constexpr (DG) {
        float* rg = ln_red;
        float* rb = ln_red + NW * D;
        float* pp = part + (size_t)blockIdx.x * (dcol ? 3 : 2) * D;
#pragma unroll
        for (int it = 0; it < NV; it++) {
            const int c = ln_col(lane, it);
            if (c < D) {
                *reinterpret_cast<float4*>(rg + wave * D + c) = pg[it];
                *reinterpret_cast<float4*>(rb + wave * D + c) = pb[it];
            }
        }
        __syncthreads();
        for (int c = threadIdx.x; c < D; c += NW * 64) {
            float sg = 0.f, sb = 0.f;
#pragma unroll
            for (int w = 0; w < NW; w++) { sg += rg[w * D + c]; sb += rb[w * D + c]; }
            pp[c] = sg;
            pp[D + c] = sb;
        }
        if (dcol) {
            __syncthreads();
#pragma unroll
            for (int it = 0; it < NV; it++) {
                const int c = ln_col(lane, it);
                if (c < D) *reinterpret_cast<float4*>(rg + wave * D + c) = pc[it];
            }
            __syncthreads();
            for (int c = threadIdx.x; c < D; c += NW * 64) {
                float sc = 0.f;
#pragma unroll
                for (int w = 0; w < NW; w++) sc += rg[w * D + c];
                pp[2 * D + c] = sc;
            }
        }
    }
}
int ln_bwd(const act_t* dy, const float* x, int ldx, const int* row_map, const float* mean, const float* rstd,
           const float* gamma, const float* dres, float* dx32, Act dxo, float* dgamma, float* dbeta, int rows, int D,
           Call& cx, float* dcol, Drop dmask) {
    const hipStream_t st = cx.st;
    act_t* const dx16 = dxo.p;
    if (D > LN_MAXV * 256 || (D & 3) || (ldx & 3) || (dcol && (!dgamma || !dx16 || row_map)) || (dmask.thresh && (row_map || ldx != D)))
        return CC_ERR_SHAPE;
    if (rows <= 0) return CC_OK;
    const int nw = (dgamma && (size_t)16 * D * sizeof(float) <= 65536) ? 8 : 4;
    static const int dg_grid = []() { const char* e = cc_lab_env("CC_LNBWD_GRID"); return e ? atoi(e) : 256; }();
    const int nvec = dcol ? 3 : 2;
    const int grid = std::min((rows + nw - 1) / nw, dgamma ? std::max(1, std::min(dg_grid, (int)(RED_SCRATCH_FLOATS / ((size_t)nvec * D)))) : 8192);
    float* part = dgamma ? red_scratch(cx, (size_t)grid * nvec * D) : nullptr;
    if (dgamma && !part) return CC_ERR_STATE;
    const size_t sh = dgamma ? (size_t)2 * nw * D * sizeof(float) : 0;
    const int img = dxo.img ? 1 : 0;
    if (img && (!kX3 || dxo.img != D || ldx != D || dcol || dmask.thresh)) return CC_ERR_STATE;
#define LN_BWD(NV, DG, NW) hipLaunchKernelGGL((k_ln_bwd<NV, DG, NW>), dim3(grid), dim3(NW * 64), sh, st, dy, x, ldx, row_map, mean, rstd, gamma, dres, dx32, dx16, dgamma, dbeta, dcol, rows, D, dmask, img, part)
    if (dgamma && nw == 8) LN_NV(D, LN_BWD, true, 8) else if (dgamma) LN_NV(D, LN_BWD, true, 4) else LN_NV(D, LN_BWD, false, 4)
#undef LN_BWD
    if (!dgamma) return CC_OK;
    FoldOut o{};
    o.p[0] = dgamma; o.p[1] = dbeta; o.p[2] = dcol; o.m = D; o.k = nvec;
    return fold_partials(part, grid, nvec * D, 1, o, st);
}

}
```

Before: 22460 samples/s.

## Fuse backward zero-fills into kernels, add paired attention forward and early epilogue aux loads

Several independent changes land together. A fused mapper seed kernel replaces the memset, copy and convert sequence. The LM-head layernorm backward zeroes the prefix rows itself instead of running full memsets. The GPT-2 backward exits early for the frozen-LM case, running the last layernorm backward only over prefix rows and writing dprefix directly. A one-wave-per-(batch, head) attention forward kernel serves 33-64 token sequences, and the GEMM mainloop loads epilogue aux data two iterations early. Together these aim to cut launch count, memory traffic and skipped work, at the cost of more specialised code paths and extra register pressure.

```diff
diff --git a/clipcap_amd/csrc/api.hip b/clipcap_amd/csrc/api.hip
--- a/clipcap_amd/csrc/api.hip
+++ b/clipcap_amd/csrc/api.hip
@@ -396,11 +396,7 @@
     MapperPass ps(c, B, 1, ws, stream);
     auto& [st, o, w, cx, D, PP, S, M, H, hd, Hm, PD] = ps;
     const uint16_t* w16t = W16(w16, o.total);
-    if (l_hi == c->N) {
-        if (hipMemsetAsync(w.dx32, 0, (size_t)M * D * sizeof(float), st) != hipSuccess) return CC_ERR_LAUNCH;
-        CC_TRY(copy_rows(dout, (size_t)c->L * D, w.dx32 + (size_t)PP * D, (size_t)S * D, c->L * D, B, st));
-        if (c->N > 0) CC_TRY(f32_to_act(w.dx32, w.gdx[c->N - 1], (size_t)M * D, st));
-    }
+    if (l_hi == c->N) CC_TRY(mapper_seed(dout, w.dx32, c->N > 0 ? w.gdx[c->N - 1] : nullptr, PP, S, D, B, st));
     WgradBatch wb;
     wb.defer = true;
     constexpr bool kDeferAll = !kX3;
@@ -693,11 +689,14 @@
             CC_TRY(gemm_wgrad(lg, c->Vp, w.hf16, D, c->Vp, D, Mc, g32 + o.wte, D, w.wg_scratch, cx));
         }
     }
-    if (hipMemsetAsync(w.dx32, 0, (size_t)M * D * sizeof(float), st) != hipSuccess) return CC_ERR_LAUNCH;
-    const size_t dx16_bytes = (size_t)M * D * (w.dx16.img ? 3 * sizeof(op16_t) : sizeof(act_t));
-    if (hipMemsetAsync(w.dx16.p, 0, dx16_bytes, st) != hipSuccess) return CC_ERR_LAUNCH;
+    const bool own_zeros = !full && s->L >= 1 && cap >= 1;
+    if (!own_zeros) {
+        if (hipMemsetAsync(w.dx32, 0, (size_t)M * D * sizeof(float), st) != hipSuccess) return CC_ERR_LAUNCH;
+        const size_t dx16_bytes = (size_t)M * D * (w.dx16.img ? 3 * sizeof(op16_t) : sizeof(act_t));
+        if (hipMemsetAsync(w.dx16.p, 0, dx16_bytes, st) != hipSuccess) return CC_ERR_LAUNCH;
+    }
     CC_TRY(ln_bwd(w.dhf16, w.x[c->NL], D, w.row_map, w.meanf, w.rstdf, w32 + o.lnf_w, nullptr, w.dx32, w.dx16, full ? g32 + o.lnf_w : nullptr,
-                  full ? g32 + o.lnf_b : nullptr, Mc, D, cx));
+                  full ? g32 + o.lnf_b : nullptr, Mc, D, cx, nullptr, Drop(), own_zeros ? LnGeo{1, s->B, s->T, s->L} : LnGeo()));
     return CC_OK;
 }
 
@@ -765,6 +764,7 @@
     WgradBatch wb;
     wb.defer = full;
     WgradBatch* wbp = full ? &wb : nullptr;
+    const bool prefix_only = !full && l_lo == 0 && s->L > 0 && s->L < s->T && !(s->p_embd > 0.f);
     if (full && (w.dx16.img || w.dx16b.img || w.du16.img || w.dqkv16.img)) return CC_ERR_STATE;
     for (int l = l_hi - 1; l >= l_lo; l--) {
         const auto y = o.layer(l);
@@ -797,6 +797,11 @@
         }
         CC_TRY(gemm_bf16out(0, 0, w.dqkv16, D3, W16(w16, y.aw), D3, M, D, D3, w.dxn16, D, nullptr, 0, nullptr, cx));
         if (full) CC_TRY(wgrad_flush(wb, st));
+        if (prefix_only && l == 0) {
+            CC_TRY(ln_bwd(w.dxn16, w.x[0], D, nullptr, w.mean1[0], w.rstd1[0], w32 + y.l1w, w.dx32, dprefix, Act(), nullptr, nullptr, s->B * s->L, D,
+                          cx, nullptr, Drop(), LnGeo{2, s->B, s->T, s->L}));
+            return CC_OK;
+        }
         CC_TRY(ln_bwd(w.dxn16, w.x[l], D, nullptr, w.mean1[l], w.rstd1[l], w32 + y.l1w, w.dx32, w.dx32, w.dx16, full ? g32 + y.l1w : nullptr,
                       full ? g32 + y.l1b : nullptr, M, D, cx, (full && l > 0) ? g32 + o.layer(l - 1).p2b : nullptr,
                       l > 0 ? make_drop(s->p_resid, s->drop_seed, DROP_RESID_MLP, l - 1) : Drop()));
diff --git a/clipcap_amd/csrc/attention.hip b/clipcap_amd/csrc/attention.hip
--- a/clipcap_amd/csrc/attention.hip
+++ b/clipcap_amd/csrc/attention.hip
@@ -549,10 +549,84 @@
 #endif
 
 #if CC_OP != 2
+template <int HD>
+__device__ __forceinline__ void attn_store_tile(op16_t* T, const f32x16 (&acc)[HD / 32], op16_t* gblock, size_t gstride, int rows_left, int lane);
+
+template <int HD>
+__device__ __forceinline__ void attn_fwd_fetch(const op16_t* __restrict__ base, int D, size_t rs, int S, int kb, int lane, uint4 (&kd)[HD / 16],
+                                               uint4 (&vd)[HD / 16]) {
+    constexpr int KK = HD / 16, C8 = HD / 8;
+    const int half = lane >> 5, key = kb * 32 + (lane & 31);
+#pragma unroll
+    for (int kk = 0; kk < KK; kk++) {
+        kd[kk] = *reinterpret_cast<const uint4*>(base + D + (size_t)min(key, S - 1) * rs + kk * 16 + half * 8);
+        if (key >= S) kd[kk] = make_uint4(0, 0, 0, 0);
+    }
+#pragma unroll
+    for (int c = 0; c < HD / 16; c++) {
+        const int idx = lane + 64 * c;
+        const int vk = idx / C8, vc = idx % C8;
+        vd[c] = *reinterpret_cast<const uint4*>(base + 2 * D + (size_t)min(kb * 32 + vk, S - 1) * rs + vc * 8);
+        if (kb * 32 + vk >= S) vd[c] = make_uint4(0, 0, 0, 0);
+    }
+}
+template <int HD, bool CAUSAL, bool DROP>
+__device__ __forceinline__ void attn_fwd_step(const uint4 (&kq)[HD / 16], const uint4 (&vq)[HD / 16], const op16x8 (&qf)[HD / 16], op16_t* vs,
+                                              f32x16 (&o)[HD / 32], float& m, float& l, int kb, int q, int S, float scale, int lane,
+                                              const Drop& drop, int b, int H, int h) {
+    constexpr int KK = HD / 16, NB = HD / 32, C8 = HD / 8;
+    const int half = lane >> 5;
+    f32x16 s;
+    acc_zero(s);
+#pragma unroll
+    for (int kk = 0; kk < KK; kk++) s = CC_MFMA_32x32x16(__builtin_bit_cast(op16x8, kq[kk]), qf[kk], s);
+#pragma unroll
+    for (int c = 0; c < HD / 16; c++) {
+        const int idx = lane + 64 * c;
+        *reinterpret_cast<uint4*>(vs + (idx / C8) * AttLd<HD>::v + (idx % C8) * 8) = vq[c];
+    }
+    float mx = -INFINITY;
+#pragma unroll
+    for (int r = 0; r < 16; r++) {
+        const int kr = kb * 32 + c_row(r, half);
+        const bool ok = kr < S && (!CAUSAL || kr <= q);
+        s[r] = ok ? s[r] * scale : -INFINITY;
+        mx = fmaxf(mx, s[r]);
+    }
+    mx = fmaxf(mx, __shfl_xor(mx, 32, 64));
+    const float m_new = fmaxf(m, mx);
+    const float alpha = (m == -INFINITY) ? 0.f : __expf(m - m_new);
+    float p[16], ps = 0.f;
+#pragma unroll
+    for (int r = 0; r < 16; r++) {
+        p[r] = (m_new == -INFINITY) ? 0.f : __expf(s[r] - m_new);
+        ps += p[r];
+    }
+    ps += __shfl_xor(ps, 32, 64);
+    l = l * alpha + ps;
+    m = m_new;
+#pragma unroll
+    for (int nb = 0; nb < NB; nb++)
+#pragma unroll
+        for (int r = 0; r < 16; r++) o[nb][r] *= alpha;
+    if (DROP) {
+        const unsigned rowbase = attn_drop_idx(b, H, h, S, min(q, S - 1), 0);
+#pragma unroll
+        for (int r = 0; r < 16; r++) p[r] *= drop_mul(drop, rowbase + min(kb * 32 + c_row(r, half), S - 1));
+    }
+    op16x8 pf[2];
+#pragma unroll
+    for (int t = 0; t < 2; t++) pf[t] = pack_frag(p + t * 8);
+#pragma unroll
+    for (int t = 0; t < 2; t++)
+#pragma unroll
+        for (int nb = 0; nb < NB; nb++) o[nb] = CC_MFMA_32x32x16(frag_tr<HD>(vs, nb, t, lane), pf[t], o[nb]);
+}
+
 template <int HD, bool CAUSAL, bool DROP = false>
 __global__ __launch_bounds__(256, HD == 64 ? 3 : 2) void k_attn_fwd_mfma(const op16_t* __restrict__ qkv, int B, int S, int H, float scale,
                                                        op16_t* __restrict__ out, float* __restrict__ lse_out, Drop drop = Drop()) {
-    constexpr int KK = HD / 16, NB = HD / 32, C8 = HD / 8;
+    constexpr int KK = HD / 16, NB = HD / 32;
     __shared__ __attribute__((aligned(16))) op16_t vsm[4][32 * AttLd<HD>::v];
     const int lane = threadIdx.x & 63, wave = threadIdx.x >> 6;
     const int nqb = (S + 31) >> 5;
@@ -575,70 +649,11 @@
     float m = -INFINITY, l = 0.f;
     const int nkb = CAUSAL ? qb + 1 : nqb;
     uint4 kq[KK], vq[HD / 16];
-    auto fetch = [&](int kb, uint4 (&kd)[KK], uint4 (&vd)[HD / 16]) {
-        const int key = kb * 32 + (lane & 31);
-#pragma unroll
-        for (int kk = 0; kk < KK; kk++) {
-            kd[kk] = *reinterpret_cast<const uint4*>(base + D + (size_t)min(key, S - 1) * rs + kk * 16 + half * 8);
-            if (key >= S) kd[kk] = make_uint4(0, 0, 0, 0);
-        }
-#pragma unroll
-        for (int c = 0; c < HD / 16; c++) {
-            const int idx = lane + 64 * c;
-            const int vk = idx / C8, vc = idx % C8;
-            vd[c] = *reinterpret_cast<const uint4*>(base + 2 * D + (size_t)min(kb * 32 + vk, S - 1) * rs + vc * 8);
-            if (kb * 32 + vk >= S) vd[c] = make_uint4(0, 0, 0, 0);
-        }
-    };
-    fetch(0, kq, vq);
+    attn_fwd_fetch<HD>(base, D, rs, S, 0, lane, kq, vq);
     for (int kb = 0; kb < nkb; kb++) {
         uint4 kn[KK], vn[HD / 16];
-        fetch(kb + 1, kn, vn);
-        f32x16 s;
-        acc_zero(s);
-#pragma unroll
-        for (int kk = 0; kk < KK; kk++) s = CC_MFMA_32x32x16(__builtin_bit_cast(op16x8, kq[kk]), qf[kk], s);
-#pragma unroll
-        for (int c = 0; c < HD / 16; c++) {
-            const int idx = lane + 64 * c;
-            *reinterpret_cast<uint4*>(vs + (idx / C8) * AttLd<HD>::v + (idx % C8) * 8) = vq[c];
-        }
-        float mx = -INFINITY;
-#pragma unroll
-        for (int r = 0; r < 16; r++) {
-            const int kr = kb * 32 + c_row(r, half);
-            const bool ok = kr < S && (!CAUSAL || kr <= q);
-            s[r] = ok ? s[r] * scale : -INFINITY;
-            mx = fmaxf(mx, s[r]);
-        }
-        mx = fmaxf(mx, __shfl_xor(mx, 32, 64));
-        const float m_new = fmaxf(m, mx);
-        const float alpha = (m == -INFINITY) ? 0.f : __expf(m - m_new);
-        float p[16], ps = 0.f;
-#pragma unroll
-        for (int r = 0; r < 16; r++) {
-            p[r] = (m_new == -INFINITY) ? 0.f : __expf(s[r] - m_new);
-            ps += p[r];
-        }
-        ps += __shfl_xor(ps, 32, 64);
-        l = l * alpha + ps;
-        m = m_new;
-#pragma unroll
-        for (int nb = 0; nb < NB; nb++)
-#pragma unroll
-            for (int r = 0; r < 16; r++) o[nb][r] *= alpha;
-        if (DROP) {
-            const unsigned rowbase = attn_drop_idx(b, H, h, S, min(q, S - 1), 0);
-#pragma unroll
-            for (int r = 0; r < 16; r++) p[r] *= drop_mul(drop, rowbase + min(kb * 32 + c_row(r, half), S - 1));
-        }
-        op16x8 pf[2];
-#pragma unroll
-        for (int t = 0; t < 2; t++) pf[t] = pack_frag(p + t * 8);
-#pragma unroll
-        for (int t = 0; t < 2; t++)
-#pragma unroll
-            for (int nb = 0; nb < NB; nb++) o[nb] = CC_MFMA_32x32x16(frag_tr<HD>(vs, nb, t, lane), pf[t], o[nb]);
+        attn_fwd_fetch<HD>(base, D, rs, S, kb + 1, lane, kn, vn);
+        attn_fwd_step<HD, CAUSAL, DROP>(kq, vq, qf, vs, o, m, l, kb, q, S, scale, lane, drop, b, H, h);
 #pragma unroll
         for (int kk = 0; kk < KK; kk++) kq[kk] = kn[kk];
 #pragma unroll
@@ -652,11 +667,61 @@
     }
 }
 
+template <bool CAUSAL>
+__global__ __launch_bounds__(256, 3) void k_attn_fwd_mfma_pair(const op16_t* __restrict__ qkv, int B, int S, int H, float scale,
+                                                                op16_t* __restrict__ out, float* __restrict__ lse_out) {
+    constexpr int HD = 64, KK = HD / 16, NB = HD / 32;
+    __shared__ __attribute__((aligned(16))) op16_t vsm[4][32 * AttLd<HD>::v];
+    const int lane = threadIdx.x & 63, wave = threadIdx.x >> 6;
+    const int item = blockIdx.x * 4 + wave;
+    if (item >= B * H) return;
+    const int h = item % H, b = item / H;
+    const int D = H * HD;
+    const size_t rs = (size_t)3 * D;
+    const op16_t* base = qkv + (size_t)b * S * rs + h * HD;
+    const int half = lane >> 5;
+    op16_t* vs = vsm[wave];
+    uint4 kq[2][KK], vq[2][HD / 16];
+#pragma unroll
+    for (int kb = 0; kb < 2; kb++) attn_fwd_fetch<HD>(base, D, rs, S, kb, lane, kq[kb], vq[kb]);
+#pragma unroll
+    for (int qb = 0; qb < 2; qb++) {
+        const int q = qb * 32 + (lane & 31);
+        op16x8 qf[KK];
+#pragma unroll
+        for (int kk = 0; kk < KK; kk++) qf[kk] = load_frag(base + (size_t)min(q, S - 1) * rs + kk * 16 + half * 8, q < S);
+        f32x16 o[NB];
+        acc_zero(o);
+        float m = -INFINITY, l = 0.f;
+#pragma unroll
+        for (int kb = 0; kb < (CAUSAL ? qb + 1 : 2); kb++)
+            attn_fwd_step<HD, CAUSAL, false>(kq[kb], vq[kb], qf, vs, o, m, l, kb, q, S, scale, lane, Drop(), b, H, h);
+        const float inv = l > 0.f ? 1.f / l : 0.f;
+#pragma unroll
+        for (int nb = 0; nb < NB; nb++)
+#pragma unroll
+            for (int r = 0; r < 16; r++) o[nb][r] *= inv;
+        attn_store_tile<HD>(vs, o, out + ((size_t)b * S + qb * 32) * D + h * HD, (size_t)D, S - qb * 32, lane);
+        if (q < S && half == 0 && lse_out) lse_out[((size_t)b * H + h) * S + q] = m + __logf(l);
+    }
+}
+static bool attn_fwd_pair_on() {
+    const char* e = cc_lab_env("CC_ATTN_FWD_PAIR");
+    return !e || atoi(e) != 0;
+}
+
 template <int HD>
 static int attn_fwd_mfma_launch(const op16_t* qkv, int B, int S, int H, bool causal, op16_t* out, float* lse, hipStream_t st, Drop drop) {
     const int items = B * H * ((S + 31) / 32);
     const float scale = 1.0f / sqrtf((float)HD);
     if (drop.thresh && !causal) return CC_ERR_SHAPE;
+    if constexpr (HD == 64) {
+        if (S > 32 && S <= 64 && !drop.thresh && attn_fwd_pair_on()) {
+            if (causal) attn_launch<k_attn_fwd_mfma_pair<true>>(dim3((B * H + 3) / 4), dim3(256), 0, st, qkv, B, S, H, scale, out, lse);
+            else attn_launch<k_attn_fwd_mfma_pair<false>>(dim3((B * H + 3) / 4), dim3(256), 0, st, qkv, B, S, H, scale, out, lse);
+            return hipGetLastError() == hipSuccess ? CC_OK : CC_ERR_LAUNCH;
+        }
+    }
 #define CC_L(C, DR) attn_launch<k_attn_fwd_mfma<HD, C, DR>>(dim3((items + 3) / 4), dim3(256), 0, st, qkv, B, S, H, scale, out, lse, drop)
     ATTN_LADDER(CC_L)
 #undef CC_L
diff --git a/clipcap_amd/csrc/gemm.hip.h b/clipcap_amd/csrc/gemm.hip.h
--- a/clipcap_amd/csrc/gemm.hip.h
+++ b/clipcap_amd/csrc/gemm.hip.h
@@ -106,13 +106,8 @@
 template <class E> struct epi_strip_aux<E, decltype((void)sizeof(typename E::StripAux))> { static constexpr bool value = true; typedef typename E::StripAux type; };
 
 template <class Epi, int I0 = 0, int I1 = 4>
-__device__ __forceinline__ void gemm_epilogue(f32x4 (&acc)[4][4], char* smem, int wave, int lane, int row0, int col0, const Epi& epi) {
-    float* strip = reinterpret_cast<float*>(smem) + wave * (16 * G_EPI_LD);
-    const int er = (lane >> 4) * 4, ec = lane & 15;
-    constexpr bool kAux = epi_strip_aux<Epi>::value;
-    typename epi_strip_aux<Epi>::type aux[4][2];
-    (void)aux;
-    if constexpr (kAux) {
+__device__ __forceinline__ void gemm_epilogue_aux(typename epi_strip_aux<Epi>::type (&aux)[4][2], int lane, int row0, int col0, const Epi& epi) {
+    if constexpr (epi_strip_aux<Epi>::value) {
 #pragma unroll
         for (int i = I0; i < I1; i++)
 #pragma unroll
@@ -120,6 +115,19 @@
                 const int q = lane + 64 * s;
                 aux[i][s] = epi.load_aux(row0 + i * 16 + (q >> 3), col0 + (q & 7) * 8);
             }
+    }
+}
+template <class Epi, int I0 = 0, int I1 = 4, bool EARLY = false>
+__device__ __forceinline__ void gemm_epilogue(f32x4 (&acc)[4][4], char* smem, int wave, int lane, int row0, int col0, const Epi& epi,
+                                              typename epi_strip_aux<Epi>::type (*early)[2] = nullptr) {
+    float* strip = reinterpret_cast<float*>(smem) + wave * (16 * G_EPI_LD);
+    const int er = (lane >> 4) * 4, ec = lane & 15;
+    constexpr bool kAux = epi_strip_aux<Epi>::value;
+    typename epi_strip_aux<Epi>::type own[4][2];
+    (void)own;
+    typename epi_strip_aux<Epi>::type (*aux)[2] = EARLY ? early : own;
+    if constexpr (kAux && !EARLY) {
+        gemm_epilogue_aux<Epi, I0, I1>(own, lane, row0, col0, epi);
         __builtin_amdgcn_sched_barrier(0);
     }
 #pragma unroll
@@ -313,6 +321,10 @@
     glds_tile(A, g.lda, g.M, m0, kbeg, smem, wave, lane);
     glds_tile(B, g.ldb, g.N, n0, kbeg, smem + G_TILE_BYTES, wave, lane);
     const int frow = lane & 15, fchunk = lane >> 4;
+    constexpr bool kEarlyAux = epi_strip_aux<Epi>::value && !kX3 && ABL == 0;
+    typename epi_strip_aux<Epi>::type aux[4][2];
+    (void)aux;
+    const int kaux = max(nk - 2, 0);
     for (int kt = 0; kt < nk; kt++) {
         char* cur = smem + (kt & 1) * 2 * G_TILE_BYTES;
         char* nxt = smem + ((kt + 1) & 1) * 2 * G_TILE_BYTES;
@@ -322,6 +334,9 @@
             glds_tile(A, g.lda, g.M, m0, kbeg + (kt + 1) * G_BK, nxt, wave, lane);
             glds_tile(B, g.ldb, g.N, n0, kbeg + (kt + 1) * G_BK, nxt + G_TILE_BYTES, wave, lane);
         }
+        if constexpr (kEarlyAux) {
+            if (kt == kaux) gemm_epilogue_aux(aux, lane, m0 + wm * 64, n0 + wn * 64, epi);
+        }
 #pragma unroll
         for (int ks = 0; ks < 2; ks++) {
             op16x8 af[4], bfr[4];
@@ -348,7 +363,12 @@
         }
     }
     __syncthreads();
-    gemm_epilogue(acc, smem, wave, lane, m0 + wm * 64, n0 + wn * 64, epi);
+    if constexpr (kEarlyAux) {
+        if (nk <= 0) gemm_epilogue_aux(aux, lane, m0 + wm * 64, n0 + wn * 64, epi);
+        gemm_epilogue<Epi, 0, 4, true>(acc, smem, wave, lane, m0 + wm * 64, n0 + wn * 64, epi, aux);
+    } else {
+        gemm_epilogue(acc, smem, wave, lane, m0 + wm * 64, n0 + wn * 64, epi);
+    }
 }
 
 template <class Epi>
diff --git a/clipcap_amd/csrc/kernels.h b/clipcap_amd/csrc/kernels.h
--- a/clipcap_amd/csrc/kernels.h
+++ b/clipcap_amd/csrc/kernels.h
@@ -19,6 +19,7 @@
 inline float* red_scratch(const Call& cx, size_t floats) { return floats <= RED_SCRATCH_FLOATS ? cx.red : nullptr; }
 int fold_partials(const float* part, int S, int n, int groups, const FoldOut& o, hipStream_t st);
 int copy_rows(const float* src, size_t src_stride, float* dst, size_t dst_stride, int len, int B, hipStream_t st);
+int mapper_seed(const float* dout, float* dx32, act_t* dx16, int PP, int S, int D, int B, hipStream_t st);
 
 int transpose_bf16(const op16_t* src, op16_t* dst, int R, int C, hipStream_t st);
 struct TransposeBatch {
@@ -31,9 +32,10 @@
 
 int ln_fwd(const float* x, int ldx, const int* row_map, const float* gamma, const float* beta, Act y, float* y32, float* mean,
            float* rstd, int rows, int D, hipStream_t st);
+struct LnGeo { int mode = 0, B = 0, T = 0, L = 0; };
 int ln_bwd(const act_t* dy, const float* x, int ldx, const int* row_map, const float* mean, const float* rstd, const float* gamma,
            const float* dres, float* dx32, Act dx16, float* dgamma, float* dbeta, int rows, int D, Call& cx,
-           float* dcol = nullptr, Drop dmask = Drop());
+           float* dcol = nullptr, Drop dmask = Drop(), LnGeo geo = LnGeo());
 int colsum_bf16(const act_t* X, int ld, int M, int N, float* out, Call& cx);
 struct ColsumBatch { const act_t* X[32]; float* out[32]; int n = 0; void add(const act_t* x, float* o) { X[n] = x; out[n] = o; n++; } };
 int colsum_bf16_multi(const ColsumBatch& b, int ld, int M, int N, Call& cx);
diff --git a/clipcap_amd/csrc/kernels.hip b/clipcap_amd/csrc/kernels.hip
--- a/clipcap_amd/csrc/kernels.hip
+++ b/clipcap_amd/csrc/kernels.hip
@@ -91,6 +91,27 @@
     const size_t total = (size_t)(len >> 2) * B;
     if (!total) return CC_OK;
     hipLaunchKernelGGL(k_copy_rows, flat_grid(total, 256, 2048), dim3(256), 0, st, src, src_stride, dst, dst_stride, len >> 2, B);
+    return CC_OK;
+}
+
+__global__ void k_mapper_seed(const float* __restrict__ dout, float* __restrict__ dx32, act_t* __restrict__ dx16, int PP, int S, int D8, int B) {
+    const size_t total = (size_t)B * S * D8;
+    for (size_t i = (size_t)blockIdx.x * blockDim.x + threadIdx.x; i < total; i += (size_t)gridDim.x * blockDim.x) {
+        const size_t row = i / D8;
+        const int c = (int)(i % D8) * 8, t = (int)(row % S);
+        float v[8] = {0.f, 0.f, 0.f, 0.f, 0.f, 0.f, 0.f, 0.f};
+        if (t >= PP) ld8_f32(dout + ((row / S) * (size_t)(S - PP) + (t - PP)) * (D8 * 8) + c, v);
+        float* o = dx32 + row * (D8 * 8) + c;
+        *reinterpret_cast<float4*>(o) = make_float4(v[0], v[1], v[2], v[3]);
+        *reinterpret_cast<float4*>(o + 4) = make_float4(v[4], v[5], v[6], v[7]);
+        if (dx16) act_st8(dx16 + row * (D8 * 8) + c, v);
+    }
+}
+int mapper_seed(const float* dout, float* dx32, act_t* dx16, int PP, int S, int D, int B, hipStream_t st) {
+    if ((D & 7) || PP < 0 || PP > S) return CC_ERR_SHAPE;
+    const size_t total = (size_t)B * S * (D >> 3);
+    if (!total) return CC_OK;
+    hipLaunchKernelGGL(k_mapper_seed, flat_grid(total, 256, 2048), dim3(256), 0, st, dout, dx32, dx16, PP, S, D >> 3, B);
     return CC_OK;
 }
 
diff --git a/clipcap_amd/csrc/layernorm.hip b/clipcap_amd/csrc/layernorm.hip
--- a/clipcap_amd/csrc/layernorm.hip
+++ b/clipcap_amd/csrc/layernorm.hip
@@ -95,15 +95,39 @@
     return CC_OK;
 }
 
-template <int NV, bool DG, int NW>
+template <int NV, bool DG, int NW, int GEO = 0>
 __global__ __launch_bounds__(NW * 64) void k_ln_bwd(const act_t* __restrict__ dy, const float* __restrict__ x, int ldx,
                                                 const int* __restrict__ row_map, const float* __restrict__ mean,
                                                 const float* __restrict__ rstd, const float* __restrict__ gamma,
                                                 const float* __restrict__ dres, float* __restrict__ dx32,
                                                 act_t* __restrict__ dx16, float* __restrict__ dgamma, float* __restrict__ dbeta,
-                                                float* __restrict__ dcol, int rows, int D, Drop dmask, int img, float* __restrict__ part) {
+                                                float* __restrict__ dcol, int rows, int D, Drop dmask, int img, float* __restrict__ part,
+                                                LnGeo geo, int nblk) {
     extern __shared__ __attribute__((aligned(16))) float ln_red[];
     const int lane = threadIdx.x & 63, wave = threadIdx.x >> 6;
+    if constexpr (GEO == 1) {
+        if ((int)blockIdx.x >= nblk) {
+            const int z = ((int)blockIdx.x - nblk) * NW + wave;
+            if (z >= geo.B * geo.L) return;
+            const int b = z / geo.L, j = z % geo.L;
+            const size_t xr = (size_t)(b * geo.T + (j < geo.L - 1 ? j : geo.T - 1)) * ldx;
+#pragma unroll
+            for (int it = 0; it < NV; it++) {
+                const int c = ln_col(lane, it);
+                if (c < D) {
+                    *reinterpret_cast<float4*>(dx32 + xr + c) = make_float4(0, 0, 0, 0);
+                    if (dx16) {
+#if CC_OP == 2
+                        if (img) x3_store4(reinterpret_cast<op16_t*>(dx16) + 3 * (size_t)xr + c, D, make_uint2(0, 0), make_uint2(0, 0));
+                        else
+#endif
+                        act_straw4(dx16 + xr + c, act_pack4(0.f, 0.f, 0.f, 0.f));
+                    }
+                }
+            }
+            return;
+        }
+    }
     float4 pg[DG ? NV : 1], pb[DG ? NV : 1], pc[DG ? NV : 1];
 #pragma unroll
     for (int it = 0; it < (DG ? NV : 1); it++) pg[it] = pb[it] = pc[it] = make_float4(0, 0, 0, 0);
@@ -115,6 +139,7 @@
     }
     struct RowIn { act_raw4 d[NV]; float4 xv[NV], rr[NV]; float mu, rs; size_t xr; };
     auto fetch = [&](int row, RowIn& r) {
+        if constexpr (GEO == 2) row = (row / geo.L) * geo.T + row % geo.L;
         r.xr = (size_t)(row_map ? row_map[row] : row) * ldx;
         r.mu = mean[row]; r.rs = rstd[row];
 #pragma unroll
@@ -127,7 +152,7 @@
             }
         }
     };
-    const int rstep = gridDim.x * NW;
+    const int rstep = (GEO == 1 ? nblk : (int)gridDim.x) * NW;
     int row = blockIdx.x * NW + wave;
     RowIn cur;
     if (row < rows) fetch(row, cur);
@@ -136,6 +161,7 @@
         const bool more = DG && row + rstep < rows;
         if constexpr (DG) { if (more) fetch(row + rstep, nxt); }
         const size_t xr = cur.xr;
+        const size_t xo = GEO == 2 ? (size_t)row * D : xr;
         const float mu = cur.mu, rs = cur.rs;
         float4 g[NV], xh[NV], rr[NV];
         float s1 = 0.f, s2 = 0.f;
@@ -166,7 +192,7 @@
                 float4 o = make_float4(rs * (g[it].x - m1 - xh[it].x * m2), rs * (g[it].y - m1 - xh[it].y * m2),
                                        rs * (g[it].z - m1 - xh[it].z * m2), rs * (g[it].w - m1 - xh[it].w * m2));
                 o.x += rr[it].x; o.y += rr[it].y; o.z += rr[it].z; o.w += rr[it].w;
-                *reinterpret_cast<float4*>(dx32 + xr + c) = o;
+                *reinterpret_cast<float4*>(dx32 + xo + c) = o;
                 if (dx16) {
                     if (dmask.thresh) {
                         const unsigned e = (unsigned)(xr + c);
@@ -235,23 +261,28 @@
 }
 int ln_bwd(const act_t* dy, const float* x, int ldx, const int* row_map, const float* mean, const float* rstd,
            const float* gamma, const float* dres, float* dx32, Act dxo, float* dgamma, float* dbeta, int rows, int D,
-           Call& cx, float* dcol, Drop dmask) {
+           Call& cx, float* dcol, Drop dmask, LnGeo geo) {
     const hipStream_t st = cx.st;
     act_t* const dx16 = dxo.p;
     if (D > LN_MAXV * 256 || (D & 3) || (ldx & 3) || (dcol && (!dgamma || !dx16 || row_map)) || (dmask.thresh && (row_map || ldx != D)))
         return CC_ERR_SHAPE;
+    if (geo.mode && (dgamma || dmask.thresh || geo.B <= 0 || geo.L < 1 || geo.L >= geo.T)) return CC_ERR_SHAPE;
+    if (geo.mode == 1 && (!row_map || rows != geo.B * (geo.T - geo.L))) return CC_ERR_SHAPE;
+    if (geo.mode == 2 && (row_map || dx16 || rows != geo.B * geo.L)) return CC_ERR_SHAPE;
     if (rows <= 0) return CC_OK;
     const int nw = (dgamma && (size_t)16 * D * sizeof(float) <= 65536) ? 8 : 4;
     static const int dg_grid = []() { const char* e = cc_lab_env("CC_LNBWD_GRID"); return e ? atoi(e) : 256; }();
     const int nvec = dcol ? 3 : 2;
-    const int grid = std::min((rows + nw - 1) / nw, dgamma ? std::max(1, std::min(dg_grid, (int)(RED_SCRATCH_FLOATS / ((size_t)nvec * D)))) : 8192);
+    const int nblk = std::min((rows + nw - 1) / nw, dgamma ? std::max(1, std::min(dg_grid, (int)(RED_SCRATCH_FLOATS / ((size_t)nvec * D)))) : 8192);
+    const int grid = nblk + (geo.mode == 1 ? (geo.B * geo.L + nw - 1) / nw : 0);
     float* part = dgamma ? red_scratch(cx, (size_t)grid * nvec * D) : nullptr;
     if (dgamma && !part) return CC_ERR_STATE;
     const size_t sh = dgamma ? (size_t)2 * nw * D * sizeof(float) : 0;
     const int img = dxo.img ? 1 : 0;
     if (img && (!kX3 || dxo.img != D || ldx != D || dcol || dmask.thresh)) return CC_ERR_STATE;
-#define LN_BWD(NV, DG, NW) hipLaunchKernelGGL((k_ln_bwd<NV, DG, NW>), dim3(grid), dim3(NW * 64), sh, st, dy, x, ldx, row_map, mean, rstd, gamma, dres, dx32, dx16, dgamma, dbeta, dcol, rows, D, dmask, img, part)
-    if (dgamma && nw == 8) LN_NV(D, LN_BWD, true, 8) else if (dgamma) LN_NV(D, LN_BWD, true, 4) else LN_NV(D, LN_BWD, false, 4)
+#define LN_BWD(NV, DG, NW, GEO) hipLaunchKernelGGL((k_ln_bwd<NV, DG, NW, GEO>), dim3(grid), dim3(NW * 64), sh, st, dy, x, ldx, row_map, mean, rstd, gamma, dres, dx32, dx16, dgamma, dbeta, dcol, rows, D, dmask, img, part, geo, nblk)
+    if (dgamma && nw == 8) LN_NV(D, LN_BWD, true, 8, 0) else if (dgamma) LN_NV(D, LN_BWD, true, 4, 0)
+    else if (geo.mode == 1) LN_NV(D, LN_BWD, false, 4, 1) else if (geo.mode == 2) LN_NV(D, LN_BWD, false, 4, 2) else LN_NV(D, LN_BWD, false, 4, 0)
 #undef LN_BWD
     if (!dgamma) return CC_OK;
     FoldOut o{};
```

Result: no change. 22670 samples/s (median of 6 runs) (+0.9%).
